# agakshat/spacefortress

Hardware: NVIDIA B200
Metric: env-steps/sec with 84x84 obs (higher is better)
Workload: dtype f64

## Files before the change

### spacefortress_b200/csrc/sf_kernels.cu

```cuda
#include <cuda_runtime.h>
#include <stdio.h>
#include <stdlib.h>
#include <string.h>

#include <algorithm>
#include <mutex>
#include <string>
#include <vector>

#include "../../include/sf_b200.h"
#include "sf_geom.h"
#include "sf_render.cuh"
#include "sf_state.cuh"
#include "sf_step.cuh"
#include "sf_tables.h"

#define SF_WARPS_PER_BLOCK SF_RENDER_WARPS
#define SF_BLOCK (32 * SF_WARPS_PER_BLOCK)
#ifndef SF_BLOCKS_PER_SM
#define SF_BLOCKS_PER_SM 1
#endif

__host__ __device__ inline unsigned sf_hash3(unsigned seed, unsigned long long env, unsigned long long t) {
  unsigned long long z = (env * 0x9E3779B97F4A7C15ull) ^ (t * 0xC2B2AE3D27D4EB4Full) ^ ((unsigned long long)seed << 32 | 0x5Fu);
  z ^= z >> 30; z *= 0xBF58476D1CE4E5B9ull;
  z ^= z >> 27; z *= 0x94D049BB133111EBull;
  z ^= z >> 31;
  return (unsigned)(z >> 32);
}
__host__ __device__ inline int sf_hash_action(unsigned seed, unsigned long long env, unsigned long long t, int num_actions) {
  return (int)(((unsigned long long)sf_hash3(seed, env, t) * (unsigned)num_actions) >> 32);
}

__device__ __forceinline__ long long sf_warp_sum_ll(long long v) {
#pragma unroll
  for (int o = 16; o; o >>= 1) v += __shfl_xor_sync(0xffffffffu, v, o);
  return v;
}

__device__ __noinline__ void sf_accumulate_episode_vals(unsigned long long* epi, bool finished, int lane, int ret_i, int length, int points_bits, int raw_bits,
                                                        int max_vlner, int4 st0, int4 st1, int4 st2) {
  long long f[SF_NUM_EPISODE_STATS];
  long long ret = ret_i;
  f[0] = 1; f[1] = ret; f[2] = ret * ret; f[3] = length;
  f[4] = st0.x; f[5] = st0.y; f[6] = st0.z; f[7] = st0.w;
  f[8] = st1.x; f[9] = st1.y; f[10] = st1.z; f[11] = st1.w;
  f[12] = st2.x; f[13] = st2.y; f[14] = st2.z; f[15] = st2.w; f[16] = max_vlner;
  f[17] = (long long)__float2int_rz(__int_as_float(points_bits));
  f[18] = __double2ll_rn((double)__int_as_float(raw_bits) * 1000.0);
  f[19] = st1.y;
  f[20] = 0; f[21] = 0; f[22] = 0; f[23] = 0;
#pragma unroll
  for (int k = 0; k < 20; k++) {
    long long v = sf_warp_sum_ll(finished ? f[k] : 0);
    if (lane == 0 && v) atomicAdd(&epi[k], (unsigned long long)v);
  }
  int mv = finished ? max_vlner : 0;
  mv = sf_warp_max(mv);
  if (lane == 0 && mv) atomicMax(&epi[20], (unsigned long long)mv);
}
__device__ __forceinline__ void sf_accumulate_episode(const SfDev& D, int env, SfEnv& e, bool finished, int lane) {
  int4 st0 = make_int4(0, 0, 0, 0), st1 = st0, st2 = st0;
  if (finished) { sf_flush_stats(D, env, e); st0 = __ldcg(&D.st0[env]); st1 = __ldcg(&D.st1[env]); st2 = __ldcg(&D.st2[env]); }
  sf_accumulate_episode_vals(D.epi, finished, lane, e.q3.w, e.q3.z, e.q3.x, e.q3.y, e.st3.x, st0, st1, st2);
}
__device__ __noinline__ void sf_accumulate_episode_ref(const SfDev& D, int env, SfEnv& e, bool finished, int lane) {
  sf_accumulate_episode(D, env, e, finished, lane);
}

__device__ __forceinline__ void sf_make_env_rec(const SfEnv& e, int env, unsigned shell_vis, SfEnvRec& r) {
  r.px = e.pos.x; r.py = e.pos.y;
  r.core = (unsigned)e.q0.x; r.pmask = (unsigned)e.q0.y;
  r.points_i = __float2int_rz(__int_as_float(e.q3.x));
  r.vuln = e.q1.z;
  r.kill_bar = (e.q1.z > 10 && e.q1.y < 250) ? 1 : 0;
  r.env = env;
  r.s0 = 0; r.ebox = 0;
  if (!(r.core & SF_CORE_SHIP_ALIVE)) {
    const SfPt c = sf_xform_base(r.px, r.py);
    r.ebox = (((c.x >> 8) - 13) + 64) | ((((c.y >> 8) - 13) + 64) << 8);
  }
  r.life = (unsigned)e.st3.z + 1u;
  r.building = 0;
  r.ns = sf_count_strokes(r.core, r.pmask, shell_vis);
  r.shell_vis = (int)shell_vis;
}

struct SfSched {
  int next_group, done;
};

struct SfRollArgs {
  int T, EB, ngroups, flags;
  const int* actions;
  unsigned action_seed;
  long long t0;
  unsigned char* obs;
  int* reward;
  unsigned char* done;
  unsigned char* fortkill;
  unsigned* events;
  SfSched* sched;
  int env0, envn;
  uint4* host_obs;
  uint4* mirror;
  unsigned long long* delta_stats;
  int delta_lanes;
};

__device__ __noinline__ void sf_step_group(const SfDev& D, const SfRollArgs& A, int group, int t, SfEnvRec* recs) {
  const int lane = threadIdx.x & 31;
  const SfHot* H = &sf_block_smem().hot;
  const bool autoreset = !(A.flags & SF_FLAG_NO_AUTORESET);
  const int env = A.env0 + group * A.EB + lane;
  const bool mine = lane < A.EB && env < A.env0 + A.envn;
  SfEnv e;
  bool finished = false;
  unsigned shell_vis = 0;
#ifdef SF_BARRIER_TIMING
  unsigned stmask_ = __ballot_sync(0xffffffffu, mine);
#endif
  SF_ST_BEGIN();
  SfStepSmem& SS = sf_block_smem().step;
  const bool first_tick = t == 0, last_tick = t == A.T - 1;
  if (mine) {
    if (first_tick) sf_load_env(D, env, e);
    else {
      e.pos = SS.pos[lane]; e.vel = SS.vel[lane];
      e.q0 = SS.q0[lane]; e.q1 = SS.q1[lane]; e.q2 = SS.q2[lane]; e.q3 = SS.q3[lane]; e.st3 = SS.st3[lane];
      e.d0 = SS.d0[lane]; e.d1 = SS.d1[lane]; e.d2 = SS.d2[lane];
    }
#ifdef SF_BARRIER_TIMING
    if (e.q0.x == 0x7fffffff) e.q0.y = 0;
#endif
    SF_ST(8);
    int a = A.actions ? A.actions[(size_t)t * D.n + env]
                      : sf_hash_action(A.action_seed, (unsigned long long)(D.first_global_env + env), (unsigned long long)(A.t0 + t), D.num_actions);
    int km = (A.flags & SF_FLAG_ACTIONS_ARE_KEYMASKS) ? (a & 15) : D.keymask_of_action[min(max(a, 0), D.num_actions - 1)];
    SfStepOut o;
#ifdef SF_BARRIER_TIMING
    o.sync_mask = stmask_;
#endif
    sf_env_step(D, H, env, e, km, autoreset, (A.flags & SF_FLAG_RAW_REWARD) != 0, o);
    size_t oi = (size_t)t * D.n + env;
    if (A.reward) A.reward[oi] = o.reward;
    if (A.done) A.done[oi] = o.done;
    if (A.fortkill) A.fortkill[oi] = o.fort_kill;
    if (A.events) A.events[oi] = o.events;
    finished = o.done && autoreset;
    shell_vis = o.shell_vis;
  }
#ifdef SF_BARRIER_TIMING
  ts_ = clock64(); stmask_ = 0xffffffffu;
#endif
  if (__any_sync(0xffffffffu, finished)) {
#ifdef SF_STEP_ENV_BY_REF
    sf_accumulate_episode_ref(D, env, e, finished, lane);
#else
    sf_accumulate_episode(D, env, e, finished, lane);
#endif
    if (finished) { sf_new_game(D, H, env, e); shell_vis = 0; }
  }
  if (mine) {
    if (last_tick) sf_store_env(D, env, e);
    else {
      SS.pos[lane] = e.pos; SS.vel[lane] = e.vel;
      SS.q0[lane] = e.q0; SS.q1[lane] = e.q1; SS.q2[lane] = e.q2; SS.q3[lane] = e.q3; SS.st3[lane] = e.st3;
      if ((t & 7) == 7) sf_flush_stats(D, env, e);
      SS.d0[lane] = e.d0; SS.d1[lane] = e.d1; SS.d2[lane] = e.d2;
    }
    sf_make_env_rec(e, env, shell_vis, recs[lane]);
  } else recs[lane].env = -1;
  __syncwarp();
  SF_ST(15);
}


__device__ __noinline__ void sf_rollout_stepper(const SfDev& D, const SfRollArgs& A) {
  const int lane = threadIdx.x & 31;
  SfBlockSmem& B = sf_block_smem();
  const bool native = (A.flags & SF_FLAG_NATIVE_OBS) != 0;
  int stage = 0, group = blockIdx.x;
#pragma unroll 1
  for (int k = 1; group < A.ngroups; k ^= 1) {
    if (lane == 0) B.next_group[k] = A.sched ? (int)gridDim.x + atomicAdd(&A.sched->next_group, 1) : group + (int)gridDim.x;
    sf_stepper_ticks(D, B, lane, native, A.T, stage, [&](int t, SfTeamSmem& Tm, int h) { sf_step_group(D, A, group, t, &Tm.env[32 * h]); });
    group = B.next_group[k];
  }
  if (lane == 0 && A.sched) {
    __threadfence();
    if (atomicAdd(&A.sched->done, 1) == (int)gridDim.x - 1) { A.sched->next_group = 0; A.sched->done = 0; __threadfence(); }
  }
}
__device__ __forceinline__ void sf_rollout_drawer(const SfDev& D, const SfRollArgs& A) {
  const int lane = threadIdx.x & 31;
  SfBlockSmem& B = sf_block_smem();
  SfWarpSmem& W = sf_my_smem();
  SfFrameOut out;
  out.native = (A.flags & SF_FLAG_NATIVE_OBS) ? 1 : 0;
  out.obs_bytes = out.native ? (size_t)SF_NAT_H * SF_NAT_W : (size_t)84 * 84;
  out.obs = A.obs;
  out.tick_bytes = (size_t)D.n * out.obs_bytes;
  SfStageState st;
  st.stage = 0; st.prev_used = 0;
  int group = blockIdx.x;
#pragma unroll 1
  for (int k = 1; group < A.ngroups; k ^= 1) {
    sf_drawer_ticks(D, B, W, lane, out, A.T, st);
    group = B.next_group[k];
  }
}

__device__ __noinline__ void sf_block_host_delta(const SfDev& D, const SfRollArgs& A) {
  const unsigned lane = threadIdx.x & 31;
  const unsigned gmask = (1u << A.delta_lanes) - 1u, gsh = lane & ~(unsigned)(A.delta_lanes - 1);
  const uint4* cur = reinterpret_cast<const uint4*>(A.obs);
  const size_t per16 = (size_t)(84 * 84) / 16;
  unsigned sent = 0;
#pragma unroll 1
  for (int group = blockIdx.x; group < A.ngroups; group += gridDim.x) {
    const int env_lo = A.env0 + group * A.EB, env_hi = min(env_lo + A.EB, A.env0 + A.envn);
    const size_t c1 = (size_t)env_hi * per16;
#pragma unroll 1
    for (size_t base = (size_t)env_lo * per16; base < c1; base += 4 * SF_BLOCK) {
      uint4 a[4], b[4];
#pragma unroll
      for (int u = 0; u < 4; u++) {
        const size_t i = base + u * SF_BLOCK + threadIdx.x;
        a[u] = b[u] = make_uint4(0, 0, 0, 0);
        if (i < c1) { a[u] = __ldcg(cur + i); b[u] = __ldcg(A.mirror + i); }
      }
#pragma unroll
      for (int u = 0; u < 4; u++) {
        const size_t i = base + u * SF_BLOCK + threadIdx.x;
        const bool diff = (a[u].x != b[u].x) | (a[u].y != b[u].y) | (a[u].z != b[u].z) | (a[u].w != b[u].w);
        const unsigned m = __ballot_sync(0xffffffffu, diff);
        if (m == 0) continue;
        if (i < c1 && ((m >> gsh) & gmask)) { A.host_obs[i] = a[u]; sent++; }
        if (diff) A.mirror[i] = a[u];
      }
    }
  }
  for (int o = 16; o; o >>= 1) sent += __shfl_xor_sync(0xffffffffu, sent, o);
  if (lane == 0 && sent) atomicAdd(&A.delta_stats[0], (unsigned long long)sent * 16u);
  if (blockIdx.x == 0 && threadIdx.x == 0) atomicAdd(&A.delta_stats[1], 1ull);
}

template <bool HOST_DELTA>
__global__ void __launch_bounds__(SF_BLOCK, SF_BLOCKS_PER_SM) sf_rollout_kernel(const __grid_constant__ SfDev D, const __grid_constant__ SfRollArgs A) {
  sf_block_smem_init(D.static_image);
  sf_warp_smem_init(sf_my_smem(), threadIdx.x & 31);
  if (threadIdx.x < 32) sf_rollout_stepper(D, A); else sf_rollout_drawer(D, A);
  if (HOST_DELTA) {
    __syncthreads();
    sf_block_host_delta(D, A);
  }
}

__global__ void __launch_bounds__(128) sf_step_only_kernel(SfDev D, SfRollArgs A) {
  const int env = A.env0 + blockIdx.x * blockDim.x + threadIdx.x;
  const int lane = threadIdx.x & 31;
  const bool mine = env < A.env0 + A.envn;
  const bool autoreset = !(A.flags & SF_FLAG_NO_AUTORESET);
  SfEnv e;
  if (mine) sf_load_env(D, env, e);
  for (int t = 0; t < A.T; t++) {
    bool finished = false;
    if (mine) {
      int a = A.actions ? A.actions[(size_t)t * D.n + env]
                        : sf_hash_action(A.action_seed, (unsigned long long)(D.first_global_env + env), (unsigned long long)(A.t0 + t), D.num_actions);
      int km = (A.flags & SF_FLAG_ACTIONS_ARE_KEYMASKS) ? (a & 15) : D.keymask_of_action[min(max(a, 0), D.num_actions - 1)];
      SfStepOut o;
#ifdef SF_BARRIER_TIMING
      o.sync_mask = __activemask();
#endif
      sf_env_step(D, &D.tab->hot, env, e, km, autoreset, (A.flags & SF_FLAG_RAW_REWARD) != 0, o);
      size_t oi = (size_t)t * D.n + env;
      if (A.reward) A.reward[oi] = o.reward;
      if (A.done) A.done[oi] = o.done;
      if (A.fortkill) A.fortkill[oi] = o.fort_kill;
      if (A.events) A.events[oi] = o.events;
      finished = o.done && autoreset;
    }
    if (__any_sync(0xffffffffu, finished)) {
      sf_accumulate_episode(D, env, e, finished, lane);
      if (finished) sf_new_game(D, &D.tab->hot, env, e);
    }
    if (mine && (t & 7) == 7) sf_flush_stats(D, env, e);
  }
  if (mine) sf_store_env(D, env, e);
}

__global__ void __launch_bounds__(SF_BLOCK, SF_BLOCKS_PER_SM) sf_render_kernel(SfDev D, unsigned char* obs, int flags, const unsigned char* mask, int EB, int ngroups) {
  const int lane = threadIdx.x & 31;
  SfBlockSmem& B = sf_block_smem();
  SfWarpSmem& W = sf_my_smem();
  sf_block_smem_init(D.static_image);
  sf_warp_smem_init(W, lane);
  const bool native = (flags & SF_FLAG_NATIVE_OBS) != 0;
  if (threadIdx.x < 32) {
    int stage = 0;
#pragma unroll 1
    for (int group = blockIdx.x; group < ngroups; group += gridDim.x)
      sf_stepper_ticks(D, B, lane, native, 1, stage, [&](int, SfTeamSmem& Tm, int) {
        const int env = group * EB + lane;
        const bool mine = lane < EB && env < D.n && (!mask || mask[env]);
        if (mine) {
          SfEnv e;
          sf_load_env(D, env, e);
          sf_make_env_rec(e, env, sf_visible_shells(D, env, (unsigned)e.q0.y), Tm.env[lane]);
        } else Tm.env[lane].env = -1;
        __syncwarp();
      });
  } else {
    SfFrameOut out;
    out.native = native ? 1 : 0;
    out.obs_bytes = out.native ? (size_t)SF_NAT_H * SF_NAT_W : (size_t)84 * 84;
    out.obs = obs;
    out.tick_bytes = 0;
    SfStageState st;
    st.stage = 0; st.prev_used = 0;
#pragma unroll 1
    for (int group = blockIdx.x; group < ngroups; group += gridDim.x) sf_drawer_ticks(D, B, W, lane, out, 1, st);
  }
}

__global__ void __launch_bounds__(SF_BLOCK) sf_pack_static_kernel(SfDev D, unsigned char* image) {
  sf_block_smem_fill(D.tab);
  __syncthreads();
  const int4* src = reinterpret_cast<const int4*>(&sf_block_smem());
  for (int k = threadIdx.x; k < (int)(SF_STATIC_BYTES / 16); k += blockDim.x) reinterpret_cast<int4*>(image)[k] = src[k];
}

__global__ void sf_seed_kernel(SfDev D, const unsigned* seeds) {
  const int env = blockIdx.x * blockDim.x + threadIdx.x;
  if (env >= D.n) return;
  SfEnv e;
  sf_load_env(D, env, e);
  sf_srand(D, env, e, seeds ? seeds[env] : 1u);
  D.expstamp[env] = 0;
  D.expo_meta[env] = make_uint2(0u, 0u);
  sf_store_env(D, env, e);
}

__global__ void sf_set_ticks_kernel(SfDev D, const int* ticks) {
  const int env = blockIdx.x * blockDim.x + threadIdx.x;
  if (env >= D.n) return;
  int4 q = D.q3[env];
  q.z = max(ticks[env], 0);
  D.q3[env] = q;
}

__global__ void sf_reset_kernel(SfDev D, const unsigned char* mask, int clear_prev_vlner) {
  const int env = blockIdx.x * blockDim.x + threadIdx.x;
  if (env >= D.n) return;
  if (mask && !mask[env]) return;
  SfEnv e;
  sf_load_env(D, env, e);
  if (clear_prev_vlner) e.q1.w = 0;
  sf_new_game(D, &D.tab->hot, env, e);
  sf_store_env(D, env, e);
}


struct SfExtra { double vdir, aim, ndist; };
__device__ inline SfExtra sf_compute_extra(const SfEnv& e) {
  SfExtra x;
  x.vdir = 0.0; x.aim = 0.0; x.ndist = 0.0;
  if (e.q3.z == 0) return x;
  const double ang = (double)((unsigned)e.q0.x & SF_CORE_ANGLE_MASK);
  if (SF_DSQRT(SF_DADD(SF_DMUL(e.vel.x, e.vel.x), SF_DMUL(e.vel.y, e.vel.y))) != 0.0) {
    const double o = atan2(-SF_DSUB(SF_FORT_Y, e.pos.y), SF_DSUB(SF_FORT_X, e.pos.x));
    const double v = atan2(e.vel.y, e.vel.x);
    double d = SF_DSUB(v, o);
    if (d > SF_PI) d = SF_DSUB(d, SF_PI * 2);
    if (d < -SF_PI) d = SF_DADD(d, SF_PI * 2);
    x.vdir = sf_rad2deg(d);
  }
  double o = atan2(SF_DSUB(e.pos.y, SF_FORT_Y), SF_DSUB(e.pos.x, SF_FORT_X));
  o = SF_DADD(SF_DSUB(sf_rad2deg(o), ang), 180.0);
  if (o < -180.0) o = SF_DADD(o, 360.0);
  x.aim = o;
  const double dx = SF_DSUB(e.pos.x, SF_FORT_X), dy0 = SF_DSUB(e.pos.y, e.pos.y);
  const double fdist = SF_DSQRT(SF_DADD(SF_DMUL(dx, dx), SF_DMUL(dy0, dy0)));
  x.ndist = SF_DADD(-1.0, SF_DDIV(SF_DSUB(fdist, 40.0), SF_DDIV(SF_DSUB(200.0, 40.0), 2.0)));
  return x;
}
__device__ __forceinline__ double sf_clip1(double v) { return v < -1.0 ? -1.0 : (v > 1.0 ? 1.0 : v); }
__device__ __forceinline__ double sf_pymod360(double v) {
  double m = fmod(v, 360.0);
  if (m != 0.0) { if (m < 0.0) m = SF_DADD(m, 360.0); } else m = 0.0;
  return m;
}

template <class OutT>
__global__ void sf_features_kernel(SfDev D, int kind, OutT* out) {
  const int env = blockIdx.x * blockDim.x + threadIdx.x;
  if (env >= D.n) return;
  SfEnv e;
  sf_load_env(D, env, e);
  const SfExtra x = sf_compute_extra(e);
  const unsigned core = (unsigned)e.q0.x;
  const double alive = (core & SF_CORE_SHIP_ALIVE) ? 1.0 : 0.0, falive = (core & SF_CORE_FORT_ALIVE) ? 1.0 : 0.0;
  const int vuln = e.q1.z;
  const double kill_window = (vuln > 10 && e.q1.y < 250) ? 1.0 : 0.0;
  const int nm = __popc((unsigned)e.q0.y & SF_PMASK_MISSILES), ns = __popc(((unsigned)e.q0.y >> SF_PMASK_SHELL_SHIFT) & 0xFu);
  const double fang = 10.0 * (double)((core >> SF_CORE_FANG_SHIFT) & 63u), sang = (double)(core & SF_CORE_ANGLE_MASK);
  const int nt = D.autoturn ? 2 : 4;
  double f[19];
  int nf;
  if (kind == SF_OBS_MONITORS) {
    nf = 10;
    f[0] = nm > 0 ? 0.5 : -0.5; f[1] = falive != 0.0 ? 0.5 : -0.5; f[2] = vuln > 10 ? 0.5 : -0.5; f[3] = kill_window != 0.0 ? 0.5 : -0.5;
    f[4] = x.aim < 3 ? 0.5 : -0.5; f[5] = x.aim > 3 ? 0.5 : -0.5;
    f[6] = x.ndist > .75 ? 0.5 : -0.5; f[7] = x.ndist > .25 ? 0.5 : -0.5; f[8] = x.ndist < -.25 ? 0.5 : -0.5; f[9] = x.ndist < -.75 ? 0.5 : -0.5;
  } else if (kind == SF_OBS_NORMALIZED_FEATURES) {
    nf = 15 + nt;
    f[0] = alive; f[1] = SF_DDIV(e.pos.x, 90.0); f[2] = SF_DDIV(e.pos.y, 92.0); f[3] = SF_DDIV(e.vel.x, 10.0); f[4] = SF_DDIV(e.vel.y, 10.0);
    f[5] = SF_DDIV(sang, 360.0); f[6] = SF_DDIV(x.aim, 180.0); f[7] = SF_DDIV(sf_pymod360(x.vdir), 360.0); f[8] = x.ndist;
    f[9] = falive; f[10] = SF_DDIV(fang, 360.0); f[11] = SF_DDIV((double)max(vuln, 10), 10.0); f[12] = kill_window;
    f[13] = SF_DDIV((double)nm, 20.0); f[14] = SF_DDIV((double)ns, 20.0);
    const double max_ticks = 5294.0;
    f[15] = SF_DDIV((double)e.q2.x, max_ticks); f[16] = SF_DDIV((double)e.q2.y, max_ticks);
    f[17] = SF_DDIV((double)e.q2.z, max_ticks); f[18] = SF_DDIV((double)e.q2.w, max_ticks);
    for (int k = 0; k < 19; k++) f[k] = sf_clip1(f[k]);
  } else {
    nf = 15 + nt;
    f[0] = alive; f[1] = e.pos.x; f[2] = e.pos.y; f[3] = e.vel.x; f[4] = e.vel.y; f[5] = sang; f[6] = x.aim; f[7] = x.vdir; f[8] = x.ndist;
    f[9] = falive; f[10] = fang; f[11] = (double)vuln; f[12] = kill_window; f[13] = (double)nm; f[14] = (double)ns;
    f[15] = (double)e.q2.x; f[16] = (double)e.q2.y; f[17] = (double)e.q2.z; f[18] = (double)e.q2.w;
  }
  OutT* o = out + (size_t)env * nf;
  for (int k = 0; k < nf; k++) o[k] = (OutT)f[k];
}

__global__ void sf_get_state_kernel(SfDev D, int first, int count, sf_state_record* out) {
  const int k = blockIdx.x * blockDim.x + threadIdx.x;
  if (k >= count) return;
  const int i = first + k;
  const SfTables* T = D.tab;
  SfEnv e;
  sf_load_env(D, i, e);
  sf_state_record r;
  memset(&r, 0, sizeof(r));
  unsigned core = (unsigned)e.q0.x;
  r.ship_x = e.pos.x; r.ship_y = e.pos.y; r.ship_vx = e.vel.x; r.ship_vy = e.vel.y;
  r.ship_angle = (double)(core & SF_CORE_ANGLE_MASK);
  r.fortress_angle = 10.0 * ((core >> SF_CORE_FANG_SHIFT) & 63u);
  r.fortress_last_angle = 10.0 * ((core >> SF_CORE_FLAST_SHIFT) & 63u);
  r.missile_mask = (unsigned)e.q0.y & SF_PMASK_MISSILES;
  r.shell_mask = ((unsigned)e.q0.y >> SF_PMASK_SHELL_SHIFT) & 0xFu;
  for (int s = 0; s < SF_MAX_MISSILES; s++) if ((r.missile_mask >> s) & 1) {
    double2 p = D.mpos[(size_t)s * D.n_pad + i];
    int a = D.mang[(size_t)s * D.n_pad + i];
    r.missile_x[s] = p.x; r.missile_y[s] = p.y; r.missile_angle[s] = a;
    r.missile_vx[s] = SF_DMUL(20.0, T->cos_deg[a]); r.missile_vy[s] = SF_DMUL(20.0, T->sin_deg[a]);
  }
  for (int s = 0; s < SF_DEV_SHELLS; s++) if ((r.shell_mask >> s) & 1) {
    double2 p = D.spos[(size_t)s * D.n_pad + i], v = D.svel[(size_t)s * D.n_pad + i];
    r.shell_x[s] = p.x; r.shell_y[s] = p.y; r.shell_vx[s] = v.x; r.shell_vy[s] = v.y;
    r.shell_angle[s] = D.sang[(size_t)s * D.n_pad + i];
  }
  r.points = __int_as_float(e.q3.x); r.raw_points = __int_as_float(e.q3.y);
  r.ship_alive = (core & SF_CORE_SHIP_ALIVE) != 0; r.fortress_alive = (core & SF_CORE_FORT_ALIVE) != 0;
  r.ship_death_timer = e.q0.z;
  r.fire_timer = e.q2.x; r.thrust_timer = e.q2.y; r.left_timer = e.q2.z; r.right_timer = e.q2.w;
  r.thrust_flag = (core & SF_CORE_THRUST) != 0; r.fire_flag = (core & SF_CORE_FIRE) != 0;
  r.left_flag = (core & SF_CORE_LEFT) != 0; r.right_flag = (core & SF_CORE_RIGHT) != 0;
  r.turn_flag = (r.left_flag && !r.right_flag) ? 1 : (!r.left_flag && r.right_flag) ? 2 : 0;
  r.fortress_timer = e.q0.w; r.fortress_death_timer = e.q1.x; r.fortress_vuln_timer = e.q1.y;
  r.vulnerability = e.q1.z; r.tick = e.q3.z; r.time = e.q3.z * SF_TICK_MS;
  const int4 st0 = D.st0[i], st1 = D.st1[i], st2 = D.st2[i];
  r.stats[0] = st0.x; r.stats[1] = st0.y; r.stats[2] = st0.z; r.stats[3] = st0.w;
  r.stats[4] = st1.x; r.stats[5] = st1.y; r.stats[6] = st1.z; r.stats[7] = st1.w;
  r.stats[8] = st2.x; r.stats[9] = st2.y; r.stats[10] = st2.z; r.stats[11] = st2.w;
  r.stats[12] = e.st3.x;
  r.prev_vlner = e.q1.w;
  r.rng_seed = (unsigned)e.st3.w; r.rng_count = (unsigned)e.st3.z;
  r.ep_return = e.q3.w;
  out[k] = r;
}

__global__ void sf_set_state_kernel(SfDev D, int first, int count, const sf_state_record* in) {
  const int k = blockIdx.x * blockDim.x + threadIdx.x;
  if (k >= count) return;
  const int i = first + k;
  const sf_state_record& r = in[k];
  SfEnv e;
  sf_load_env(D, i, e);
  if ((unsigned)e.st3.w != r.rng_seed || (unsigned)e.st3.z > r.rng_count) sf_srand(D, i, e, r.rng_seed);
  while ((unsigned)e.st3.z < r.rng_count) (void)sf_rand(D, i, e);
  unsigned core = ((unsigned)(int)r.ship_angle & SF_CORE_ANGLE_MASK) | (((unsigned)(int)(r.fortress_angle / 10.0) & 63u) << SF_CORE_FANG_SHIFT) |
                  (((unsigned)(int)(r.fortress_last_angle / 10.0) & 63u) << SF_CORE_FLAST_SHIFT);
  if (r.ship_alive) core |= SF_CORE_SHIP_ALIVE;
  if (r.fortress_alive) core |= SF_CORE_FORT_ALIVE;
  if (r.fire_flag) core |= SF_CORE_FIRE;
  if (r.thrust_flag) core |= SF_CORE_THRUST;
  if (r.left_flag) core |= SF_CORE_LEFT;
  if (r.right_flag) core |= SF_CORE_RIGHT;
  e.pos = make_double2(r.ship_x, r.ship_y); e.vel = make_double2(r.ship_vx, r.ship_vy);
  e.q0 = make_int4((int)core, (int)((r.missile_mask & SF_PMASK_MISSILES) | ((r.shell_mask & 0xFu) << SF_PMASK_SHELL_SHIFT)), r.ship_death_timer, r.fortress_timer);
  e.q1 = make_int4(r.fortress_death_timer, r.fortress_vuln_timer, r.vulnerability, r.prev_vlner);
  e.q2 = make_int4(r.fire_timer, r.thrust_timer, r.left_timer, r.right_timer);
  e.q3 = make_int4(__float_as_int(r.points), __float_as_int(r.raw_points), r.tick, r.ep_return);
  D.st0[i] = make_int4(r.stats[0], r.stats[1], r.stats[2], r.stats[3]);
  D.st1[i] = make_int4(r.stats[4], r.stats[5], r.stats[6], r.stats[7]);
  D.st2[i] = make_int4(r.stats[8], r.stats[9], r.stats[10], r.stats[11]);
  e.st3.x = r.stats[12];
  for (int s = 0; s < SF_MAX_MISSILES; s++) if ((r.missile_mask >> s) & 1) {
    D.mpos[(size_t)s * D.n_pad + i] = make_double2(r.missile_x[s], r.missile_y[s]);
    D.mang[(size_t)s * D.n_pad + i] = (short)(int)r.missile_angle[s];
  }
  for (int s = 0; s < SF_DEV_SHELLS; s++) if ((r.shell_mask >> s) & 1) {
    D.spos[(size_t)s * D.n_pad + i] = make_double2(r.shell_x[s], r.shell_y[s]);
    D.svel[(size_t)s * D.n_pad + i] = make_double2(r.shell_vx[s], r.shell_vy[s]);
    D.sang[(size_t)s * D.n_pad + i] = r.shell_angle[s];
  }
  D.expstamp[i] = 0;
  D.expo_meta[i] = make_uint2(0u, 0u);
  sf_store_env(D, i, e);
}

#define SF_BLOB_CHUNKS (SF_ENV_BLOB_BYTES / 16)
#define SF_BLOB_PITCH (SF_BLOB_CHUNKS + 1)
#define SF_BLOB_BLOCKS_PER_SM 8
enum { SF_BO_POS = 16, SF_BO_VEL = 32, SF_BO_Q = 48, SF_BO_ST = 112, SF_BO_MPOS = 176, SF_BO_SPOS = 496, SF_BO_SVEL = 560,
       SF_BO_SANG = 624, SF_BO_MANG = 656, SF_BO_RNG = 696, SF_BO_END = 820 };
static_assert(SF_BO_MANG + 2 * SF_MAX_MISSILES == SF_BO_RNG && SF_BO_RNG + 4 * SF_RNG_WORDS == SF_BO_END, "blob layout");
static_assert(SF_BO_END <= SF_ENV_BLOB_BYTES && SF_ENV_BLOB_BYTES % 16 == 0, "blob size");

__device__ __forceinline__ void sf_cp_async(void* smem, const void* gmem, int bytes) {
  const unsigned s = (unsigned)__cvta_generic_to_shared(smem);
  if (bytes == 16) asm volatile("cp.async.cg.shared.global [%0], [%1], 16;\n" ::"r"(s), "l"(gmem) : "memory");
  else if (bytes == 8) asm volatile("cp.async.ca.shared.global [%0], [%1], 8;\n" ::"r"(s), "l"(gmem) : "memory");
  else asm volatile("cp.async.ca.shared.global [%0], [%1], 4;\n" ::"r"(s), "l"(gmem) : "memory");
}
__device__ __forceinline__ void sf_cp_async_wait() { asm volatile("cp.async.wait_all;\n" ::: "memory"); }

__global__ void __launch_bounds__(32) sf_save_envs_kernel(SfDev D, int gametype, const int* __restrict__ idx, int count, int4* __restrict__ blob) {
  __shared__ int4 tile[32 * SF_BLOB_PITCH];
  const int lane = threadIdx.x;
  const size_t np = (size_t)D.n_pad;
  int4* row = tile + lane * SF_BLOB_PITCH;
  char* rb = reinterpret_cast<char*>(row);
  const int4 z = make_int4(0, 0, 0, 0);
  for (int base = blockIdx.x * 32; base < count; base += gridDim.x * 32) {
    const int k = base + lane;
    const int i = k < count ? (idx ? idx[k] : k) : -1;
    if (i >= 0 && i < D.n) {
      const int4 q0 = D.q0[i];
      const unsigned pm = (unsigned)q0.y;
      row[0] = make_int4((int)SF_ENV_BLOB_MAGIC, SF_ENV_BLOB_VERSION, gametype, 0);
      sf_cp_async(rb + SF_BO_POS, &D.pos[i], 16);
      sf_cp_async(rb + SF_BO_VEL, &D.vel[i], 16);
      row[SF_BO_Q / 16] = q0;
      sf_cp_async(rb + SF_BO_Q + 16, &D.q1[i], 16);
      sf_cp_async(rb + SF_BO_Q + 32, &D.q2[i], 16);
      sf_cp_async(rb + SF_BO_Q + 48, &D.q3[i], 16);
      sf_cp_async(rb + SF_BO_ST, &D.st0[i], 16);
      sf_cp_async(rb + SF_BO_ST + 16, &D.st1[i], 16);
      sf_cp_async(rb + SF_BO_ST + 32, &D.st2[i], 16);
      sf_cp_async(rb + SF_BO_ST + 48, &D.st3[i], 16);
      short* mang = reinterpret_cast<short*>(rb + SF_BO_MANG);
#pragma unroll
      for (int s = 0; s < SF_MAX_MISSILES; s++) {
        const bool live = (pm >> s) & 1u;
        if (live) sf_cp_async(rb + SF_BO_MPOS + 16 * s, &D.mpos[s * np + i], 16);
        else row[SF_BO_MPOS / 16 + s] = z;
        mang[s] = live ? D.mang[s * np + i] : (short)0;
      }
#pragma unroll
      for (int s = 0; s < SF_DEV_SHELLS; s++) {
        if ((pm >> (SF_PMASK_SHELL_SHIFT + s)) & 1u) {
          sf_cp_async(rb + SF_BO_SPOS + 16 * s, &D.spos[s * np + i], 16);
          sf_cp_async(rb + SF_BO_SVEL + 16 * s, &D.svel[s * np + i], 16);
          sf_cp_async(rb + SF_BO_SANG + 8 * s, &D.sang[s * np + i], 8);
        } else {
          row[SF_BO_SPOS / 16 + s] = z;
          row[SF_BO_SVEL / 16 + s] = z;
          reinterpret_cast<double*>(rb + SF_BO_SANG)[s] = 0.0;
        }
      }
#pragma unroll
      for (int w = 0; w < SF_RNG_WORDS; w++) sf_cp_async(rb + SF_BO_RNG + 4 * w, &D.rng[w * np + i], 4);
      for (int b = SF_BO_END; b < SF_ENV_BLOB_BYTES; b += 4) *reinterpret_cast<int*>(rb + b) = 0;
    } else if (k < count) {
      for (int c = 0; c < SF_BLOB_CHUNKS; c++) row[c] = z;
    }
    sf_cp_async_wait();
    __syncwarp();
    const int rows = min(32, count - base);
    int4* out = blob + (size_t)base * SF_BLOB_CHUNKS;
#pragma unroll 4
    for (int c = lane; c < rows * SF_BLOB_CHUNKS; c += 32) {
      const int r = c / SF_BLOB_CHUNKS;
      out[c] = tile[r * SF_BLOB_PITCH + (c - r * SF_BLOB_CHUNKS)];
    }
    __syncwarp();
  }
}

__global__ void __launch_bounds__(32) sf_load_envs_kernel(SfDev D, int gametype, const int4* __restrict__ blob, const int* __restrict__ idx, int count,
                                                          int* rejected) {
  __shared__ int4 tile[32 * SF_BLOB_PITCH];
  const int lane = threadIdx.x;
  const size_t np = (size_t)D.n_pad;
  const int4* row = tile + lane * SF_BLOB_PITCH;
  const char* rb = reinterpret_cast<const char*>(row);
  for (int base = blockIdx.x * 32; base < count; base += gridDim.x * 32) {
    const int rows = min(32, count - base);
    const int4* in = blob + (size_t)base * SF_BLOB_CHUNKS;
#pragma unroll 4
    for (int c = lane; c < rows * SF_BLOB_CHUNKS; c += 32) {
      const int r = c / SF_BLOB_CHUNKS;
      sf_cp_async(&tile[r * SF_BLOB_PITCH + (c - r * SF_BLOB_CHUNKS)], &in[c], 16);
    }
    sf_cp_async_wait();
    __syncwarp();
    const int k = base + lane;
    const int i = k < count ? (idx ? idx[k] : k) : -1;
    bool ok = false;
    if (k < count) {
      const int4 hd = row[0];
      ok = (unsigned)hd.x == SF_ENV_BLOB_MAGIC && hd.y == SF_ENV_BLOB_VERSION && hd.z == gametype && i >= 0 && i < D.n;
    }
    const unsigned bad = __ballot_sync(0xFFFFFFFFu, k < count && !ok);
    if (lane == 0 && bad && rejected) atomicAdd(rejected, __popc(bad));
    if (ok) {
      const int4 q0 = row[SF_BO_Q / 16];
      const unsigned pm = (unsigned)q0.y;
      D.pos[i] = *reinterpret_cast<const double2*>(rb + SF_BO_POS);
      D.vel[i] = *reinterpret_cast<const double2*>(rb + SF_BO_VEL);
      D.q0[i] = q0;
      D.q1[i] = row[SF_BO_Q / 16 + 1];
      D.q2[i] = row[SF_BO_Q / 16 + 2];
      D.q3[i] = row[SF_BO_Q / 16 + 3];
      D.st0[i] = row[SF_BO_ST / 16];
      D.st1[i] = row[SF_BO_ST / 16 + 1];
      D.st2[i] = row[SF_BO_ST / 16 + 2];
      D.st3[i] = row[SF_BO_ST / 16 + 3];
      const short* mang = reinterpret_cast<const short*>(rb + SF_BO_MANG);
#pragma unroll
      for (int s = 0; s < SF_MAX_MISSILES; s++) if ((pm >> s) & 1u) {
        D.mpos[s * np + i] = *reinterpret_cast<const double2*>(rb + SF_BO_MPOS + 16 * s);
        D.mang[s * np + i] = mang[s];
      }
#pragma unroll
      for (int s = 0; s < SF_DEV_SHELLS; s++) if ((pm >> (SF_PMASK_SHELL_SHIFT + s)) & 1u) {
        D.spos[s * np + i] = *reinterpret_cast<const double2*>(rb + SF_BO_SPOS + 16 * s);
        D.svel[s * np + i] = *reinterpret_cast<const double2*>(rb + SF_BO_SVEL + 16 * s);
        D.sang[s * np + i] = reinterpret_cast<const double*>(rb + SF_BO_SANG)[s];
      }
      const unsigned* rng = reinterpret_cast<const unsigned*>(rb + SF_BO_RNG);
#pragma unroll
      for (int w = 0; w < SF_RNG_WORDS; w++) D.rng[w * np + i] = rng[w];
      D.expstamp[i] = 0;
      D.expo_meta[i] = make_uint2(0u, 0u);
    }
    __syncwarp();
  }
}

static thread_local std::string g_err;
static int fail(int code, const std::string& msg) { g_err = msg; return code; }
#define CUDA_TRY(x) do { cudaError_t e_ = (x); if (e_ != cudaSuccess) return fail(SF_ERR_CUDA, std::string(#x) + ": " + cudaGetErrorString(e_)); } while (0)

#define SF_MAX_MIRRORS 4
#define SF_HOST_MAX_SLICES 8
struct sf_handle {
  SfDev dev;
  int device;
  int action_set;
  int gametype;
  int num_sms;
  void* slab;
  size_t slab_bytes;
  SfTables* h_tab;
  int* d_actions; unsigned char* d_obs; int* d_reward; unsigned char* d_done; unsigned char* d_kill; unsigned* d_events;
  size_t staging_obs_bytes;
  SfSched* d_sched;
  cudaStream_t host_compute, host_copy;
  cudaEvent_t host_ev[SF_HOST_MAX_SLICES];
  int host_slices;
  struct Mirror { const void* host; unsigned char* d; size_t cap, bytes; unsigned long long used; };
  Mirror mirrors[SF_MAX_MIRRORS];
  unsigned long long mirror_clock;
  unsigned long long* d_delta_stats;
  unsigned long long full_calls;
  int delta_lanes;
};

extern "C" const char* sf_last_error(void) { return g_err.c_str(); }
extern "C" int sf_version(void) { return 100; }

static int gametype_of(const char* s) {
  if (!s) return -1;
  if (!strcmp(s, "youturn")) return 0;
  if (!strcmp(s, "autoturn")) return 1;
  if (!strcmp(s, "test-youturn")) return 2;
  if (!strcmp(s, "test-autoturn")) return 3;
  return -1;
}

static int build_actions(int gametype, int action_set, int* km) {
  bool youturn = gametype == 0 || gametype == 2;
  if (action_set == 1) {
    const int tab[5] = {0, SF_KEY_FIRE, SF_KEY_THRUST, SF_KEY_LEFT, SF_KEY_RIGHT};
    int n = youturn ? 5 : 3;
    for (int i = 0; i < n; i++) km[i] = tab[i];
    return n;
  }
  if (action_set == 0 && !youturn) {
    for (int a = 0; a < 4; a++) km[a] = ((a >> 1) & 1 ? SF_KEY_FIRE : 0) | ((a & 1) ? SF_KEY_THRUST : 0);
    return 4;
  }
  if (action_set == 0 || action_set == -1) {
    for (int a = 0; a < 16; a++) {
      int m = ((a >> 1) & 1 ? SF_KEY_FIRE : 0) | ((a & 1) ? SF_KEY_THRUST : 0) | ((a >> 2) & 1 ? SF_KEY_LEFT : 0) | ((a >> 3) & 1 ? SF_KEY_RIGHT : 0);
      km[a] = youturn ? m : (m & (SF_KEY_FIRE | SF_KEY_THRUST));
    }
    return 16;
  }
  return -1;
}

template <class T>
static T* carve(char*& p, size_t count) {
  T* r = reinterpret_cast<T*>(p);
  size_t bytes = (count * sizeof(T) + 255) & ~(size_t)255;
  p += bytes;
  return r;
}

static size_t layout(SfDev& d, char* base) {
  char* p = base;
  size_t np = (size_t)d.n_pad;
  d.pos = carve<double2>(p, np); d.vel = carve<double2>(p, np);
  d.q0 = carve<int4>(p, np); d.q1 = carve<int4>(p, np); d.q2 = carve<int4>(p, np); d.q3 = carve<int4>(p, np);
  d.st0 = carve<int4>(p, np); d.st1 = carve<int4>(p, np); d.st2 = carve<int4>(p, np); d.st3 = carve<int4>(p, np);
  d.mpos = carve<double2>(p, np * SF_MAX_MISSILES); d.mang = carve<short>(p, np * SF_MAX_MISSILES);
  d.spos = carve<double2>(p, np * SF_DEV_SHELLS); d.svel = carve<double2>(p, np * SF_DEV_SHELLS); d.sang = carve<double>(p, np * SF_DEV_SHELLS);
  d.rng = carve<unsigned>(p, np * SF_RNG_WORDS);
  d.expc = carve<unsigned char>(p, np * SF_EXP_W * SF_EXP_W);
  d.expstamp = carve<unsigned>(p, np);
  d.expo = carve<unsigned char>(p, np * SF_EXPO_BYTES);
  d.expo_meta = carve<uint2>(p, np);
  d.epi = carve<unsigned long long>(p, SF_NUM_EPISODE_STATS);
  d.tab = carve<SfTables>(p, 1);
  d.static_image = carve<unsigned char>(p, SF_STATIC_BYTES);
  return (size_t)(p - base);
}

extern "C" int sf_destroy(sf_handle* h);

extern "C" int sf_create(const char* gametype, int action_set, int n_envs, int device, sf_handle** out) {
  if (!out) return fail(SF_ERR_INVALID, "out is NULL");
  *out = nullptr;
  int gt = gametype_of(gametype);
  if (gt < 0) return fail(SF_ERR_INVALID, std::string("cannot initialize Game. Unknown config value: `") + (gametype ? gametype : "(null)") + "'");
  if (n_envs <= 0) return fail(SF_ERR_INVALID, "n_envs must be positive");
  int km[16];
  int na = build_actions(gt, action_set, km);
  if (na < 0) return fail(SF_ERR_INVALID, "action_set must be 1, 0 or -1");
  int ndev = 0;
  CUDA_TRY(cudaGetDeviceCount(&ndev));
  if (device < 0 || device >= ndev) return fail(SF_ERR_CUDA, "no such CUDA device (this library has no CPU fallback)");
  CUDA_TRY(cudaSetDevice(device));
  int num_sms = 0;
  CUDA_TRY(cudaDeviceGetAttribute(&num_sms, cudaDevAttrMultiProcessorCount, device));

  sf_handle* h = new sf_handle();
  memset(h, 0, sizeof(*h));
  h->device = device; h->num_sms = num_sms > 0 ? num_sms : 148; h->action_set = action_set; h->gametype = gt;
  SfDev& d = h->dev;
  d.n = n_envs; d.n_pad = (n_envs + 31) & ~31;
  d.autoturn = (gt == 1 || gt == 3);
  bool test = gt >= 2;
  d.shaped = !test;
  d.destroy_fortress = test ? 100 : 1;
  d.death_penalty = test ? 100 : 1;
  d.missile_penalty = test ? 2.0f : (float)0.05;
  d.num_actions = na;
  for (int i = 0; i < 16; i++) d.keymask_of_action[i] = i < na ? km[i] : 0;
  d.first_global_env = 0;

  h->h_tab = new SfTables();
  char err[256] = {0};
  if (sf_build_tables(h->h_tab, err, sizeof(err))) { std::string m = err; delete h->h_tab; delete h; return fail(SF_ERR_INVALID, "table build failed: " + m); }

  auto bail = [&](const char* what, cudaError_t ce) { std::string m = std::string(what) + ": " + cudaGetErrorString(ce); sf_destroy(h); return fail(SF_ERR_CUDA, m); };
  cudaError_t ce;
  h->slab_bytes = layout(d, nullptr);
  if ((ce = cudaMalloc(&h->slab, h->slab_bytes)) != cudaSuccess) return bail("cudaMalloc state slab", ce);
  layout(d, (char*)h->slab);
  if ((ce = cudaMalloc(&h->d_sched, sizeof(SfSched))) != cudaSuccess) return bail("cudaMalloc scheduler state", ce);
  if ((ce = cudaMemset(h->d_sched, 0, sizeof(SfSched))) != cudaSuccess) return bail("cudaMemset scheduler state", ce);
  if ((ce = cudaMemset(h->slab, 0, h->slab_bytes)) != cudaSuccess) return bail("cudaMemset state slab", ce);
  if ((ce = cudaMemcpy((void*)d.tab, h->h_tab, sizeof(SfTables), cudaMemcpyHostToDevice)) != cudaSuccess) return bail("upload tables", ce);
  if ((ce = cudaFuncSetAttribute(sf_rollout_kernel<false>, cudaFuncAttributeMaxDynamicSharedMemorySize, (int)SF_RENDER_SMEM_BYTES(SF_WARPS_PER_BLOCK))) != cudaSuccess) return bail("shared memory opt-in (rollout)", ce);
  if ((ce = cudaFuncSetAttribute(sf_rollout_kernel<true>, cudaFuncAttributeMaxDynamicSharedMemorySize, (int)SF_RENDER_SMEM_BYTES(SF_WARPS_PER_BLOCK))) != cudaSuccess) return bail("shared memory opt-in (rollout, host delta)", ce);
  if ((ce = cudaFuncSetAttribute(sf_render_kernel, cudaFuncAttributeMaxDynamicSharedMemorySize, (int)SF_RENDER_SMEM_BYTES(SF_WARPS_PER_BLOCK))) != cudaSuccess) return bail("shared memory opt-in (render)", ce);
  if ((ce = cudaFuncSetAttribute(sf_pack_static_kernel, cudaFuncAttributeMaxDynamicSharedMemorySize, (int)SF_RENDER_SMEM_BYTES(SF_WARPS_PER_BLOCK))) != cudaSuccess) return bail("shared memory opt-in (pack)", ce);
  if ((ce = cudaFuncSetAttribute(sf_save_envs_kernel, cudaFuncAttributePreferredSharedMemoryCarveout, (int)cudaSharedmemCarveoutMaxShared)) != cudaSuccess) return bail("shared memory carveout (save envs)", ce);
  if ((ce = cudaFuncSetAttribute(sf_load_envs_kernel, cudaFuncAttributePreferredSharedMemoryCarveout, (int)cudaSharedmemCarveoutMaxShared)) != cudaSuccess) return bail("shared memory carveout (load envs)", ce);
  sf_pack_static_kernel<<<1, SF_BLOCK, SF_RENDER_SMEM_BYTES(SF_WARPS_PER_BLOCK)>>>(d, const_cast<unsigned char*>(d.static_image));
  if ((ce = cudaGetLastError()) != cudaSuccess) return bail("static image kernel launch", ce);
  sf_seed_kernel<<<(d.n + 127) / 128, 128>>>(d, nullptr);
  if ((ce = cudaGetLastError()) != cudaSuccess) return bail("seed kernel launch", ce);
  if ((ce = cudaDeviceSynchronize()) != cudaSuccess) return bail("seed kernel", ce);
  *out = h;
  return SF_OK;
}

extern "C" int sf_destroy(sf_handle* h) {
  if (!h) return SF_OK;
  cudaSetDevice(h->device);
  if (h->slab) cudaFree(h->slab);
  if (h->d_actions) cudaFree(h->d_actions);
  if (h->d_obs) cudaFree(h->d_obs);
  if (h->d_reward) cudaFree(h->d_reward);
  if (h->d_done) cudaFree(h->d_done);
  if (h->d_kill) cudaFree(h->d_kill);
  if (h->d_events) cudaFree(h->d_events);
  if (h->d_sched) cudaFree(h->d_sched);
  for (auto& m : h->mirrors) if (m.d) cudaFree(m.d);
  if (h->d_delta_stats) cudaFree(h->d_delta_stats);
  if (h->host_compute) cudaStreamDestroy(h->host_compute);
  if (h->host_copy) cudaStreamDestroy(h->host_copy);
  for (int k = 0; k < SF_HOST_MAX_SLICES; k++) if (h->host_ev[k]) cudaEventDestroy(h->host_ev[k]);
  delete h->h_tab;
  delete h;
  return SF_OK;
}

extern "C" int sf_num_envs(const sf_handle* h) { return h ? h->dev.n : -1; }
extern "C" int sf_num_actions(const sf_handle* h) { return h ? h->dev.num_actions : -1; }
extern "C" int sf_action_keymask(const sf_handle* h, int action) {
  if (!h || action < 0 || action >= h->dev.num_actions) return -1;
  return h->dev.keymask_of_action[action];
}
extern "C" long long sf_state_bytes(const sf_handle* h) { return h ? (long long)h->slab_bytes : -1; }

extern "C" int sf_seed(sf_handle* h, const uint32_t* h_seeds, long long first_global_env, void* stream) {
  if (!h) return fail(SF_ERR_INVALID, "handle is NULL");
  CUDA_TRY(cudaSetDevice(h->device));
  cudaStream_t st = (cudaStream_t)stream;
  h->dev.first_global_env = first_global_env;
  unsigned* d_seeds = nullptr;
  cudaError_t ce = cudaSuccess;
  if (h_seeds) {
    CUDA_TRY(cudaMalloc(&d_seeds, sizeof(unsigned) * h->dev.n));
    ce = cudaMemcpyAsync(d_seeds, h_seeds, sizeof(unsigned) * h->dev.n, cudaMemcpyHostToDevice, st);
  }
  if (ce == cudaSuccess) {
    sf_seed_kernel<<<(h->dev.n + 127) / 128, 128, 0, st>>>(h->dev, d_seeds);
    ce = cudaGetLastError();
  }
  if (d_seeds) {
    cudaError_t cs = cudaStreamSynchronize(st);
    if (ce == cudaSuccess) ce = cs;
    cudaFree(d_seeds);
  }
  if (ce != cudaSuccess) return fail(SF_ERR_CUDA, std::string("sf_seed: ") + cudaGetErrorString(ce));
  return SF_OK;
}

static void group_shape(const sf_handle* h, int n, int* EB, int* ngroups, int* blocks) {
  const int sms = h->num_sms * SF_BLOCKS_PER_SM, teams = sms;
  int eb = n <= teams * SF_GROUP_ENVS ? (n + teams - 1) / teams : SF_GROUP_ENVS;
  if (const char* ov = getenv("SF_ENVS_PER_BLOCK")) { int e = atoi(ov); if (e >= 1 && e <= SF_GROUP_ENVS) eb = e; }
  *EB = eb;
  *ngroups = (n + eb - 1) / eb;
  *blocks = std::min(*ngroups, sms);
}

static int launch_render(sf_handle* h, unsigned char* d_obs, int flags, const unsigned char* d_mask, cudaStream_t st) {
  int EB, ngroups, blocks;
  group_shape(h, h->dev.n, &EB, &ngroups, &blocks);
  sf_render_kernel<<<blocks, SF_BLOCK, SF_RENDER_SMEM_BYTES(SF_WARPS_PER_BLOCK), st>>>(h->dev, d_obs, flags, d_mask, EB, ngroups);
  CUDA_TRY(cudaGetLastError());
  return SF_OK;
}

#include <cuda_bf16.h>
#define SF_PI_THREADS 192
template <bool F32>
__global__ void __launch_bounds__(SF_PI_THREADS) sf_policy_input_kernel(const unsigned char* __restrict__ frames, long long fstride, int n, const int* __restrict__ valid,
                                                                       uint4* __restrict__ out) {
  __shared__ unsigned tile[2][4 * 4 * 21];
  __shared__ unsigned lut[256];
  const int env = blockIdx.x, tid = threadIdx.x;
  for (int v = tid; v < 256; v += SF_PI_THREADS) {
    if (F32) lut[v] = __float_as_uint(__fmul_rn((float)v, __fdiv_rn(1.0f, 255.0f)));
    else { const __nv_bfloat16 h = __float2bfloat16_rn(__fdiv_rn((float)v, 255.0f)); lut[v] = *reinterpret_cast<const unsigned short*>(&h); }
  }
  const int nvalid = min(max(valid[env], 0), 4);
  const unsigned char* base = frames + (long long)env * (84 * 84);
  const int k1 = tid + SF_PI_THREADS;
  const int f0 = tid / 84, r0 = tid - f0 * 84, f1 = k1 / 84, r1 = k1 - f1 * 84;
  const bool on0 = f0 >= 4 - nvalid, on1 = k1 < 336 && f1 >= 4 - nvalid;
  const unsigned char* p0 = base + (long long)f0 * fstride + (r0 / 21) * 84 + (r0 % 21) * 4;
  const unsigned char* p1 = base + (long long)(k1 < 336 ? f1 : 0) * fstride + (r1 / 21) * 84 + (r1 % 21) * 4;
  const int X = tid >> 3, c8 = tid & 7, f = c8 >> 1, dy0 = (c8 & 1) * 2;
  const int ta = (f * 4 + dy0) * 21 + X, tb = ta + 21;
  uint4* orow = out + (long long)env * (21 * 21 * 8) * (F32 ? 2 : 1);
  auto cvt2 = [&](unsigned lo, unsigned hi) { return lut[lo] | (lut[hi] << 16); };
#pragma unroll 1
  for (int Y = 0; Y < 21; Y++) {
    unsigned* T = tile[Y & 1];
    T[tid] = on0 ? *reinterpret_cast<const unsigned*>(p0 + Y * (4 * 84)) : 0u;
    if (k1 < 336) T[k1] = on1 ? *reinterpret_cast<const unsigned*>(p1 + Y * (4 * 84)) : 0u;
    __syncthreads();
    if (tid < 21 * 8) {
      const unsigned a = T[ta], b = T[tb];
      if (F32) {
        uint4 o0, o1;
        o0.x = lut[a & 255u]; o0.y = lut[(a >> 8) & 255u]; o0.z = lut[(a >> 16) & 255u]; o0.w = lut[a >> 24];
        o1.x = lut[b & 255u]; o1.y = lut[(b >> 8) & 255u]; o1.z = lut[(b >> 16) & 255u]; o1.w = lut[b >> 24];
        orow[(Y * (21 * 8) + tid) * 2] = o0; orow[(Y * (21 * 8) + tid) * 2 + 1] = o1;
      } else {
        uint4 o;
        o.x = cvt2(a & 255u, (a >> 8) & 255u); o.y = cvt2((a >> 16) & 255u, a >> 24);
        o.z = cvt2(b & 255u, (b >> 8) & 255u); o.w = cvt2((b >> 16) & 255u, b >> 24);
        orow[Y * (21 * 8) + tid] = o;
      }
    }
  }
}

static int policy_input_common(const uint8_t* d_frames, long long frame_stride_bytes, int n, const int32_t* d_valid, void* d_out, bool f32, void* stream) {
  if (!d_frames || !d_valid || !d_out || n <= 0 || (frame_stride_bytes & 3)) return fail(SF_ERR_INVALID, "sf_policy_input: bad arguments");
  cudaPointerAttributes pa;
  CUDA_TRY(cudaPointerGetAttributes(&pa, d_frames));
  if (pa.type != cudaMemoryTypeDevice && pa.type != cudaMemoryTypeManaged) return fail(SF_ERR_INVALID, "sf_policy_input: d_frames is not device memory");
  CUDA_TRY(cudaSetDevice(pa.device));
  if (f32) sf_policy_input_kernel<true><<<(unsigned)n, SF_PI_THREADS, 0, (cudaStream_t)stream>>>(d_frames, frame_stride_bytes, n, d_valid, reinterpret_cast<uint4*>(d_out));
  else sf_policy_input_kernel<false><<<(unsigned)n, SF_PI_THREADS, 0, (cudaStream_t)stream>>>(d_frames, frame_stride_bytes, n, d_valid, reinterpret_cast<uint4*>(d_out));
  CUDA_TRY(cudaGetLastError());
  return SF_OK;
}
extern "C" int sf_policy_input(const uint8_t* d_frames, long long frame_stride_bytes, int n, const int32_t* d_valid, void* d_out_bf16, void* stream) {
  return policy_input_common(d_frames, frame_stride_bytes, n, d_valid, d_out_bf16, false, stream);
}
extern "C" int sf_policy_input_f32(const uint8_t* d_frames, long long frame_stride_bytes, int n, const int32_t* d_valid, float* d_out_f32, void* stream) {
  return policy_input_common(d_frames, frame_stride_bytes, n, d_valid, d_out_f32, true, stream);
}

extern "C" int sf_num_features(const sf_handle* h, int obs_type) {
  if (!h) return -1;
  if (obs_type == SF_OBS_MONITORS) return 10;
  if (obs_type == SF_OBS_FEATURES || obs_type == SF_OBS_NORMALIZED_FEATURES) return 15 + (h->dev.autoturn ? 2 : 4);
  return -1;
}
static int features_common(sf_handle* h, int obs_type, void* d_out, bool f64, void* stream) {
  if (!h || !d_out) return fail(SF_ERR_INVALID, "handle or out is NULL");
  if (sf_num_features(h, obs_type) < 0) return fail(SF_ERR_INVALID, "obs_type must be SF_OBS_FEATURES, SF_OBS_NORMALIZED_FEATURES or SF_OBS_MONITORS");
  CUDA_TRY(cudaSetDevice(h->device));
  if (f64) sf_features_kernel<double><<<(h->dev.n + 127) / 128, 128, 0, (cudaStream_t)stream>>>(h->dev, obs_type, (double*)d_out);
  else sf_features_kernel<float><<<(h->dev.n + 127) / 128, 128, 0, (cudaStream_t)stream>>>(h->dev, obs_type, (float*)d_out);
  CUDA_TRY(cudaGetLastError());
  return SF_OK;
}
extern "C" int sf_features(sf_handle* h, int obs_type, float* d_out, void* stream) { return features_common(h, obs_type, d_out, false, stream); }
extern "C" int sf_features_f64(sf_handle* h, int obs_type, double* d_out, void* stream) { return features_common(h, obs_type, d_out, true, stream); }

extern "C" int sf_set_ticks(sf_handle* h, const int32_t* h_ticks) {
  if (!h || !h_ticks) return fail(SF_ERR_INVALID, "handle or ticks is NULL");
  CUDA_TRY(cudaSetDevice(h->device));
  int* d = nullptr;
  CUDA_TRY(cudaMalloc(&d, sizeof(int) * (size_t)h->dev.n));
  cudaError_t ce = cudaDeviceSynchronize();
  if (ce == cudaSuccess) ce = cudaMemcpy(d, h_ticks, sizeof(int) * (size_t)h->dev.n, cudaMemcpyHostToDevice);
  if (ce == cudaSuccess) {
    sf_set_ticks_kernel<<<(h->dev.n + 127) / 128, 128>>>(h->dev, d);
    ce = cudaDeviceSynchronize();
  }
  cudaFree(d);
  if (ce != cudaSuccess) return fail(SF_ERR_CUDA, std::string("sf_set_ticks: ") + cudaGetErrorString(ce));
  return SF_OK;
}

extern "C" int sf_reset(sf_handle* h, const uint8_t* d_mask, int clear_prev_vlner, uint8_t* d_obs, int flags, void* stream) {
  if (!h) return fail(SF_ERR_INVALID, "handle is NULL");
  CUDA_TRY(cudaSetDevice(h->device));
  cudaStream_t st = (cudaStream_t)stream;
  sf_reset_kernel<<<(h->dev.n + 127) / 128, 128, 0, st>>>(h->dev, d_mask, clear_prev_vlner);
  CUDA_TRY(cudaGetLastError());
  if (d_obs) return launch_render(h, d_obs, flags, d_mask, st);
  return SF_OK;
}

extern "C" int sf_render(sf_handle* h, uint8_t* d_obs, int flags, void* stream) {
  if (!h || !d_obs) return fail(SF_ERR_INVALID, "handle or obs is NULL");
  CUDA_TRY(cudaSetDevice(h->device));
  return launch_render(h, d_obs, flags, nullptr, (cudaStream_t)stream);
}

static int launch_rollout(sf_handle* h, const SfRollArgs& a, cudaStream_t st) {
  const SfDev& d = h->dev;
  bool render = (a.flags & SF_FLAG_RENDER) && a.obs;
  if (render) {
    SfRollArgs b = a;
    int blocks;
    group_shape(h, b.envn, &b.EB, &b.ngroups, &blocks);
    b.sched = (a.env0 == 0 && a.envn == d.n && !a.host_obs) ? h->d_sched : nullptr;
    if (b.host_obs) sf_rollout_kernel<true><<<blocks, SF_BLOCK, SF_RENDER_SMEM_BYTES(SF_WARPS_PER_BLOCK), st>>>(d, b);
    else sf_rollout_kernel<false><<<blocks, SF_BLOCK, SF_RENDER_SMEM_BYTES(SF_WARPS_PER_BLOCK), st>>>(d, b);
  } else {
    sf_step_only_kernel<<<(a.envn + 127) / 128, 128, 0, st>>>(d, a);
  }
  CUDA_TRY(cudaGetLastError());
  return SF_OK;
}

extern "C" int sf_step(sf_handle* h, const int32_t* d_actions, uint8_t* d_obs, int32_t* d_reward, uint8_t* d_done,
                       uint8_t* d_fortkill, uint32_t* d_events, int flags, void* stream) {
  if (!h || !d_actions) return fail(SF_ERR_INVALID, "handle or actions is NULL");
  CUDA_TRY(cudaSetDevice(h->device));
  SfRollArgs a = {};
  a.T = 1; a.EB = 1; a.ngroups = 0; a.flags = flags; a.actions = d_actions; a.action_seed = 0; a.t0 = 0;
  a.obs = d_obs; a.reward = d_reward; a.done = d_done; a.fortkill = d_fortkill; a.events = d_events; a.sched = nullptr; a.env0 = 0; a.envn = h->dev.n;
  return launch_rollout(h, a, (cudaStream_t)stream);
}

extern "C" int sf_rollout(sf_handle* h, int T, const int32_t* d_actions, uint32_t action_seed, long long t0, uint8_t* d_obs,
                          int32_t* d_reward, uint8_t* d_done, uint8_t* d_fortkill, int flags, void* stream) {
  if (!h || T <= 0) return fail(SF_ERR_INVALID, "handle is NULL or T <= 0");
  CUDA_TRY(cudaSetDevice(h->device));
  SfRollArgs a = {};
  a.T = T; a.EB = 1; a.ngroups = 0; a.flags = flags; a.actions = d_actions; a.action_seed = action_seed; a.t0 = t0;
  a.obs = d_obs; a.reward = d_reward; a.done = d_done; a.fortkill = d_fortkill; a.events = nullptr; a.sched = nullptr; a.env0 = 0; a.envn = h->dev.n;
  return launch_rollout(h, a, (cudaStream_t)stream);
}

extern "C" int sf_synthetic_action(uint32_t action_seed, long long global_env, long long t, int num_actions) {
  return sf_hash_action(action_seed, (unsigned long long)global_env, (unsigned long long)t, num_actions);
}

template <int LANES>
__global__ void __launch_bounds__(256) sf_host_delta_kernel(const uint4* __restrict__ cur, uint4* __restrict__ mirror, uint4* __restrict__ host,
                                                             size_t n16, int tail, unsigned long long* stats) {
  __shared__ unsigned block_sent;
  if (threadIdx.x == 0) block_sent = 0;
  __syncthreads();
  const unsigned lane = threadIdx.x & 31;
  const size_t stride = (size_t)gridDim.x * blockDim.x;
  const size_t n16_warp = (n16 + 31) & ~(size_t)31;
  unsigned sent = 0;
  for (size_t i = (size_t)blockIdx.x * blockDim.x + threadIdx.x; i < n16_warp; i += stride) {
    const bool in = i < n16;
    uint4 a = make_uint4(0, 0, 0, 0), b = a;
    if (in) { a = __ldcg(cur + i); b = __ldcg(mirror + i); }
    const bool diff = (a.x != b.x) | (a.y != b.y) | (a.z != b.z) | (a.w != b.w);
    const unsigned m = __ballot_sync(0xffffffffu, diff);
    if (m == 0) continue;
    if (in && ((m >> (lane & ~(unsigned)(LANES - 1))) & ((1u << LANES) - 1u))) { host[i] = a; sent++; }
    if (diff) mirror[i] = a;
  }
  if (tail && blockIdx.x == 0 && threadIdx.x < (unsigned)tail) {
    const size_t o = n16 * 16 + threadIdx.x;
    const unsigned char v = reinterpret_cast<const unsigned char*>(cur)[o];
    reinterpret_cast<unsigned char*>(host)[o] = v; reinterpret_cast<unsigned char*>(mirror)[o] = v;
  }
  for (int o = 16; o; o >>= 1) sent += __shfl_xor_sync(0xffffffffu, sent, o);
  if (lane == 0 && sent) atomicAdd(&block_sent, sent);
  __syncthreads();
  if (threadIdx.x == 0) {
    if (block_sent) atomicAdd(&stats[0], (unsigned long long)block_sent * 16u);
    if (blockIdx.x == 0) atomicAdd(&stats[1], 1ull);
  }
}

static int ensure_staging(sf_handle* h, size_t obs_bytes) {
  size_t n = (size_t)h->dev.n;
  if (!h->host_compute) {
    CUDA_TRY(cudaStreamCreateWithFlags(&h->host_compute, cudaStreamNonBlocking));
    CUDA_TRY(cudaStreamCreateWithFlags(&h->host_copy, cudaStreamNonBlocking));
    for (int k = 0; k < SF_HOST_MAX_SLICES; k++) CUDA_TRY(cudaEventCreateWithFlags(&h->host_ev[k], cudaEventDisableTiming));
    h->host_slices = 4;
    if (const char* ov = getenv("SF_HOST_SLICES")) { int v = atoi(ov); if (v >= 1 && v <= SF_HOST_MAX_SLICES) h->host_slices = v; }
    h->delta_lanes = 4;
    if (const char* ov = getenv("SF_DELTA_GRANULE")) { int v = atoi(ov); if (v == 16 || v == 32 || v == 64 || v == 128 || v == 256) h->delta_lanes = v / 16; }
  }
  if (!h->d_actions) {
    CUDA_TRY(cudaMalloc(&h->d_actions, n * 4)); CUDA_TRY(cudaMalloc(&h->d_reward, n * 4));
    CUDA_TRY(cudaMalloc(&h->d_done, n)); CUDA_TRY(cudaMalloc(&h->d_kill, n)); CUDA_TRY(cudaMalloc(&h->d_events, n * 4));
  }
  if (obs_bytes > h->staging_obs_bytes) {
    if (h->d_obs) { cudaFree(h->d_obs); h->d_obs = nullptr; }
    CUDA_TRY(cudaMalloc(&h->d_obs, obs_bytes));
    h->staging_obs_bytes = obs_bytes;
  }
  return SF_OK;
}

extern "C" int sf_host_alloc(void** out, long long bytes) {
  if (!out || bytes <= 0) return fail(SF_ERR_INVALID, "sf_host_alloc: bad arguments");
  CUDA_TRY(cudaHostAlloc(out, (size_t)bytes, cudaHostAllocPortable | cudaHostAllocMapped));
  return SF_OK;
}
extern "C" int sf_host_free(void* p) {
  if (p) CUDA_TRY(cudaFreeHost(p));
  return SF_OK;
}

static void* device_alias(const void* host) {
  cudaPointerAttributes at;
  if (!host || cudaPointerGetAttributes(&at, host) != cudaSuccess) { cudaGetLastError(); return nullptr; }
  return at.type == cudaMemoryTypeHost ? at.devicePointer : nullptr;
}

#ifdef SF_HOST_PROFILE
#include <time.h>
static double g_hp[8]; static long g_hp_calls; static double g_hp_last;
static double hp_now() { timespec ts; clock_gettime(CLOCK_MONOTONIC, &ts); return ts.tv_sec * 1e9 + ts.tv_nsec; }
#define SF_HP(k) do { double t_ = hp_now(); if (k == 0) { g_hp_calls++; } else g_hp[k] += t_ - g_hp_last; g_hp_last = t_; \
  if (k == 5 && g_hp_calls % 512 == 0) { fprintf(stderr, "sf_step_host phases (us): entry %.1f legacy-sync %.1f aliases %.1f launches %.1f wait %.1f\n", \
    g_hp[1] / 512e3, g_hp[2] / 512e3, g_hp[3] / 512e3, g_hp[4] / 512e3, g_hp[5] / 512e3); for (double& v : g_hp) v = 0; } } while (0)
#else
#define SF_HP(k) do {} while (0)
#endif

extern "C" int sf_step_host(sf_handle* h, const int32_t* h_actions, uint8_t* h_obs, int32_t* h_reward, uint8_t* h_done,
                            uint8_t* h_fortkill, uint32_t* h_events, int flags) {
  SF_HP(0);
  if (!h || !h_actions) return fail(SF_ERR_INVALID, "handle or actions is NULL");
  CUDA_TRY(cudaSetDevice(h->device));
  size_t n = (size_t)h->dev.n;
  size_t per = (flags & SF_FLAG_NATIVE_OBS) ? (size_t)SF_NAT_H * SF_NAT_W : (size_t)84 * 84;
  bool render = (flags & SF_FLAG_RENDER) && h_obs;
  int rc = ensure_staging(h, render ? n * per : 0);
  if (rc) return rc;
  cudaStream_t sc = h->host_compute, sx = h->host_copy;
  uint4* host_alias = nullptr;
  sf_handle::Mirror* mir = nullptr;
  const size_t obs_bytes = n * per;
  const bool want_delta = render && (flags & SF_FLAG_HOST_DELTA);
  if (want_delta) {
    host_alias = reinterpret_cast<uint4*>(device_alias(h_obs));
    if (!host_alias) return fail(SF_ERR_INVALID, "SF_FLAG_HOST_DELTA needs a page-locked h_obs (sf_host_alloc, cudaHostAlloc, cudaHostRegister)");
    if (((uintptr_t)h_obs | (uintptr_t)host_alias) & 15) return fail(SF_ERR_INVALID, "SF_FLAG_HOST_DELTA needs a 16-byte aligned h_obs");
    for (auto& m : h->mirrors) if (m.host == h_obs) mir = &m;
    if (!mir) {
      for (auto& m : h->mirrors) if (!mir || (mir->host && (!m.host || m.used < mir->used))) mir = &m;
      mir->host = nullptr;
    }
    if (obs_bytes > mir->cap) {
      if (mir->d) { cudaFree(mir->d); mir->d = nullptr; mir->cap = 0; }
      mir->host = nullptr;
      CUDA_TRY(cudaMalloc(&mir->d, obs_bytes));
      mir->cap = obs_bytes;
    }
    mir->used = ++h->mirror_clock;
    if (!h->d_delta_stats) {
      CUDA_TRY(cudaMalloc(&h->d_delta_stats, 16));
      CUDA_TRY(cudaMemset(h->d_delta_stats, 0, 16));
    }
  }
  const bool delta = want_delta && mir->host == h_obs && mir->bytes == obs_bytes;
  flags &= ~SF_FLAG_HOST_DELTA;
  SF_HP(1);
  CUDA_TRY(cudaStreamSynchronize(cudaStreamLegacy));
  SF_HP(2);
  const int* k_actions = (const int*)device_alias(h_actions);
  int* k_reward = (int*)device_alias(h_reward);
  unsigned char* k_done = (unsigned char*)device_alias(h_done);
  unsigned char* k_kill = (unsigned char*)device_alias(h_fortkill);
  unsigned* k_events = (unsigned*)device_alias(h_events);
  SF_HP(3);
  if (!k_actions) CUDA_TRY(cudaMemcpyAsync(h->d_actions, h_actions, n * 4, cudaMemcpyHostToDevice, sc));
  const int slices = (render && !delta && n >= 2048) ? h->host_slices : 1;
  const bool fused_delta = delta && per % 16 == 0;
  for (int k = 0; k < slices; k++) {
    const size_t e0 = n * k / slices, e1 = n * (k + 1) / slices;
    SfRollArgs a = {};
    a.T = 1; a.EB = 1; a.ngroups = 0; a.flags = render ? flags : (flags & ~SF_FLAG_RENDER); a.action_seed = 0; a.t0 = 0;
    a.actions = k_actions ? k_actions : h->d_actions;
    a.obs = render ? h->d_obs : nullptr; a.reward = k_reward ? k_reward : h->d_reward; a.done = k_done ? k_done : h->d_done;
    a.fortkill = k_kill ? k_kill : h->d_kill; a.events = k_events ? k_events : h->d_events; a.sched = nullptr;
    a.env0 = (int)e0; a.envn = (int)(e1 - e0);
    if (fused_delta) { a.host_obs = host_alias; a.mirror = reinterpret_cast<uint4*>(mir->d); a.delta_stats = h->d_delta_stats; a.delta_lanes = h->delta_lanes; }
    rc = launch_rollout(h, a, sc);
    if (rc) { cudaStreamSynchronize(sc); cudaStreamSynchronize(sx); return rc; }
    if (render && !delta) {
      CUDA_TRY(cudaEventRecord(h->host_ev[k], sc));
      CUDA_TRY(cudaStreamWaitEvent(sx, h->host_ev[k], 0));
      CUDA_TRY(cudaMemcpyAsync(h_obs + e0 * per, h->d_obs + e0 * per, (e1 - e0) * per, cudaMemcpyDeviceToHost, sx));
    }
  }
  if (delta && !fused_delta) {
    const size_t n16 = obs_bytes / 16;
    const int blocks = (int)std::min<size_t>((n16 + 255) / 256, (size_t)h->num_sms * 8);
    auto kern = h->delta_lanes == 1 ? sf_host_delta_kernel<1> : (h->delta_lanes >= 4 ? sf_host_delta_kernel<4> : sf_host_delta_kernel<2>);
    kern<<<std::max(blocks, 1), 256, 0, sc>>>(reinterpret_cast<const uint4*>(h->d_obs), reinterpret_cast<uint4*>(mir->d), host_alias,
                                              n16, (int)(obs_bytes & 15), h->d_delta_stats);
    CUDA_TRY(cudaGetLastError());
  } else if (want_delta) {
    CUDA_TRY(cudaMemcpyAsync(mir->d, h->d_obs, obs_bytes, cudaMemcpyDeviceToDevice, sc));
    mir->host = h_obs; mir->bytes = obs_bytes;
  }
  if (render && !delta) h->full_calls++;
  if (h_reward && !k_reward) CUDA_TRY(cudaMemcpyAsync(h_reward, h->d_reward, n * 4, cudaMemcpyDeviceToHost, sc));
  if (h_done && !k_done) CUDA_TRY(cudaMemcpyAsync(h_done, h->d_done, n, cudaMemcpyDeviceToHost, sc));
  if (h_fortkill && !k_kill) CUDA_TRY(cudaMemcpyAsync(h_fortkill, h->d_kill, n, cudaMemcpyDeviceToHost, sc));
  if (h_events && !k_events) CUDA_TRY(cudaMemcpyAsync(h_events, h->d_events, n * 4, cudaMemcpyDeviceToHost, sc));
  SF_HP(4);
  cudaError_t e1 = cudaStreamSynchronize(sc), e2 = (render && !delta) ? cudaStreamSynchronize(sx) : cudaSuccess;
  SF_HP(5);
  if (e1 != cudaSuccess || e2 != cudaSuccess) {
    for (auto& m : h->mirrors) m.host = nullptr;
    return fail(SF_ERR_CUDA, std::string("sf_step_host: ") + cudaGetErrorString(e1 != cudaSuccess ? e1 : e2));
  }
  return SF_OK;
}

extern "C" int sf_host_forget(sf_handle* h, const void* h_obs) {
  if (!h) return fail(SF_ERR_INVALID, "handle is NULL");
  for (auto& m : h->mirrors) if (m.host == h_obs || !h_obs) m.host = nullptr;
  return SF_OK;
}

extern "C" int sf_host_delta_stats(sf_handle* h, unsigned long long* out3) {
  if (!h || !out3) return fail(SF_ERR_INVALID, "handle or out is NULL");
  CUDA_TRY(cudaSetDevice(h->device));
  out3[0] = out3[1] = 0; out3[2] = h->full_calls;
  if (h->d_delta_stats) {
    CUDA_TRY(cudaStreamSynchronize(h->host_compute));
    CUDA_TRY(cudaMemcpy(out3, h->d_delta_stats, 16, cudaMemcpyDeviceToHost));
  }
  return SF_OK;
}

extern "C" int sf_get_state(sf_handle* h, int first, int count, sf_state_record* h_out) {
  if (!h || !h_out || first < 0 || count < 0 || first + count > h->dev.n) return fail(SF_ERR_INVALID, "bad range");
  if (count == 0) return SF_OK;
  CUDA_TRY(cudaSetDevice(h->device));
  sf_state_record* d = nullptr;
  CUDA_TRY(cudaMalloc(&d, sizeof(sf_state_record) * (size_t)count));
  cudaError_t ce = cudaDeviceSynchronize();
  if (ce == cudaSuccess) {
    sf_get_state_kernel<<<(count + 63) / 64, 64>>>(h->dev, first, count, d);
    ce = cudaMemcpy(h_out, d, sizeof(sf_state_record) * (size_t)count, cudaMemcpyDeviceToHost);
  }
  cudaFree(d);
  if (ce != cudaSuccess) return fail(SF_ERR_CUDA, std::string("get_state: ") + cudaGetErrorString(ce));
  return SF_OK;
}

extern "C" int sf_set_state(sf_handle* h, int first, int count, const sf_state_record* h_in) {
  if (!h || !h_in || first < 0 || count < 0 || first + count > h->dev.n) return fail(SF_ERR_INVALID, "bad range");
  for (int k = 0; k < count; k++) {
    const sf_state_record& r = h_in[k];
    if (r.ship_angle != (double)(int)r.ship_angle || r.ship_angle < 0 || r.ship_angle >= 360)
      return fail(SF_ERR_UNSUPPORTED, "ship_angle must be an integer degree in [0,360) (it always is in the reference: game.cpp:148,317-324)");
    double fa = r.fortress_angle / 10.0, fl = r.fortress_last_angle / 10.0;
    if (fa != (double)(int)fa || fa < 0 || fa >= 36 || fl != (double)(int)fl || fl < 0 || fl >= 36)
      return fail(SF_ERR_UNSUPPORTED, "fortress angles must be multiples of 10 in [0,360) (game.cpp:40-41,206)");
    if (r.shell_mask >> SF_DEV_SHELLS) return fail(SF_ERR_UNSUPPORTED, "shell slots >= 4 can never be alive (at most 3 shells are in flight)");
    if (r.missile_mask >> SF_MAX_MISSILES) return fail(SF_ERR_INVALID, "missile_mask has more than 20 bits");
    for (int s = 0; s < SF_MAX_MISSILES; s++) if ((r.missile_mask >> s) & 1) {
      double a = r.missile_angle[s];
      if (a != (double)(int)a || a < 0 || a >= 360) return fail(SF_ERR_UNSUPPORTED, "missile angles must be integer degrees in [0,360)");
    }
  }
  if (count == 0) return SF_OK;
  CUDA_TRY(cudaSetDevice(h->device));
  sf_state_record* d = nullptr;
  CUDA_TRY(cudaMalloc(&d, sizeof(sf_state_record) * (size_t)count));
  cudaError_t ce = cudaMemcpy(d, h_in, sizeof(sf_state_record) * (size_t)count, cudaMemcpyHostToDevice);
  if (ce == cudaSuccess) ce = cudaDeviceSynchronize();
  if (ce == cudaSuccess) {
    sf_set_state_kernel<<<(count + 63) / 64, 64>>>(h->dev, first, count, d);
    ce = cudaDeviceSynchronize();
  }
  cudaFree(d);
  if (ce != cudaSuccess) return fail(SF_ERR_CUDA, std::string("set_state: ") + cudaGetErrorString(ce));
  return SF_OK;
}

static int blob_args(const sf_handle* h, const int32_t* d_env_idx, int count, const void* d_blob) {
  if (!h || !d_blob) return fail(SF_ERR_INVALID, "handle or blob is NULL");
  if (count < 0 || (!d_env_idx && count > h->dev.n)) return fail(SF_ERR_INVALID, "count out of range");
  if ((uintptr_t)d_blob & 15) return fail(SF_ERR_INVALID, "the blob must be 16-byte aligned");
  return SF_OK;
}
static int blob_blocks(const sf_handle* h, int count) { return std::min((count + 31) / 32, h->num_sms * SF_BLOB_BLOCKS_PER_SM); }

extern "C" int sf_save_envs(sf_handle* h, const int32_t* d_env_idx, int count, uint8_t* d_blob, void* stream) {
  if (int rc = blob_args(h, d_env_idx, count, d_blob)) return rc;
  if (count == 0) return SF_OK;
  CUDA_TRY(cudaSetDevice(h->device));
  sf_save_envs_kernel<<<blob_blocks(h, count), 32, 0, (cudaStream_t)stream>>>(h->dev, h->gametype, d_env_idx, count, reinterpret_cast<int4*>(d_blob));
  CUDA_TRY(cudaGetLastError());
  return SF_OK;
}

extern "C" int sf_load_envs(sf_handle* h, const uint8_t* d_blob, const int32_t* d_env_idx, int count, int32_t* d_rejected, void* stream) {
  if (int rc = blob_args(h, d_env_idx, count, d_blob)) return rc;
  if (count == 0) return SF_OK;
  CUDA_TRY(cudaSetDevice(h->device));
  sf_load_envs_kernel<<<blob_blocks(h, count), 32, 0, (cudaStream_t)stream>>>(h->dev, h->gametype, reinterpret_cast<const int4*>(d_blob), d_env_idx, count, d_rejected);
  CUDA_TRY(cudaGetLastError());
  return SF_OK;
}

__global__ void sf_epi_copy_kernel(unsigned long long* epi, long long* out, int reset) {
  int k = threadIdx.x;
  if (k < SF_NUM_EPISODE_STATS) {
    out[k] = (long long)epi[k];
    if (reset) epi[k] = 0;
  }
}

extern "C" int sf_episode_stats(sf_handle* h, long long* d_out, int reset, void* stream) {
  if (!h || !d_out) return fail(SF_ERR_INVALID, "handle or out is NULL");
  CUDA_TRY(cudaSetDevice(h->device));
  sf_epi_copy_kernel<<<1, 32, 0, (cudaStream_t)stream>>>(h->dev.epi, d_out, reset);
  CUDA_TRY(cudaGetLastError());
  return SF_OK;
}

#ifdef SF_BARRIER_TIMING
extern "C" int sf_barrier_cycles(unsigned long long* h_out, int reset) {
  cudaDeviceSynchronize();
  cudaMemcpyFromSymbol(h_out, sf_bar_cycles, sizeof(unsigned long long) * 16);
  if (reset) { unsigned long long z[16] = {0}; cudaMemcpyToSymbol(sf_bar_cycles, z, sizeof(z)); }
  return SF_OK;
}
#endif
#ifdef SF_TIMELINE
extern "C" int sf_timeline(unsigned long long* h_out) {
  cudaDeviceSynchronize();
  cudaMemcpyFromSymbol(h_out, sf_tl, sizeof(unsigned long long) * 160 * 2 * SF_TL_MAX);
  static unsigned long long z[160 * 2 * SF_TL_MAX];
  cudaMemcpyToSymbol(sf_tl, z, sizeof(z));
  return SF_TL_MAX;
}
#endif
#ifdef SF_PHASE_TIMING
extern "C" int sf_debug_cycles(unsigned long long* h_out, int reset) {
  cudaDeviceSynchronize();
  cudaMemcpyFromSymbol(h_out, sf_dbg_cycles, sizeof(unsigned long long) * 96);
  if (reset) { unsigned long long z[96] = {0}; cudaMemcpyToSymbol(sf_dbg_cycles, z, sizeof(z)); }
  return SF_OK;
}
#endif

extern "C" int sf_set_glyph_masks(sf_handle* h, const uint8_t* h_alpha, const uint8_t* h_slot) {
  if (!h || (!h_alpha) != (!h_slot)) return fail(SF_ERR_INVALID, "handle is NULL, or only one of alpha / slot given");
  SfTables* nt = new SfTables();
  char err[256] = {0};
  if (sf_build_tables_glyphs(nt, err, sizeof(err), h_alpha, h_slot)) { std::string m = err; delete nt; return fail(SF_ERR_INVALID, "table build failed: " + m); }
  cudaError_t ce = cudaSetDevice(h->device);
  if (ce == cudaSuccess) ce = cudaDeviceSynchronize();
  if (ce == cudaSuccess) ce = cudaMemcpy((void*)h->dev.tab, nt, sizeof(SfTables), cudaMemcpyHostToDevice);
  if (ce == cudaSuccess) ce = cudaMemset(h->dev.expo_meta, 0, sizeof(uint2) * (size_t)h->dev.n_pad);
  if (ce == cudaSuccess) {
    sf_pack_static_kernel<<<1, SF_BLOCK, SF_RENDER_SMEM_BYTES(SF_WARPS_PER_BLOCK)>>>(h->dev, const_cast<unsigned char*>(h->dev.static_image));
    ce = cudaGetLastError();
    if (ce == cudaSuccess) ce = cudaDeviceSynchronize();
  }
  if (ce != cudaSuccess) { delete nt; return fail(SF_ERR_CUDA, std::string("sf_set_glyph_masks: ") + cudaGetErrorString(ce)); }
  delete h->h_tab;
  h->h_tab = nt;
  return SF_OK;
}

extern "C" int sf_background(const sf_handle* h, uint8_t* h_native, uint8_t* h_obs) {
  if (!h) return fail(SF_ERR_INVALID, "handle is NULL");
  if (h_native)
    for (int r = 0; r < SF_NAT_H; r++) memcpy(h_native + r * SF_NAT_W, h->h_tab->bg_nat + r * SF_NAT_STRIDE, SF_NAT_W);
  if (h_obs) memcpy(h_obs, h->h_tab->bg_obs, 84 * 84);
  return SF_OK;
}
```

### spacefortress_b200/csrc/sf_render.cuh

```cuda
#pragma once
#include "sf_geom.h"
#include "sf_state.cuh"
#include "sf_tables.h"

#define SF_GROUP_ENVS_ 32
#define SF_BATCH_QUADS 32
#define SF_MAX_GROUPS 256
#define SF_PATCH_STRIDE 32
#define SF_PATCH_BYTES (36 * 32)
#define SF_WIN_MAX_W 31
#define SF_WIN_MAX_H 34
#define SF_YBIAS 4096
#define SF_TAG_SHIP 0
#define SF_TAG_PROJECTILE 1
#define SF_SPAN_NONE 0xFFFFFFFFu
#define SF_QF_IRREGULAR 2

#ifndef SF_RENDER_WARPS
#define SF_RENDER_WARPS 24
#endif
#define SF_FORT_LIST_SMEM 48
#define SF_GROUP_ENVS 32
#ifndef SF_STAGE_TICKS
#define SF_STAGE_TICKS 2
#endif
#define SF_STAGE_SLOTS (SF_GROUP_ENVS * SF_STAGE_TICKS)
#define SF_ROUND_STROKES (8 * (SF_RENDER_WARPS - 1))
#define SF_CELLS_SHIP 144
#define SF_CELLS_MISSILE 49
#define SF_CELLS_SHELL 49
#ifndef SF_POOL_CELLS
#define SF_POOL_CELLS 12288
#endif
#define SF_POOL_REGIONS SF_ROUND_STROKES


struct __align__(16) SfWarpSmem {
  union {
    int4 edge[SF_BATCH_QUADS * 4];
    unsigned char patch[SF_PATCH_BYTES];
  };
  int4 qinfo[SF_BATCH_QUADS];
  int4 srec[SF_BATCH_QUADS];
  unsigned short glist[SF_MAX_GROUPS];
  int ngroups, pad0, pad1, pad2;
#ifdef SF_PHASE_TIMING
  long long prof_last, prof_pad;
#endif
};

struct __align__(16) SfEnvRec {
  double px, py;
  unsigned core, pmask;
  int points_i, vuln, kill_bar;
  int env;
  int s0, ns;
  int ebox;
  int shell_vis;
  int building;
  unsigned life;
};
__device__ __forceinline__ unsigned sf_expo_key(const SfEnvRec& r) {
  const int fst = (r.core & (1u << 22)) ? (int)((r.core >> 9) & 63u) : 36;
  const int bst = r.kill_bar ? 11 : min(r.vuln, 10);
  return (unsigned)fst | ((unsigned)bst << 6) | (((unsigned)r.points_i & 0x3FFFFu) << 10);
}
struct __align__(8) SfStrokeRec { double x, y; int desc, region; };

struct __align__(16) SfTeamSmem {
  SfEnvRec env[SF_STAGE_SLOTS];
  SfStrokeRec stroke[SF_ROUND_STROKES];
  int4 region[SF_POOL_REGIONS];
  int r0, r1, nstrokes, build_env;
  int next_task, netask, next_patch, chunk;
  int more, nticks, build_env2, base_ready;
  int nregions, cells_used, dbg_max_b, dbg_max_c;
  unsigned short etask[SF_STAGE_SLOTS * 5];
  unsigned short exp_item0[SF_EXP_QUADS];
  short exp_qxmin[SF_EXP_QUADS];
  signed char exp_row0[SF_EXP_QUADS];
  unsigned short exp_len[SF_EXPT_ITEMS][SF_EXPT_NC];
  alignas(16) unsigned arc_mask[SF_EXP_W * SF_EXP_W][4];
  alignas(16) unsigned short cells[SF_POOL_CELLS];
};

struct __align__(16) SfStepSmem {
  double2 pos[SF_GROUP_ENVS_], vel[SF_GROUP_ENVS_];
  int4 q0[SF_GROUP_ENVS_], q1[SF_GROUP_ENVS_], q2[SF_GROUP_ENVS_], q3[SF_GROUP_ENVS_], st3[SF_GROUP_ENVS_];
  unsigned d0[SF_GROUP_ENVS_], d1[SF_GROUP_ENVS_], d2[SF_GROUP_ENVS_];
};

struct __align__(16) SfBlockSmem {
  int4 xtap[84];
  int4 ytap[84];
  alignas(16) unsigned char bg_obs[84 * 84];
  alignas(16) unsigned char bg_nat[SF_NAT_H * SF_NAT_STRIDE];
  unsigned char col_out0[SF_NAT_W + 2], col_out1[SF_NAT_W + 2], row_out0[SF_NAT_H], row_out1[SF_NAT_H];
  unsigned char fort_rect[SF_FORT_STATES][4];
  unsigned short fort_list_xy[36][SF_FORT_LIST_SMEM];
  unsigned char fort_list_a[36][SF_FORT_LIST_SMEM];
  unsigned char fort_list_n[36];
  unsigned char fort_sparse[SF_FORT_STATES][16];
  alignas(16) unsigned magic[SF_MAGIC_N];
  alignas(16) SfHot hot;
  double wf_line[3][4][4];
  int wf_nlines[4];
  unsigned colour_white, padc[3];
  unsigned char exp_colour[SF_EXP_STROKES + 3];
  alignas(16) unsigned long long init_mbar, pad_mbar;
#ifdef SF_TIMELINE
  int tl_n[4];
#endif
  int next_group[2], padg[2];
  SfStepSmem step;
  SfTeamSmem team[2];
};

#define SF_STATIC_BYTES ((offsetof(SfBlockSmem, init_mbar) + 15) & ~(size_t)15)

extern __shared__ __align__(16) unsigned char sf_smem_raw[];
__device__ __forceinline__ SfBlockSmem& sf_block_smem() { return *reinterpret_cast<SfBlockSmem*>(sf_smem_raw); }
__device__ __forceinline__ SfTeamSmem& sf_team(int sg) { return sf_block_smem().team[sg]; }
#ifdef SF_BARRIER_TIMING
__device__ unsigned long long sf_bar_cycles[16];
__device__ __forceinline__ void sf_bar_add(int k, long long t0) { if ((threadIdx.x & 31) == 0) atomicAdd(&sf_bar_cycles[k], (unsigned long long)(clock64() - t0)); }
#endif
__device__ __forceinline__ void sf_team_sync() {
#ifdef SF_BARRIER_TIMING
  const long long t0 = clock64();
#endif
  asm volatile("bar.sync 1, %0;" :: "r"(32 * SF_RENDER_WARPS) : "memory");
#ifdef SF_BARRIER_TIMING
  sf_bar_add(threadIdx.x < 32 ? 2 : 0, t0);
#endif
}
__device__ __forceinline__ void sf_render_sync() {
#ifdef SF_BARRIER_TIMING
  const long long t0 = clock64();
#endif
  asm volatile("bar.sync 2, %0;" :: "r"(32 * (SF_RENDER_WARPS - 1)) : "memory");
#ifdef SF_BARRIER_TIMING
  sf_bar_add(1, t0);
#endif
}
#ifdef SF_TIMELINE
#define SF_TL_MAX 96
__device__ unsigned long long sf_tl[160 * 2 * SF_TL_MAX];
__device__ __forceinline__ void sf_tl_mark(int tag) {
  const int warp = threadIdx.x >> 5;
  if ((threadIdx.x & 31) == 0 && warp < 2 && blockIdx.x < 160) {
    SfBlockSmem& B = sf_block_smem();
    const int k = B.tl_n[warp]++;
    if (k < SF_TL_MAX) {
      unsigned long long g;
      asm volatile("mov.u64 %0, %%globaltimer;" : "=l"(g));
      sf_tl[(blockIdx.x * 2 + warp) * SF_TL_MAX + k] = (g << 8) | (unsigned long long)tag;
    }
  }
}
#define SF_TL(tag) sf_tl_mark(tag)
#else
#define SF_TL(tag) ((void)0)
#endif
__device__ __forceinline__ SfWarpSmem& sf_warp_smem(int warp) { return reinterpret_cast<SfWarpSmem*>(sf_smem_raw + sizeof(SfBlockSmem))[warp]; }
__device__ __forceinline__ SfWarpSmem& sf_my_smem() { return sf_warp_smem(threadIdx.x >> 5); }
#define SF_RENDER_SMEM_BYTES(warps) (sizeof(SfBlockSmem) + sizeof(SfWarpSmem) * (warps))

#ifdef SF_PHASE_TIMING
__device__ unsigned long long sf_dbg_cycles[96];
__device__ __forceinline__ void sf_prof(int k) {
  if ((threadIdx.x & 31) == 0 && blockIdx.x == 0) {
    SfWarpSmem& W = sf_my_smem();
    const long long now = clock64();
    atomicAdd(&sf_dbg_cycles[k], (unsigned long long)(now - W.prof_last));
    W.prof_last = now;
  }
}
__device__ __forceinline__ void sf_prof_reset() { if ((threadIdx.x & 31) == 0 && blockIdx.x == 0) sf_my_smem().prof_last = clock64(); }
__device__ __forceinline__ void sf_prof_count(int k, int v) { if ((threadIdx.x & 31) == 0 && blockIdx.x == 0) atomicAdd(&sf_dbg_cycles[k], (unsigned long long)v); }
#define SF_PROF(k) sf_prof(k)
#define SF_PROF_RESET() sf_prof_reset()
#define SF_PROF_COUNT(k, v) sf_prof_count(k, v)
#else
#define SF_PROF(k) ((void)0)
#define SF_PROF_RESET() ((void)0)
#define SF_PROF_COUNT(k, v) ((void)0)
#endif

__device__ __forceinline__ int sf_warp_min(int v) {
#pragma unroll
  for (int o = 16; o; o >>= 1) v = min(v, __shfl_xor_sync(0xffffffffu, v, o));
  return v;
}
__device__ __forceinline__ int sf_warp_max(int v) {
#pragma unroll
  for (int o = 16; o; o >>= 1) v = max(v, __shfl_xor_sync(0xffffffffu, v, o));
  return v;
}
__device__ __forceinline__ int sf_div_small(int a, int b, float inv_b) {
  return __float2int_rz(((float)a + 0.5f) * inv_b);
}
__device__ __forceinline__ int sf_div15(int d) { return (d * 2185) >> 15; }

__device__ __forceinline__ void sf_block_smem_fill(const SfTables* T) {
  SfBlockSmem& B = sf_block_smem();
  for (int k = threadIdx.x; k < 168; k += blockDim.x) {
    const SfTap t = k < 84 ? T->xtap[k] : T->ytap[k - 84];
    int4 v = make_int4(t.si | (t.cnt << 8), __float_as_int(t.a[0]), __float_as_int(t.a[1]), __float_as_int(t.a[2]));
    if (k < 84) B.xtap[k] = v; else B.ytap[k - 84] = v;
  }
  for (int k = threadIdx.x; k < 84 * 84 / 16; k += blockDim.x) reinterpret_cast<int4*>(B.bg_obs)[k] = __ldg(reinterpret_cast<const int4*>(T->bg_obs) + k);
  for (int k = threadIdx.x; k < SF_NAT_H * SF_NAT_STRIDE / 16; k += blockDim.x) reinterpret_cast<int4*>(B.bg_nat)[k] = __ldg(reinterpret_cast<const int4*>(T->bg_nat) + k);
  for (int k = threadIdx.x; k < SF_NAT_W + 2; k += blockDim.x) { B.col_out0[k] = k < SF_NAT_W ? (unsigned char)T->col_out0[k] : 0; B.col_out1[k] = k < SF_NAT_W ? (unsigned char)T->col_out1[k] : 0; }
  for (int k = threadIdx.x; k < SF_NAT_H; k += blockDim.x) { B.row_out0[k] = (unsigned char)T->row_out0[k]; B.row_out1[k] = (unsigned char)T->row_out1[k]; }
  for (int k = threadIdx.x; k < SF_FORT_STATES * 4; k += blockDim.x) B.fort_rect[k >> 2][k & 3] = T->fort_rect[k >> 2][k & 3];
  for (int k = threadIdx.x; k < 36 * SF_FORT_LIST_SMEM; k += blockDim.x) {
    const int st = k / SF_FORT_LIST_SMEM, i = k - st * SF_FORT_LIST_SMEM;
    B.fort_list_xy[st][i] = T->fort_list_xy[st][i]; B.fort_list_a[st][i] = i < T->fort_list_n[st] ? T->fort_list_a[st][i] : 0;
  }
  if (threadIdx.x < 36) B.fort_list_n[threadIdx.x] = (unsigned char)min(T->fort_list_n[threadIdx.x], 255);
  for (int k = threadIdx.x; k < SF_FORT_STATES * 16; k += blockDim.x) B.fort_sparse[k >> 4][k & 15] = T->fort_sparse[k >> 4][k & 15];
  for (int k = threadIdx.x; k < SF_MAGIC_N; k += blockDim.x) B.magic[k] = T->magic[k];
  for (int k = threadIdx.x; k < (int)(sizeof(SfHot) / 16); k += blockDim.x) reinterpret_cast<int4*>(&B.hot)[k] = __ldg(reinterpret_cast<const int4*>(&T->hot) + k);
  for (int k = threadIdx.x; k < 48; k += blockDim.x) (&B.wf_line[0][0][0])[k] = (&T->wf_line[0][0][0])[k];
  if (threadIdx.x < 4) B.wf_nlines[threadIdx.x] = threadIdx.x < 3 ? T->wf_nlines[threadIdx.x] : 0;
  if (threadIdx.x < 4) (&B.colour_white)[threadIdx.x] = threadIdx.x == 0 ? T->colour_white : 0u;
  for (int k = threadIdx.x; k < SF_EXP_STROKES + 3; k += blockDim.x) B.exp_colour[k] = k < SF_EXP_STROKES ? T->exp_colour[k] : 0;
}

__device__ __forceinline__ void sf_block_smem_init(const unsigned char* image) {
  SfBlockSmem& B = sf_block_smem();
#ifdef SF_TIMELINE
  if ((threadIdx.x & 31) == 0 && (threadIdx.x >> 5) < 2) B.tl_n[threadIdx.x >> 5] = 0;
  SF_TL(1);
#endif
  const unsigned bar = (unsigned)__cvta_generic_to_shared(&B.init_mbar);
  if (threadIdx.x == 0) {
    asm volatile("mbarrier.init.shared::cta.b64 [%0], 1;" :: "r"(bar) : "memory");
    asm volatile("fence.mbarrier_init.release.cluster;" ::: "memory");
    asm volatile("mbarrier.arrive.expect_tx.shared::cta.b64 _, [%0], %1;" :: "r"(bar), "r"((unsigned)SF_STATIC_BYTES) : "memory");
    asm volatile("cp.async.bulk.shared::cluster.global.mbarrier::complete_tx::bytes [%0], [%1], %2, [%3];"
                 :: "r"((unsigned)__cvta_generic_to_shared(&B)), "l"(image), "r"((unsigned)SF_STATIC_BYTES), "r"(bar) : "memory");
  }
  for (int c = 0; c < 2; c++) {
    for (int k = threadIdx.x; k < SF_POOL_CELLS / 2; k += blockDim.x) reinterpret_cast<unsigned*>(B.team[c].cells)[k] = 0u;
    for (int k = threadIdx.x; k < SF_EXP_W * SF_EXP_W * 4; k += blockDim.x) (&B.team[c].arc_mask[0][0])[k] = 0u;
    if (threadIdx.x == 32) {
      SfTeamSmem& Tm = B.team[c];
      Tm.next_task = 0; Tm.next_patch = 0; Tm.netask = 0; Tm.chunk = 8; Tm.nregions = 0; Tm.cells_used = 0;
    }
  }
  asm volatile("fence.proxy.async.shared::cta;" ::: "memory");
  __syncthreads();
  unsigned ok;
  do {
    asm volatile("{ .reg .pred p; mbarrier.try_wait.parity.shared::cta.b64 p, [%1], 0; selp.u32 %0, 1, 0, p; }" : "=r"(ok) : "r"(bar) : "memory");
  } while (!ok);
  SF_TL(2);
}
__device__ __forceinline__ void sf_warp_smem_init(SfWarpSmem& W, int lane) {
  if (lane == 0) W.ngroups = 0;
  __syncwarp();
}

template <class F>
__device__ __forceinline__ void sf_for_rect(int lane, int w, int h, F body) {
  const int s = w <= 8 ? 3 : (w <= 16 ? 4 : 5);
  const int c = lane & ((1 << s) - 1), rstep = 32 >> s;
  if (c < w)
    for (int r = lane >> s; r < h; r += rstep) body(c, r);
}

template <class L, class S>
__device__ __forceinline__ void sf_for_rect4(int lane, int w, int h, L load, S store) {
  const int s = w <= 8 ? 3 : (w <= 16 ? 4 : 5);
  const int c = lane & ((1 << s) - 1), rstep = 32 >> s;
  if (c < w)
    for (int r = lane >> s; r < h; r += 4 * rstep) {
      const int r1 = r + rstep, r2 = r + 2 * rstep, r3 = r + 3 * rstep;
      auto v0 = load(c, r);
      auto v1 = load(c, r1 < h ? r1 : r), v2 = load(c, r2 < h ? r2 : r), v3 = load(c, r3 < h ? r3 : r);
      store(c, r, v0);
      if (r1 < h) store(c, r1, v1);
      if (r2 < h) store(c, r2, v2);
      if (r3 < h) store(c, r3, v3);
    }
}

__device__ __forceinline__ int4 sf_make_edge(const SfTables* T, int xa, int ga, int xb, int gb) {
  const int dy = gb - ga, dx = xb - xa;
  const unsigned M = sf_block_smem().magic[min(dy, SF_MAGIC_N - 1)];
  const int a = ga + SF_YBIAS, b = gb + SF_YBIAS;
  if (dy == 1) return make_int4(xa, a | (b << 16), 0, 0);
  return dx >= 0 ? make_int4(xa, a | (b << 16), dx, (int)M) : make_int4(xb, b | (a << 16), dx, (int)M);
}
__device__ __forceinline__ int sf_edge_x(int4 E, int sb) {
  return E.x + (int)__umulhi((unsigned)((sb - (E.y & 0xFFFF)) * E.z), (unsigned)E.w);
}

struct SfQuadGeom {
  int ymin_g, ymax_g, xmin, xmax;
  int split;
  int flags;
};

__device__ __noinline__ void sf_store_quad_edges(const SfTables* T, int qi, int x0, int y0, int x1, int y1, int x2, int y2, int x3, int y3,
                                                  SfQuadGeom& G) {
  SfWarpSmem& W = sf_my_smem();
  const int g0 = sf_grid_y(y0), g1 = sf_grid_y(y1), g2 = sf_grid_y(y2), g3 = sf_grid_y(y3);
  const int4 none = make_int4(0, 0, 0, 0);
  int4 E0 = none, E1 = none, E2 = none, E3 = none;
  int d0 = 0, d1 = 0, d2 = 0, d3 = 0;
  if (g0 < g1) { E0 = sf_make_edge(T, x0, g0, x1, g1); d0 = 1; } else if (g0 > g1) { E0 = sf_make_edge(T, x1, g1, x0, g0); d0 = -1; }
  if (g1 < g2) { E1 = sf_make_edge(T, x1, g1, x2, g2); d1 = 1; } else if (g1 > g2) { E1 = sf_make_edge(T, x2, g2, x1, g1); d1 = -1; }
  if (g2 < g3) { E2 = sf_make_edge(T, x2, g2, x3, g3); d2 = 1; } else if (g2 > g3) { E2 = sf_make_edge(T, x3, g3, x2, g2); d2 = -1; }
  if (g3 < g0) { E3 = sf_make_edge(T, x3, g3, x0, g0); d3 = 1; } else if (g3 > g0) { E3 = sf_make_edge(T, x0, g0, x3, g3); d3 = -1; }
  const int nd = (d0 > 0) + (d1 > 0) + (d2 > 0) + (d3 > 0), nu = (d0 < 0) + (d1 < 0) + (d2 < 0) + (d3 < 0);
  const int gmin = min(min(g0, g1), min(g2, g3)), gmax = max(max(g0, g1), max(g2, g3));
  G.flags = 0; G.split = 0;
  if (nd == 0 || nu == 0) { G.ymin_g = 1 << 30; G.ymax_g = -(1 << 30); G.xmin = 1 << 30; G.xmax = -(1 << 30); return; }
  if (nd > 2 || nu > 2) {
    W.edge[qi * 4 + 0] = E0; W.edge[qi * 4 + 1] = E1; W.edge[qi * 4 + 2] = E2; W.edge[qi * 4 + 3] = E3;
    G.flags = SF_QF_IRREGULAR;
  } else {
    auto top = [](int4 E) { return min(E.y & 0xFFFF, (int)((unsigned)E.y >> 16)); };
    int4 dnA = d0 > 0 ? E0 : d1 > 0 ? E1 : d2 > 0 ? E2 : E3;
    int4 dnB = d3 > 0 ? E3 : d2 > 0 ? E2 : d1 > 0 ? E1 : E0;
    int4 upA = d0 < 0 ? E0 : d1 < 0 ? E1 : d2 < 0 ? E2 : E3;
    int4 upB = d3 < 0 ? E3 : d2 < 0 ? E2 : d1 < 0 ? E1 : E0;
    if (top(dnB) < top(dnA)) { int4 t = dnA; dnA = dnB; dnB = t; }
    if (top(upB) < top(upA)) { int4 t = upA; upA = upB; upB = t; }
    W.edge[qi * 4 + 0] = dnA; W.edge[qi * 4 + 1] = dnB; W.edge[qi * 4 + 2] = upA; W.edge[qi * 4 + 3] = upB;
    G.split = top(dnB) | (top(upB) << 16);
  }
  G.ymin_g = gmin; G.ymax_g = gmax;
  G.xmin = min(min(x0, x1), min(x2, x3)); G.xmax = max(max(x0, x1), max(x2, x3));
}


__device__ __forceinline__ int sf_row_of(int g) { return (g >= 0) ? g / SF_GRID_Y : -((-g + SF_GRID_Y - 1) / SF_GRID_Y); }

__device__ __forceinline__ int sf_open_regions(int lane, bool want, int ymin_g, int ymax_g, int xmin, int xmax, unsigned colour, int tag, int sg) {
  SfTeamSmem& Tm = sf_team(sg);
  int cx0 = 0, py0 = 0, w = 0, h = 0;
  bool ok = want && ymin_g < ymax_g;
  if (ok) {
    py0 = max(sf_row_of(ymin_g), 0); int py1 = min(sf_row_of(ymax_g - 1), SF_NAT_H - 1);
    cx0 = max(xmin >> 8, 0); int cx1 = min((xmax - 1) >> 8, SF_NAT_W - 1);
    ok = py0 <= py1 && cx0 <= cx1;
    w = cx1 - cx0 + 1; h = py1 - py0 + 1;
    if (w > 255 || h > 255) ok = false;
  }
  const int cells = ok ? w * h : 0;
  int incl = cells;
#pragma unroll
  for (int o = 1; o < 32; o <<= 1) { int t = __shfl_up_sync(0xffffffffu, incl, o); if (lane >= o) incl += t; }
  const unsigned okmask = __ballot_sync(0xffffffffu, ok);
  int base_c = 0, base_r = 0;
  if (lane == 31) { base_c = atomicAdd(&Tm.cells_used, incl); base_r = atomicAdd(&Tm.nregions, __popc(okmask)); }
  base_c = __shfl_sync(0xffffffffu, base_c, 31); base_r = __shfl_sync(0xffffffffu, base_r, 31);
  const int rid = base_r + __popc(okmask & ((1u << lane) - 1u));
  if (ok && (base_c + incl > SF_POOL_CELLS || rid >= SF_POOL_REGIONS)) ok = false;
  if (!ok) return -1;
  Tm.region[rid] = make_int4(cx0, py0, w | (h << 16), (base_c + incl - cells) | (tag << 15) | ((int)colour << 16));
  return rid;
}

__device__ __forceinline__ void sf_publish_quads(SfWarpSmem& W, int lane, const SfQuadGeom& G, bool has, int rid, bool head, int slot, int nq, int ymin_g, int ymax_g, int sg) {
  const SfTeamSmem& Tm = sf_team(sg);
  int len = 0;
  int4 R = make_int4(0, 0, 0, 0);
  if (rid >= 0) R = Tm.region[rid];
  const int w = R.z & 0xFFFF, h = (R.z >> 16) & 0xFFFF;
  const int top = R.y * SF_GRID_Y + SF_YBIAS;
  if (has && rid >= 0) {
    const int g0 = max(G.ymin_g + SF_YBIAS, top), g1 = min(G.ymax_g + SF_YBIAS, top + h * SF_GRID_Y);
    W.qinfo[lane] = make_int4(g0 | (max(g1, g0) << 16), G.split, G.flags, 0);
  } else W.qinfo[lane] = make_int4(0, 0, 0, 0);
  if (head && rid >= 0) {
    const int s0 = max(ymin_g + SF_YBIAS, top), s1 = min(ymax_g + SF_YBIAS, top + h * SF_GRID_Y);
    len = max(s1 - s0, 0);
    W.srec[slot] = make_int4(R.x | (w << 8) | (nq << 16) | (lane << 24), top, R.w & 0x7FFF, s0 | (max(s1, s0) << 16));
  }
  const int n8 = (len + 7) >> 3;
  int gs = n8;
#pragma unroll
  for (int o = 1; o < 32; o <<= 1) { int t = __shfl_up_sync(0xffffffffu, gs, o); if (lane >= o) gs += t; }
  const int total = __shfl_sync(0xffffffffu, gs, 31);
  gs -= n8;
  for (int k = 0; k < n8; k++)
    if (gs + k < SF_MAX_GROUPS) W.glist[gs + k] = (unsigned short)(slot | (k << 5));
  if (lane == 0) W.ngroups = min(total, SF_MAX_GROUPS);
  __syncwarp();
}

__device__ __forceinline__ unsigned sf_quad_span_regular(const SfWarpSmem& W, int q, int sb, int xlo, int xhi) {
  const int4 Q = W.qinfo[q];
  const int4 Ed = W.edge[q * 4 + (sb >= (Q.y & 0xFFFF) ? 1 : 0)];
  const int4 Eu = W.edge[q * 4 + 2 + (sb >= (int)((unsigned)Q.y >> 16) ? 1 : 0)];
  const int xd = sf_edge_x(Ed, sb), xu = sf_edge_x(Eu, sb);
  const int lo = max(min(xd, xu), xlo) - xlo, hi = min(max(xd, xu), xhi) - xlo;
  const bool live = sb >= (Q.x & 0xFFFF) && sb < (int)((unsigned)Q.x >> 16) && lo < hi;
  return live ? (((unsigned)lo << 16) | (unsigned)hi) : SF_SPAN_NONE;
}

__device__ __forceinline__ void sf_emit_span_pred(unsigned* acc32, int cell0, int a, int b) {
  const bool any = a < b;
  const int c1 = a >> 8, c2 = (b - 1) >> 8;
  const int ci = cell0 + c1, cj = cell0 + c2;
  const unsigned len1 = (unsigned)(min(b, (c1 + 1) << 8) - a), len2 = (unsigned)(b - (c2 << 8));
  if (any) atomicAdd(&acc32[ci >> 1], len1 << ((ci & 1) << 4));
  if (any && c2 > c1) atomicAdd(&acc32[cj >> 1], len2 << ((cj & 1) << 4));
  if (any && c2 > c1 + 1)
    for (int c = c1 + 1; c < c2; c++) { const int cm = cell0 + c; atomicAdd(&acc32[cm >> 1], 256u << ((cm & 1) << 4)); }
}

__device__ __noinline__ void sf_accumulate_pass(int owner, int g0, int sg) {
  const SfWarpSmem& W = sf_warp_smem(owner);
  const int lane = threadIdx.x & 31;
  const int ngroups = W.ngroups;
  unsigned* acc32 = reinterpret_cast<unsigned*>(sf_team(sg).cells);
  const int gi = min(g0 + (lane >> 3), ngroups - 1);
  const int ent = W.glist[gi];
  const int4 S = W.srec[ent & 31];
  const int sb = (S.w & 0xFFFF) + ((ent >> 5) << 3) + (lane & 7);
  const bool valid = g0 + (lane >> 3) < ngroups && sb < (int)((unsigned)S.w >> 16);
  const int q0 = (int)((unsigned)S.x >> 24);
  const int w = (S.x >> 8) & 255;
  const int xlo = (S.x & 255) << 8, xhi = xlo + (w << 8);
  const int cell0 = S.z + sf_div15(max(sb - S.y, 0)) * w;
  unsigned k0 = sf_quad_span_regular(W, q0, sb, xlo, xhi);
  unsigned k1 = sf_quad_span_regular(W, q0 + 1, sb, xlo, xhi);
  unsigned k2 = sf_quad_span_regular(W, q0 + 2, sb, xlo, xhi);
  unsigned k3 = SF_SPAN_NONE;
  if (__any_sync(0xffffffffu, ((S.x >> 16) & 255) > 3)) k3 = sf_quad_span_regular(W, q0 + 3, sb, xlo, xhi);
  if (!valid) { k0 = SF_SPAN_NONE; k1 = SF_SPAN_NONE; k2 = SF_SPAN_NONE; k3 = SF_SPAN_NONE; }
  unsigned t0 = min(k0, k1), t1 = max(k0, k1), t2 = min(k2, k3), t3 = max(k2, k3);
  k0 = min(t0, t2); k2 = max(t0, t2);
  k1 = min(t1, t3); k3 = max(t1, t3);
  t0 = min(k1, k2); k2 = max(k1, k2); k1 = t0;
  int reach = 0;
  { const int a = (int)(k0 >> 16), b = k0 == SF_SPAN_NONE ? 0 : (int)(k0 & 0xFFFFu); sf_emit_span_pred(acc32, cell0, a, b); reach = b; }
  { const int a = max((int)(k1 >> 16), reach), b = k1 == SF_SPAN_NONE ? 0 : (int)(k1 & 0xFFFFu); sf_emit_span_pred(acc32, cell0, a, b); reach = max(reach, b); }
  { const int a = max((int)(k2 >> 16), reach), b = k2 == SF_SPAN_NONE ? 0 : (int)(k2 & 0xFFFFu); sf_emit_span_pred(acc32, cell0, a, b); reach = max(reach, b); }
  { const int a = max((int)(k3 >> 16), reach), b = k3 == SF_SPAN_NONE ? 0 : (int)(k3 & 0xFFFFu); sf_emit_span_pred(acc32, cell0, a, b); }
}

#define SF_WIN_X0(win) ((win) & 255)
#define SF_WIN_Y0(win) (((win) >> 8) & 255)
#define SF_WIN_W(win) (((win) >> 16) & 255)
#define SF_WIN_H(win) (((unsigned)(win)) >> 24)

__device__ __forceinline__ void sf_patch_init(SfWarpSmem& W, const SfTables* T, int lane, int win) {
  const int nx0 = SF_WIN_X0(win), ny0 = SF_WIN_Y0(win);
  const unsigned char* bg = sf_block_smem().bg_nat + ny0 * SF_NAT_STRIDE + nx0;
  sf_for_rect(lane, SF_WIN_W(win), SF_WIN_H(win), [&](int c, int r) { W.patch[r * SF_PATCH_STRIDE + c] = bg[r * SF_NAT_STRIDE + c]; });
  __syncwarp();
}

__device__ __noinline__ void sf_blend_region(int rid, int win, int sg) {
  SfWarpSmem& W = sf_my_smem();
  const SfTeamSmem& O = sf_team(sg);
  const int lane = threadIdx.x & 31;
  const int4 R = O.region[rid];
  const int w = R.z & 0xFFFF, h = (R.z >> 16) & 0xFFFF;
  const int nx0 = SF_WIN_X0(win), ny0 = SF_WIN_Y0(win);
  const int ix0 = max(R.x, nx0), ix1 = min(R.x + w, nx0 + SF_WIN_W(win));
  const int iy0 = max(R.y, ny0), iy1 = min(R.y + h, ny0 + (int)SF_WIN_H(win));
  if (ix0 >= ix1 || iy0 >= iy1) return;
  const unsigned colour = ((unsigned)R.w >> 16) & 255u;
  const unsigned short* cells = O.cells + (R.w & 0x7FFF) + (iy0 - R.y) * w + (ix0 - R.x);
  unsigned char* p0 = W.patch + (iy0 - ny0) * SF_PATCH_STRIDE + (ix0 - nx0);
  sf_for_rect(lane, ix1 - ix0, iy1 - iy0, [&](int c, int r) {
    unsigned L = cells[r * w + c];
    if (L) {
      unsigned char* px = p0 + r * SF_PATCH_STRIDE + c;
      *px = (unsigned char)sf_blend(*px, colour, sf_len_to_alpha(L));
    }
  });
  __syncwarp();
}

__device__ __noinline__ bool sf_composite(const SfTables* T, unsigned char* expcache, int e, int win, int sg) {
  SfWarpSmem& W = sf_my_smem();
  const SfBlockSmem& B = sf_block_smem();
  const SfEnvRec& rec = sf_team(sg).env[e];
  const int lane = threadIdx.x & 31;
  const unsigned core = rec.core;
  const int nx0 = SF_WIN_X0(win), ny0 = SF_WIN_Y0(win);
  const int nx1 = nx0 + SF_WIN_W(win), ny1 = ny0 + (int)SF_WIN_H(win);
  SF_PROF(31);
  sf_patch_init(W, T, lane, win);
  SF_PROF(22);
  int sr = -1, tag = SF_TAG_PROJECTILE;
  bool hit = false;
  if (lane < rec.ns) {
    sr = sf_team(sg).stroke[rec.s0 + lane].region;
    if (sr >= 0) {
      const int4 R = sf_team(sg).region[sr];
      hit = R.x < nx1 && R.x + (R.z & 0xFFFF) > nx0 && R.y < ny1 && R.y + ((R.z >> 16) & 0xFFFF) > ny0;
      tag = (R.w >> 15) & 1;
    }
  }
  unsigned rmask = __ballot_sync(0xffffffffu, hit);
  const bool no_wireframe = rmask == 0u;
  const bool first_is_ship = __shfl_sync(0xffffffffu, tag, 0) == SF_TAG_SHIP;
  SF_PROF(23);
  if (core & SF_CORE_SHIP_ALIVE) {
    if ((rmask & 1u) && first_is_ship) { const int s0r = __shfl_sync(0xffffffffu, sr, 0); sf_blend_region(s0r, win, sg); rmask &= ~1u; }
  } else {
    const int ebox = rec.ebox;
    const int bx0 = (ebox & 255) - 64, by0 = ((ebox >> 8) & 255) - 64;
    const int ix0 = max(max(bx0, 0), nx0), ix1 = min(min(bx0 + SF_EXP_W, SF_NAT_W), nx1);
    const int iy0 = max(max(by0, 0), ny0), iy1 = min(min(by0 + SF_EXP_W, SF_NAT_H), ny1);
    if (ix0 < ix1 && iy0 < iy1) {
      {
        const unsigned* src32 = reinterpret_cast<const unsigned*>(expcache + (iy0 - by0) * SF_EXP_W);
        const int nw = (SF_EXP_W / 4) * (iy1 - iy0);
        unsigned v[7];
#pragma unroll
        for (int u = 0; u < 7; u++) v[u] = lane + 32 * u < nw ? __ldcg(&src32[lane + 32 * u]) : 0u;
#pragma unroll
        for (int u = 0; u < 7; u++) {
          const int k = lane + 32 * u;
          if (k < nw) {
            const int row = (k * 9363) >> 16, x4 = bx0 + (k - row * (SF_EXP_W / 4)) * 4;
            unsigned char* dst = W.patch + (iy0 + row - ny0) * SF_PATCH_STRIDE - nx0;
#pragma unroll
            for (int b = 0; b < 4; b++)
              if (x4 + b >= ix0 && x4 + b < ix1) dst[x4 + b] = (unsigned char)(v[u] >> (8 * b));
          }
        }
      }
      __syncwarp();
    }
  }
  SF_PROF(24);
  {
    const int fst = (core & SF_CORE_FORT_ALIVE) ? (int)((core >> SF_CORE_FANG_SHIFT) & 63u) : 36;
    const unsigned char* fr = B.fort_rect[fst];
    if ((int)fr[0] < nx1 && (int)fr[2] >= nx0 && (int)fr[1] < ny1 && (int)fr[3] >= ny0) {
      if (fst < 36) {
        const int n = B.fort_list_n[fst];
        const bool in_smem = n <= SF_FORT_LIST_SMEM;
#pragma unroll 1
        for (int k = lane; k < n; k += 32) {
          const int xy = in_smem ? B.fort_list_xy[fst][k] : T->fort_list_xy[fst][k];
          const unsigned a = in_smem ? B.fort_list_a[fst][k] : T->fort_list_a[fst][k];
          const int x = xy & 255, y = xy >> 8;
          if (x >= nx0 && x < nx1 && y >= ny0 && y < ny1) {
            unsigned char* px = &W.patch[(y - ny0) * SF_PATCH_STRIDE + (x - nx0)];
            *px = (unsigned char)sf_blend(*px, B.colour_white, a);
          }
        }
      } else {
        const int ix0 = max(SF_FEXP_X0, nx0), ix1 = min(SF_FEXP_X0 + SF_EXP_W, nx1);
        const int iy0 = max(SF_FEXP_Y0, ny0), iy1 = min(SF_FEXP_Y0 + SF_EXP_W, ny1);
        if (ix0 < ix1 && iy0 < iy1) {
          sf_for_rect(lane, ix1 - ix0, iy1 - iy0, [&](int c, int r) {
            const int idx = (iy0 + r - SF_FEXP_Y0) * SF_EXP_W + (ix0 + c - SF_FEXP_X0);
            unsigned a0 = T->fexp_alpha[0][idx];
            if (a0) {
              unsigned char* px = &W.patch[(iy0 + r - ny0) * SF_PATCH_STRIDE + (ix0 + c - nx0)];
              unsigned v = sf_blend(*px, T->fexp_colour[0][idx], a0);
              for (int l = 1; l < T->fexp_layers; l++) {
                unsigned a = T->fexp_alpha[l][idx];
                if (!a) break;
                v = sf_blend(v, T->fexp_colour[l][idx], a);
              }
              *px = (unsigned char)v;
            }
          });
        }
      }
      __syncwarp();
    }
  }
  SF_PROF(25);
#pragma unroll 1
  while (rmask) {
    const int q = __ffs(rmask) - 1;
    rmask &= rmask - 1;
    const int sq = __shfl_sync(0xffffffffu, sr, q);
    sf_blend_region(sq, win, sg);
  }
  SF_PROF(26);
  {
    const int ix0 = max(SF_TEXT_X0, nx0), ix1 = min(SF_TEXT_X0 + SF_TEXT_W, nx1);
    const int iy0 = max(SF_TEXT_Y0, ny0), iy1 = min(SF_TEXT_Y0 + SF_TEXT_H, ny1);
    if (ix0 < ix1 && iy0 < iy1) {
      const int pts = min(max(rec.points_i, 0), 9999999);
      sf_for_rect(lane, ix1 - ix0, iy1 - iy0, [&](int c, int r) {
        const int tc = ix0 + c - SF_TEXT_X0, tr = iy0 + r - SF_TEXT_Y0;
        const int slot = T->text_slot[tc];
        if (slot < 7) {
          int div = 1;
          for (int k = slot; k < 6; k++) div *= 10;
          unsigned a = T->text_alpha[(pts / div) % 10][tr * SF_TEXT_W + tc];
          if (a) {
            unsigned char* px = &W.patch[(iy0 + r - ny0) * SF_PATCH_STRIDE + (ix0 + c - nx0)];
            *px = (unsigned char)sf_blend(*px, T->colour_text, a);
          }
        }
      });
      __syncwarp();
    }
  }
  {
    const int ix0 = max(SF_BAR_X0, nx0), ix1 = min(SF_BAR_X0 + SF_BAR_W, nx1);
    const int iy0 = max(SF_BAR_Y0, ny0), iy1 = min(SF_BAR_Y0 + SF_BAR_H, ny1);
    if (ix0 < ix1 && iy0 < iy1) {
      const int filled = 4 * min(rec.vuln, 10);
      const unsigned fg = rec.kill_bar ? T->colour_bar_kill : T->colour_bar_fg;
      sf_for_rect(lane, ix1 - ix0, iy1 - iy0, [&](int c, int r) {
        const unsigned a = T->bar_alpha[iy0 + r - SF_BAR_Y0];
        unsigned char* px = &W.patch[(iy0 + r - ny0) * SF_PATCH_STRIDE + (ix0 + c - nx0)];
        unsigned v = sf_blend(*px, T->colour_bar_bg, a);
        if (ix0 + c - SF_BAR_X0 < filled) v = sf_blend(v, fg, a);
        *px = (unsigned char)v;
      });
      __syncwarp();
    }
  }
  return no_wireframe;
}

__device__ __noinline__ void sf_window_out(int win, int orect, unsigned char* __restrict__ obs84, unsigned char* __restrict__ cache, int corigin) {
  const SfWarpSmem& W = sf_my_smem();
  const SfBlockSmem& B = sf_block_smem();
  const int lane = threadIdx.x & 31;
  const int nx0 = SF_WIN_X0(win), ny0 = SF_WIN_Y0(win);
  const int j0 = orect & 255, i0 = (orect >> 8) & 255;
  sf_for_rect(lane, (orect >> 16) & 255, (int)((unsigned)orect >> 24), [&](int c, int r) {
    const int i = i0 + r, j = j0 + c;
    const int4 tx = B.xtap[j], ty = B.ytap[i];
    const unsigned char* S = &W.patch[((ty.x & 255) - ny0) * SF_PATCH_STRIDE + ((tx.x & 255) - nx0)];
    const float ax0 = __int_as_float(tx.y), ax1 = __int_as_float(tx.z);
    const float b0 = __fadd_rn(__fmul_rn((float)S[0], ax0), __fmul_rn((float)S[1], ax1));
    const float b1 = __fadd_rn(__fmul_rn((float)S[SF_PATCH_STRIDE], ax0), __fmul_rn((float)S[SF_PATCH_STRIDE + 1], ax1));
    const float b2 = __fadd_rn(__fmul_rn((float)S[2 * SF_PATCH_STRIDE], ax0), __fmul_rn((float)S[2 * SF_PATCH_STRIDE + 1], ax1));
    float sum = __fmul_rn(__int_as_float(ty.y), b0);
    sum = __fadd_rn(sum, __fmul_rn(__int_as_float(ty.z), b1));
    sum = __fadd_rn(sum, __fmul_rn(__int_as_float(ty.w), b2));
    const unsigned char v = (unsigned char)__float2int_rn(sum);
    obs84[i * 84 + j] = v;
    if (cache) cache[(i - (corigin >> 8)) * SF_EXPO_STRIDE + (j - (corigin & 255))] = v;
  });
}

__device__ __forceinline__ bool sf_window_orect(const SfTables* T, unsigned char* expcache, int e, int j0, int i0, int j1, int i1, unsigned char* obs84,
                                                unsigned char* cache, int corigin, int sg) {
  const SfBlockSmem& B = sf_block_smem();
  const int tx0 = B.xtap[j0].x, tx1 = B.xtap[j1].x, ty0 = B.ytap[i0].x, ty1 = B.ytap[i1].x;
  const int nx0 = tx0 & 255, nx1 = (tx1 & 255) + (tx1 >> 8) - 1, ny0 = ty0 & 255, ny1 = (ty1 & 255) + (ty1 >> 8) - 1;
  if (nx1 - nx0 + 1 > SF_WIN_MAX_W || ny1 - ny0 + 1 > SF_WIN_MAX_H) __trap();
  const int win = nx0 | (ny0 << 8) | ((nx1 - nx0 + 1) << 16) | ((ny1 - ny0 + 1) << 24);
  const int orect = j0 | (i0 << 8) | ((j1 - j0 + 1) << 16) | ((i1 - i0 + 1) << 24);
  const bool pure = sf_composite(T, expcache, e, win, sg);
  SF_PROF(27);
  sf_window_out(win, orect, obs84, pure ? cache : nullptr, corigin);
  __syncwarp();
  SF_PROF(28);
  return pure && cache;
}

__device__ __forceinline__ int sf_wire_geometry(SfWarpSmem& W, int lane, const SfTables* T, int kind, double px, double py, int angle, int sg) {
  SF_PROF(31);
  const int slot = lane >> 2, line = lane & 3;
  SfQuadGeom G;
  G.ymin_g = 1 << 30; G.ymax_g = -(1 << 30); G.xmin = 1 << 30; G.xmax = -(1 << 30); G.split = 0; G.flags = 0;
  bool has = false;
  if (kind >= 0) {
    double dxv = SF_DADD(SF_DMUL(px, SF_CTM_SCALE), SF_CTM_X0), dyv = SF_DADD(SF_DMUL(py, SF_CTM_SCALE), SF_CTM_Y0);
    bool visible = !(dxv < -9.0 || dxv > SF_NAT_W + 9.0 || dyv < -9.0 || dyv > SF_NAT_H + 9.0);
    const SfBlockSmem& B = sf_block_smem();
    if (visible && line < B.wf_nlines[kind]) {
      const double2 cs = make_double2(B.hot.cs[angle][0], B.hot.cs[angle][1]);
      SfWireXf m = sf_wire_xf(px, py, cs.x, cs.y);
      const double* L = B.wf_line[kind][line];
      SfPt a = sf_xform_wire(m, L[0], L[1]), b = sf_xform_wire(m, L[2], L[3]);
      SfQuad q;
      if (sf_stroke_quad(a, b, q)) {
        sf_store_quad_edges(T, lane, q.p[0].x, q.p[0].y, q.p[1].x, q.p[1].y, q.p[2].x, q.p[2].y, q.p[3].x, q.p[3].y, G);
        has = G.ymin_g < G.ymax_g;
      }
    }
  }
  int ymin_g = G.ymin_g, ymax_g = G.ymax_g, xmin = G.xmin, xmax = G.xmax;
#pragma unroll
  for (int o = 1; o <= 2; o <<= 1) {
    ymin_g = min(ymin_g, __shfl_xor_sync(0xffffffffu, ymin_g, o)); ymax_g = max(ymax_g, __shfl_xor_sync(0xffffffffu, ymax_g, o));
    xmin = min(xmin, __shfl_xor_sync(0xffffffffu, xmin, o)); xmax = max(xmax, __shfl_xor_sync(0xffffffffu, xmax, o));
  }
  SF_PROF(16);
  int rid = sf_open_regions(lane, line == 0 && kind >= 0, ymin_g, ymax_g, xmin, xmax, sf_block_smem().colour_white, kind == 0 ? SF_TAG_SHIP : SF_TAG_PROJECTILE, sg);
  SF_PROF(17);
  rid = __shfl_sync(0xffffffffu, rid, lane & ~3);
  sf_publish_quads(W, lane, G, has, rid, line == 0 && kind >= 0, slot, kind >= 0 ? sf_block_smem().wf_nlines[kind] : 0, ymin_g, ymax_g, sg);
  SF_PROF(18);
  return rid;
}

__device__ __forceinline__ void sf_phase_exp_items(const SfDev& D, int be, int lane, int wi, int nw, int sg) {
  SfTeamSmem& Tm = sf_team(sg);
  const SfEnvRec& rec = Tm.env[be];
  const SfPt c = sf_xform_base(rec.px, rec.py);
  const SfExpPhase& P = D.tab->exp_phase[c.y & 255];
  const int Y = c.y >> 8, bx0 = (c.x >> 8) - 13, by0 = Y - 13;
  const int n = __ldg(&P.n_items);
  for (int q = wi * 32 + lane; q < SF_EXP_QUADS; q += nw * 32) { Tm.exp_item0[q] = __ldg(&P.item0[q]); Tm.exp_row0[q] = __ldg(&P.row0[q]); Tm.exp_qxmin[q] = __ldg(&P.qxmin[q]); }
#pragma unroll 1
  for (int it = wi * 32 + lane; it < n; it += nw * 32) {
    const uint2 Iw = __ldg(reinterpret_cast<const uint2*>(&P.item[it]));
    const int quad = Iw.x & 255, row = Y + (int)(signed char)((Iw.x >> 8) & 255), ns = (Iw.x >> 16) & 255, span0 = Iw.y & 0xFFFF;
    const int colmin = (c.x + __ldg(&P.qxmin[quad])) >> 8;
    const int shift = c.x - (colmin << 8);
    int acc[SF_EXPT_NC];
#pragma unroll
    for (int cc = 0; cc < SF_EXPT_NC; cc++) acc[cc] = 0;
    if (row >= 0 && row < SF_NAT_H) {
      unsigned sp[SF_GRID_Y];
#pragma unroll
      for (int k = 0; k < SF_GRID_Y; k++) sp[k] = k < ns ? __ldg(reinterpret_cast<const unsigned*>(&P.span[span0 + k][0])) : 0u;
#pragma unroll
      for (int k = 0; k < SF_GRID_Y; k++) {
        const int a = (int)(short)(sp[k] & 0xFFFFu) + shift, b = (int)(short)(sp[k] >> 16) + shift;
#pragma unroll
        for (int cc = 0; cc < SF_EXPT_NC; cc++) acc[cc] += max(min(b, (cc + 1) << 8) - max(a, cc << 8), 0);
      }
    }
#pragma unroll
    for (int cc = 0; cc < SF_EXPT_NC; cc++) {
      Tm.exp_len[it][cc] = (unsigned short)acc[cc];
      const int col = colmin + cc;
      if (acc[cc] && (unsigned)col < (unsigned)SF_NAT_W && (unsigned)(row - by0) < (unsigned)SF_EXP_W && (unsigned)(col - bx0) < (unsigned)SF_EXP_W) atomicOr(&Tm.arc_mask[(row - by0) * SF_EXP_W + (col - bx0)][quad >> 5], 1u << (quad & 31));
    }
  }
}

__device__ __forceinline__ void sf_phase_sprite(const SfDev& D, SfBlockSmem& B, int be, int lane, int wi, int nw, int sg) {
  SfTeamSmem& Tm = sf_team(sg);
  const SfTables* T = D.tab;
  SfEnvRec& rec = Tm.env[be];
  const SfPt c = sf_xform_base(rec.px, rec.py);
  const SfExpPhase& P = T->exp_phase[c.y & 255];
  const int Y = c.y >> 8, bx0 = (c.x >> 8) - 13, by0 = Y - 13;
  unsigned char* sprite = D.expc + (size_t)rec.env * (SF_EXP_W * SF_EXP_W);
#pragma unroll 1
  for (int p = wi * 32 + lane; p < SF_EXP_W * SF_EXP_W; p += nw * 32) {
    const int y = p / SF_EXP_W, x = p - y * SF_EXP_W;
    const int nx = bx0 + x, ny = by0 + y;
    unsigned v = 0;
    if ((unsigned)nx < (unsigned)SF_NAT_W && (unsigned)ny < (unsigned)SF_NAT_H) {
      v = B.bg_nat[ny * SF_NAT_STRIDE + nx];
      const uint4 M = *reinterpret_cast<const uint4*>(Tm.arc_mask[p]);
      unsigned circle = 0;
#pragma unroll 1
      for (int wd = 0; wd < 4; wd++) {
        unsigned m = wd == 0 ? M.x : wd == 1 ? M.y : wd == 2 ? M.z : M.w;
        while (m) {
          const int q = wd * 32 + __ffs(m) - 1;
          m &= m - 1;
          const int it = Tm.exp_item0[q] + (ny - Y - (int)Tm.exp_row0[q]);
          const int colmin = (c.x + Tm.exp_qxmin[q]) >> 8;
          const unsigned L = Tm.exp_len[it][nx - colmin];
          if (q < SF_EXP_STROKES - 1) v = sf_blend(v, B.exp_colour[q], sf_len_to_alpha(L));
          else circle += L;
        }
      }
      if (circle) v = sf_blend(v, B.exp_colour[SF_EXP_STROKES - 1], sf_len_to_alpha(circle));
      *reinterpret_cast<uint4*>(Tm.arc_mask[p]) = make_uint4(0u, 0u, 0u, 0u);
    }
    sprite[p] = (unsigned char)v;
  }
  if (wi == 0 && lane == 0) D.expstamp[rec.env] = rec.life;
}

struct SfFrameOut {
  unsigned char* obs;
  size_t obs_bytes;
  size_t tick_bytes;
  int native;
};
__device__ __forceinline__ unsigned char* sf_frame_ptr(const SfFrameOut& out, int e, int env) {
  return out.obs + (size_t)(e >> 5) * out.tick_bytes + (size_t)env * out.obs_bytes;
}

__device__ __forceinline__ unsigned sf_visible_shells(const SfDev& D, int env, unsigned pmask) {
  unsigned vis = 0;
  const double thr = D.tab->hot.touch2[2];
  for (unsigned m = (pmask >> SF_PMASK_SHELL_SHIFT) & 0xFu; m; m &= m - 1) {
    const int s = __ffs(m) - 1;
    const double2 p = D.spos[(size_t)s * D.n_pad + env];
    const double dx = SF_DSUB(p.x, SF_FORT_X), dy = SF_DSUB(p.y, SF_FORT_Y);
    if (SF_DADD(SF_DMUL(dx, dx), SF_DMUL(dy, dy)) > thr) vis |= 1u << s;
  }
  return vis;
}
__device__ __forceinline__ int sf_count_strokes(unsigned core, unsigned pmask, unsigned vis) {
  return ((core & SF_CORE_SHIP_ALIVE) ? 1 : 0) + __popc(pmask & SF_PMASK_MISSILES) + __popc(vis);
}

struct SfScanState {
  int carry_cnt, carry_need, carry_task;
  int r1, nst, build_env, build_env2, nbuilders;
  bool closed;
  unsigned later_any;
};
__device__ __forceinline__ void sf_scan_begin(SfScanState& S) {
  S.carry_cnt = 0; S.carry_need = 0; S.carry_task = 0;
  S.r1 = 0; S.nst = 0; S.build_env = -1; S.build_env2 = -1; S.nbuilders = 0;
  S.closed = false; S.later_any = 0u;
}
__device__ __forceinline__ void sf_scan_half(SfTeamSmem& Tm, int lane, int h, int r_begin, SfScanState& S) {
  if (!S.closed) S.r1 = 32 * (h + 1);
  const int slot = 32 * h + lane;
  SfEnvRec& rec = Tm.env[slot];
  const bool cand = slot >= r_begin && rec.env >= 0;
  const int cnt = cand ? rec.ns : 0;
  int need = 0;
  if (cand) need = ((rec.core & SF_CORE_SHIP_ALIVE) ? SF_CELLS_SHIP : 0) + __popc(rec.pmask & SF_PMASK_MISSILES) * SF_CELLS_MISSILE + __popc(rec.shell_vis) * SF_CELLS_SHELL;
  const bool deadc = cand && !(rec.core & SF_CORE_SHIP_ALIVE), scorec = cand && rec.points_i > 0;
  const int qvalidc = deadc ? (rec.building >> 4) & 15 : 0;
  const int cnttc = (deadc ? 4 - __popc(qvalidc) : 0) + (scorec ? 1 : 0);
  unsigned long long packed = (unsigned long long)cnt | ((unsigned long long)need << 12) | ((unsigned long long)cnttc << 32);
#pragma unroll
  for (int o = 1; o < 32; o <<= 1) { const unsigned long long t = __shfl_up_sync(0xffffffffu, packed, o); if (lane >= o) packed += t; }
  const int incl = (int)(packed & 0xFFFu) + S.carry_cnt, incl_need = (int)((packed >> 12) & 0xFFFFFu) + S.carry_need;
  const int inclt_all = (int)(packed >> 32);
  const unsigned builders = __ballot_sync(0xffffffffu, cand && (rec.building & 1));
  unsigned third = builders;
  for (int k = S.nbuilders; k < 2 && third; k++) third &= third - 1;
  const unsigned over = __ballot_sync(0xffffffffu, incl > SF_ROUND_STROKES || incl_need > SF_POOL_CELLS) | (third ? ~((third & (0u - third)) - 1u) : 0u);
  if (!S.closed && over) { S.r1 = 32 * h + __ffs(over) - 1; S.closed = true; }
  for (unsigned bm = builders; bm && S.build_env2 < 0; bm &= bm - 1) {
    const int sl = 32 * h + __ffs(bm) - 1;
    if (S.build_env < 0) S.build_env = sl; else S.build_env2 = sl;
  }
  S.nbuilders += __popc(builders);
  const bool in_round = cand && slot < S.r1;
  if (in_round) rec.s0 = incl - cnt;
  const unsigned inr = __ballot_sync(0xffffffffu, in_round);
  if (inr) S.nst = __shfl_sync(0xffffffffu, incl, 31 - __clz((int)inr));
  S.later_any |= __ballot_sync(0xffffffffu, cand && slot >= S.r1);
  if (in_round) {
    int k = inclt_all - cnttc + S.carry_task;
    if (deadc) for (int q = 0; q < 4; q++) if (!((qvalidc >> q) & 1)) Tm.etask[k++] = (unsigned short)(slot | (q << 6));
    if (scorec) Tm.etask[k] = (unsigned short)(slot | (4 << 6));
  }
  if (inr) S.carry_task += __shfl_sync(0xffffffffu, inclt_all, 31 - __clz((int)inr));
  S.carry_cnt = __shfl_sync(0xffffffffu, incl, 31); S.carry_need = __shfl_sync(0xffffffffu, incl_need, 31);
}
__device__ __forceinline__ void sf_scan_finish(SfTeamSmem& Tm, int lane, int r_begin, const SfScanState& S) {
  if (lane == 0) {
    Tm.more = S.later_any != 0u;
    Tm.r0 = r_begin; Tm.r1 = S.r1; Tm.nstrokes = S.nst;
    Tm.build_env = (S.build_env >= 0 && S.build_env < S.r1) ? S.build_env : -1;
    Tm.build_env2 = (Tm.build_env >= 0 && S.build_env2 >= 0 && S.build_env2 < S.r1) ? S.build_env2 : -1;
    Tm.base_ready = 0;
#ifndef SF_CHUNK_WARPS
#define SF_CHUNK_WARPS 12
#endif
    Tm.chunk = min(max((S.nst + SF_CHUNK_WARPS - 1) / SF_CHUNK_WARPS, 1), 8);
    Tm.netask = S.carry_task;
  }
  __syncwarp();
}
__device__ __forceinline__ void sf_round_scan(SfTeamSmem& Tm, int lane, int r_begin, int nslots) {
  SfScanState S;
  sf_scan_begin(S);
#pragma unroll
  for (int h = 0; h < SF_STAGE_TICKS; h++)
    if (32 * h < nslots && 32 * (h + 1) > r_begin) sf_scan_half(Tm, lane, h, r_begin, S);
  sf_scan_finish(Tm, lane, r_begin, S);
}

__device__ __forceinline__ void sf_env_base_issue(const SfBlockSmem& B, int e, const SfFrameOut& out, int sg) {
  const int env = sf_team(sg).env[e].env;
  if (env < 0) return;
  const unsigned src = (unsigned)__cvta_generic_to_shared(B.bg_obs);
  unsigned char* gb = sf_frame_ptr(out, e, env);
  asm volatile("cp.async.bulk.global.shared::cta.bulk_group [%0], [%1], %2;" :: "l"(gb), "r"(src), "r"(84 * 84) : "memory");
  asm volatile("cp.async.bulk.commit_group;" ::: "memory");
}
__device__ __forceinline__ void sf_env_base_patch(const SfDev& D, const SfBlockSmem& B, int lane, int e, const SfFrameOut& out, int sg) {
  const SfTables* T = D.tab;
  const SfEnvRec& rec = sf_team(sg).env[e];
  const int env = rec.env;
  if (env < 0) return;
  const unsigned core = rec.core;
  const int fst = (core & SF_CORE_FORT_ALIVE) ? (int)((core >> SF_CORE_FANG_SHIFT) & 63u) : 36;
  const int bst = rec.kill_bar ? 11 : min(rec.vuln, 10);
  int4* g = reinterpret_cast<int4*>(sf_frame_ptr(out, e, env));
  const int4* ft = reinterpret_cast<const int4*>(T->obs_fort[fst]);
  const int fc0 = T->fort_chunk0;
  const int c0 = lane < 16 ? B.fort_sparse[fst][lane] : 255;
  const bool bar = bst != 0 && lane < SF_OBS_CHUNKS - SF_BAR_CHUNK0;
  int4 v0, vb;
  if (c0 != 255) v0 = __ldg(&ft[c0]);
  if (bar) vb = __ldg(reinterpret_cast<const int4*>(T->obs_bar[bst]) + lane);
  if (c0 != 255) g[fc0 + c0] = v0;
  if (bar) g[SF_BAR_CHUNK0 + lane] = vb;
  if (fst == 36) {
    const int nsp = T->fort_sparse_n[fst];
#pragma unroll 1
    for (int k = 16 + lane; k < nsp; k += 32) { const int c = T->fort_sparse[fst][k]; g[fc0 + c] = __ldg(&ft[c]); }
  }
  const int qvalid = !(core & SF_CORE_SHIP_ALIVE) ? (rec.building >> 4) & 15 : 0;
  if (qvalid) {
    __syncwarp();
    const int bx0 = (rec.ebox & 255) - 64, by0 = ((rec.ebox >> 8) & 255) - 64;
    const int x0 = max(bx0, 0), y0 = max(by0, 0), x1 = min(bx0 + SF_EXP_W, SF_NAT_W) - 1, y1 = min(by0 + SF_EXP_W, SF_NAT_H) - 1;
    if (x0 <= x1 && y0 <= y1) {
      const int j0 = B.col_out0[x0], j1 = B.col_out1[x1], i0 = B.row_out0[y0], i1 = B.row_out1[y1];
      const int hb = (i1 - i0 + 4) >> 2, oh = i1 - i0 + 1;
      const int ja = j0 & ~3;
      const unsigned* src = reinterpret_cast<const unsigned*>(D.expo + (size_t)env * SF_EXPO_BYTES);
      unsigned char* dst = sf_frame_ptr(out, e, env) + i0 * 84 + ja;
      unsigned rows = 0u;
#pragma unroll
      for (int q = 0; q < 4; q++)
        if ((qvalid >> q) & 1) { const int ra = q * hb, rb = min(ra + hb, oh); if (ra < rb) rows |= ((rb - ra >= 32 ? 0u : (1u << (rb - ra))) - 1u) << ra; }
      const int wfull0 = (j0 - ja + 3) >> 2, wfull1 = (j1 + 1 - ja) >> 2;
      unsigned v[8];
#pragma unroll
      for (int u = 0; u < 8; u++) {
        const int k = lane + 32 * u, w = k & 7;
        const bool on = ((rows >> (k >> 3)) & 1u) && w >= wfull0 && w < wfull1;
        v[u] = on ? __ldcg(&src[k]) : 0u;
      }
#pragma unroll
      for (int u = 0; u < 8; u++) {
        const int k = lane + 32 * u, w = k & 7;
        if (((rows >> (k >> 3)) & 1u) && w >= wfull0 && w < wfull1) *reinterpret_cast<unsigned*>(dst + (k >> 3) * 84 + 4 * w) = v[u];
      }
      if ((rows >> lane) & 1u) {
        const int wl = wfull0 - 1, wr = wfull1;
        if (wl >= 0) {
          const unsigned x = __ldcg(&src[lane * 8 + wl]);
          unsigned char* p = dst + lane * 84 + 4 * wl;
#pragma unroll
          for (int b = 0; b < 4; b++) { const int c = ja + 4 * wl + b; if (c >= j0 && c <= j1) p[b] = (unsigned char)(x >> (8 * b)); }
        }
        if (wr != wl && ja + 4 * wr <= j1) {
          const unsigned x = __ldcg(&src[lane * 8 + wr]);
          unsigned char* p = dst + lane * 84 + 4 * wr;
#pragma unroll
          for (int b = 0; b < 4; b++) { const int c = ja + 4 * wr + b; if (c >= j0 && c <= j1) p[b] = (unsigned char)(x >> (8 * b)); }
        }
      }
    }
  }
}

__device__ __forceinline__ void sf_gather_strokes(const SfDev& D, SfTeamSmem& Tm, int lane, int h) {
  const int slot = 32 * h + lane;
  const SfEnvRec& rec = Tm.env[slot];
  if (slot >= Tm.r0 && slot < Tm.r1 && rec.env >= 0) {
    const int env = rec.env, np = D.n_pad;
    const unsigned core = rec.core;
    SfStrokeRec* S = &Tm.stroke[rec.s0];
    if (core & SF_CORE_SHIP_ALIVE) { S->x = rec.px; S->y = rec.py; S->desc = 0 | ((int)(core & SF_CORE_ANGLE_MASK) << 2) | (slot << 12); S->region = -1; S++; }
    for (unsigned m = rec.pmask & SF_PMASK_MISSILES; m;) {
      const int k0 = __ffs(m) - 1; m &= m - 1;
      const int k1 = m ? __ffs(m) - 1 : k0; m &= m - 1;
      const int k2 = m ? __ffs(m) - 1 : k0; m &= m - 1;
      const double2 p0 = D.mpos[(size_t)k0 * np + env], p1 = D.mpos[(size_t)k1 * np + env], p2 = D.mpos[(size_t)k2 * np + env];
      const int a0 = D.mang[(size_t)k0 * np + env], a1 = D.mang[(size_t)k1 * np + env], a2 = D.mang[(size_t)k2 * np + env];
      S->x = p0.x; S->y = p0.y; S->desc = 1 | (a0 << 2) | (slot << 12); S->region = -1; S++;
      if (k1 != k0) { S->x = p1.x; S->y = p1.y; S->desc = 1 | (a1 << 2) | (slot << 12); S->region = -1; S++; }
      if (k2 != k0) { S->x = p2.x; S->y = p2.y; S->desc = 1 | (a2 << 2) | (slot << 12); S->region = -1; S++; }
    }
    for (unsigned m = (unsigned)rec.shell_vis; m; m &= m - 1) {
      const int k = __ffs(m) - 1;
      const double2 p = D.spos[(size_t)k * np + env];
      int angle = __double2int_rz(D.sang[(size_t)k * np + env]);
      if (angle >= 360) angle -= 360;
      S->x = p.x; S->y = p.y; S->desc = 2 | (angle << 2) | (slot << 12); S->region = -1; S++;
    }
  }
  __syncwarp();
}

__device__ __forceinline__ void sf_phase_strokes(const SfDev& D, SfBlockSmem& B, SfWarpSmem& W, int lane, int wi, int nw, int nst, int sg) {
  const SfTables* T = D.tab;
  SfTeamSmem& Tm = sf_team(sg);
  const int chunk = Tm.chunk;
  const int be = Tm.build_env;
  if (be >= 0) sf_phase_exp_items(D, be, lane, nw - 1 - wi, nw, sg);
  SF_PROF(21);
  const int s = wi * chunk;
  if (s < nst) {
    SF_PROF_COUNT(67, 1);
    const int slot = lane >> 2;
    const bool valid = slot < chunk && s + slot < nst;
    const int idx = s + slot;
    int kind = -1, angle = 0;
    double x = 0, y = 0;
    if (valid) {
      const SfStrokeRec& S = Tm.stroke[idx];
      x = S.x; y = S.y; kind = S.desc & 3; angle = (S.desc >> 2) & 1023;
    }
    const int rid = sf_wire_geometry(W, lane, T, kind, x, y, angle, sg);
    if (valid && (lane & 3) == 0) Tm.stroke[idx].region = rid;
  } else {
    if (lane == 0) W.ngroups = 0;
  }
  sf_render_sync();
  SF_PROF(64);
  if (be >= 0) {
    sf_phase_sprite(D, B, be, lane, wi, nw, sg);
    if (Tm.build_env2 >= 0) {
      sf_render_sync();
      sf_phase_exp_items(D, Tm.build_env2, lane, wi, nw, sg);
      sf_render_sync();
      sf_phase_sprite(D, B, Tm.build_env2, lane, wi, nw, sg);
    }
  }
  const int mine = lane < nw ? (sf_warp_smem(lane + 1).ngroups + 3) >> 2 : 0;
  int incl = mine;
#pragma unroll
  for (int o = 1; o < 32; o <<= 1) { int t = __shfl_up_sync(0xffffffffu, incl, o); if (lane >= o) incl += t; }
  const int total = __shfl_sync(0xffffffffu, incl, 31);
  SF_PROF_COUNT(68, total);
#pragma unroll 1
  for (int g = wi; g < total; g += nw) {
    const int owner = __popc(__ballot_sync(0xffffffffu, incl <= g));
    const int first = __shfl_sync(0xffffffffu, incl - mine, owner);
    sf_accumulate_pass(owner + 1, (g - first) << 2, sg);
  }
  SF_PROF(20);
}

__device__ __forceinline__ void sf_phase_window(const SfDev& D, SfBlockSmem& B, SfWarpSmem& W, int lane, int t, int netask, const SfFrameOut& out, int sg) {
  const SfTables* T = D.tab;
  int e, j0, i0, j1, i1;
  int quarter = -1, corigin = 0;
  if (t < netask) {
    const int et = sf_team(sg).etask[t], kind = et >> 6;
    e = et & 63;
    const SfEnvRec& rec = sf_team(sg).env[e];
    int x0, y0, x1, y1;
    if (kind < 4) {
      const int bx0 = (rec.ebox & 255) - 64, by0 = ((rec.ebox >> 8) & 255) - 64;
      x0 = max(bx0, 0); y0 = max(by0, 0); x1 = min(bx0 + SF_EXP_W, SF_NAT_W) - 1; y1 = min(by0 + SF_EXP_W, SF_NAT_H) - 1;
      if (x0 > x1 || y0 > y1) return;
    } else {
      x0 = SF_TEXT_X0; y0 = SF_TEXT_Y0; x1 = SF_TEXT_X0 + SF_TEXT_W - 1; y1 = SF_TEXT_Y0 + SF_TEXT_H - 1;
    }
    j0 = B.col_out0[x0]; j1 = B.col_out1[x1]; i0 = B.row_out0[y0]; i1 = B.row_out1[y1];
    if (kind < 4) {
      const int hb = (i1 - i0 + 4) >> 2;
      corigin = (j0 & ~3) | (i0 << 8);
      i0 += kind * hb; i1 = min(i1, i0 + hb - 1);
      if (i0 > i1) return;
      quarter = kind;
    }
  } else {
    const SfStrokeRec& S = sf_team(sg).stroke[t - netask];
    const int sr = S.region;
    if (sr < 0) return;
    e = S.desc >> 12;
    const int4 R = sf_team(sg).region[sr];
    j0 = B.col_out0[R.x]; j1 = B.col_out1[R.x + (R.z & 0xFFFF) - 1]; i0 = B.row_out0[R.y]; i1 = B.row_out1[R.y + ((R.z >> 16) & 0xFFFF) - 1];
  }
  const int env = sf_team(sg).env[e].env;
  const bool cached = sf_window_orect(T, D.expc + (size_t)env * (SF_EXP_W * SF_EXP_W), e, j0, i0, j1, i1, sf_frame_ptr(out, e, env),
                                      quarter >= 0 ? D.expo + (size_t)env * SF_EXPO_BYTES : nullptr, corigin, sg);
  if (cached && lane == 0) {
    const SfEnvRec& rec = sf_team(sg).env[e];
    const unsigned long long want = (unsigned long long)rec.life | ((unsigned long long)sf_expo_key(rec) << 32);
    unsigned long long* m = reinterpret_cast<unsigned long long*>(&D.expo_meta[env]);
    unsigned long long old = *reinterpret_cast<volatile unsigned long long*>(m);
    while ((old & 0x0FFFFFFFFFFFFFFFull) == want) {
      const unsigned long long prev = atomicCAS(m, old, old | (1ull << (60 + quarter)));
      if (prev == old) break;
      old = prev;
    }
  }
  (void)W;
}

__device__ __forceinline__ void sf_phase_native_tile(const SfDev& D, SfBlockSmem& B, SfWarpSmem& W, int lane, int e, int tile, const SfFrameOut& out, int sg) {
  const int env = sf_team(sg).env[e].env;
  if (env < 0) return;
  const int tx = (tile % 3) * 30, ty = (tile / 3) * 30;
  const int pw = min(30, SF_NAT_W - tx), ph = min(30, SF_NAT_H - ty);
  const int win = tx | (ty << 8) | (pw << 16) | (ph << 24);
  (void)sf_composite(D.tab, D.expc + (size_t)env * (SF_EXP_W * SF_EXP_W), e, win, sg);
  unsigned char* dst = sf_frame_ptr(out, e, env) + ty * SF_NAT_W + tx;
  sf_for_rect(lane, pw, ph, [&](int c, int r) { dst[r * SF_NAT_W + c] = W.patch[r * SF_PATCH_STRIDE + c]; });
  __syncwarp();
}

#ifdef SF_PHASE_TIMING
#define SF_TICK(k) do { if (threadIdx.x == 32 && blockIdx.x == 0) { long long now_ = clock64(); atomicAdd(&sf_dbg_cycles[k], (unsigned long long)(now_ - t_last_)); t_last_ = now_; } } while (0)
#define SF_WTICK(k) do { if (lane == 0 && blockIdx.x == 0) { long long now_ = clock64(); atomicAdd(&sf_dbg_cycles[k], (unsigned long long)(now_ - w_last_)); w_last_ = now_; } } while (0)
#else
#define SF_TICK(k) ((void)0)
#define SF_WTICK(k) ((void)0)
#endif

__device__ __forceinline__ void sf_publish_recs(const SfDev& D, SfTeamSmem& Tm, int lane, int h, bool native) {
  SfEnvRec& r = Tm.env[32 * h + lane];
  if (r.env >= 0 && !(r.core & SF_CORE_SHIP_ALIVE)) {
    const unsigned stamp = __ldcg(&D.expstamp[r.env]);
    const unsigned long long mw = __ldcg(reinterpret_cast<const unsigned long long*>(&D.expo_meta[r.env]));
    const unsigned mx = (unsigned)mw, my = (unsigned)(mw >> 32);
    int building = stamp != r.life ? 1 : 0;
    if (h > 0 && building && !(Tm.env[lane].core & SF_CORE_SHIP_ALIVE) && Tm.env[lane].env == r.env && Tm.env[lane].life == r.life) building = 0;
    if (!native) {
      const unsigned key = sf_expo_key(r);
      const bool same = mx == r.life && (my & 0x0FFFFFFFu) == key;
      if (same) { if (!building) building |= (int)(my >> 28) << 4; }
      else atomicExch(reinterpret_cast<unsigned long long*>(&D.expo_meta[r.env]), (unsigned long long)r.life | ((unsigned long long)key << 32));
    }
    r.building = building;
  }
  __syncwarp();
}

struct SfStageState {
  int stage;
  int prev_used;
};

__device__ __forceinline__ void sf_restart_pools(SfTeamSmem& Tm, int lane) {
  if (lane == 0) { Tm.next_task = 0; Tm.next_patch = 0; Tm.nregions = 0; Tm.cells_used = 0; }
  __syncwarp();
}

template <class Prep>
__device__ __forceinline__ void sf_prepare_first_round(const SfDev& D, const SfBlockSmem& B, SfTeamSmem& Tm, int lane, int t, int nt, SfFrameOut out, Prep prep) {
  const bool native = out.native != 0;
#ifdef SF_BARRIER_TIMING
  long long tb_ = clock64();
#define SF_BT(k) do { sf_bar_add(k, tb_); tb_ = clock64(); } while (0)
#else
#define SF_BT(k) ((void)0)
#endif
  prep(t, Tm, 0);
  SF_BT(3);
  sf_publish_recs(D, Tm, lane, 0, native);
  SF_BT(4);
  SfScanState S;
  sf_scan_begin(S);
  sf_scan_half(Tm, lane, 0, 0, S);
  sf_scan_finish(Tm, lane, 0, S);
  SF_BT(5);
  sf_gather_strokes(D, Tm, lane, 0);
  SF_BT(6);
  int nticks = 1;
#if SF_STAGE_TICKS > 1
  if (nt > 1 && !Tm.more) {
    prep(t + 1, Tm, 1);
    SF_BT(3);
    sf_publish_recs(D, Tm, lane, 1, native);
    SF_BT(4);
    sf_scan_half(Tm, lane, 1, 0, S);
    sf_scan_finish(Tm, lane, 0, S);
    SF_BT(5);
    sf_gather_strokes(D, Tm, lane, 1);
    SF_BT(6);
    nticks = 2;
  }
#endif
  if (lane == 0) Tm.nticks = nticks;
  sf_restart_pools(Tm, lane);
  SF_BT(7);
}

__device__ __forceinline__ void sf_draw_stage(const SfDev& D, SfBlockSmem& B, SfWarpSmem& W, int lane, const SfFrameOut& out, int sg) {
  const int warp = threadIdx.x >> 5;
  const int wi = warp - 1, nw = SF_RENDER_WARPS - 1;
  SfTeamSmem& Tm = sf_team(sg);
#ifdef SF_PHASE_TIMING
  long long t_last_ = clock64(), w_last_ = t_last_;
  const int gwarp = warp;
#endif
  const int r0 = Tm.r0, r1 = Tm.r1, nst = Tm.nstrokes;
  const bool base_issuer = !out.native && wi == nw - 1;
  if (base_issuer) {
#pragma unroll 1
    for (int e = r0 + lane; e < r1; e += 32) sf_env_base_issue(B, e, out, sg);
  }
  SF_PROF_RESET();
  sf_phase_strokes(D, B, W, lane, wi, nw, nst, sg);
  SF_PROF(69);
  if (!out.native) {
    if (base_issuer) {
      asm volatile("cp.async.bulk.wait_group 0;" ::: "memory");
      __syncwarp();
      if (lane == 0) { __threadfence_block(); *(volatile int*)&Tm.base_ready = 1; }
    } else {
      while (*(volatile int*)&Tm.base_ready == 0) {}
    }
    __syncwarp();
    SF_PROF(65);
#pragma unroll 1
    for (;;) {
      int e = 0;
      if (lane == 0) e = atomicAdd(&Tm.next_patch, 1);
      e = r0 + __shfl_sync(0xffffffffu, e, 0);
      if (e >= r1) break;
      sf_env_base_patch(D, B, lane, e, out, sg);
    }
    SF_PROF(66);
  }
#ifdef SF_PHASE_TIMING
  if (lane == 0 && blockIdx.x == 0) { atomicAdd(&sf_dbg_cycles[32 + (gwarp & 15)], (unsigned long long)(clock64() - w_last_)); atomicMax(&Tm.dbg_max_b, (int)(clock64() - w_last_)); }
#endif
  SF_WTICK(10);
  sf_render_sync();
  SF_TICK(2); SF_WTICK(8);
  SF_PROF_RESET();
  if (!out.native) {
    const int netask = Tm.netask;
#pragma unroll 1
    for (;;) {
      int t = 0;
      if (lane == 0) t = atomicAdd(&Tm.next_task, 1);
      t = __shfl_sync(0xffffffffu, t, 0);
      if (t >= netask + nst) break;
      SF_PROF(29);
      sf_phase_window(D, B, W, lane, t, netask, out, sg);
    }
  } else {
#pragma unroll 1
    for (int t = wi; t < (r1 - r0) * 12; t += nw) sf_phase_native_tile(D, B, W, lane, r0 + t / 12, t % 12, out, sg);
  }
#ifdef SF_PHASE_TIMING
  if (lane == 0 && blockIdx.x == 0) { atomicAdd(&sf_dbg_cycles[48 + (gwarp & 15)], (unsigned long long)(clock64() - w_last_)); atomicMax(&Tm.dbg_max_c, (int)(clock64() - w_last_)); }
  SF_WTICK(11);
  if (threadIdx.x == 32 && blockIdx.x == 0) {
    atomicAdd(&sf_dbg_cycles[71], (unsigned long long)Tm.dbg_max_b); atomicAdd(&sf_dbg_cycles[72], (unsigned long long)Tm.dbg_max_c);
    atomicAdd(&sf_dbg_cycles[73], 1ull); atomicAdd(&sf_dbg_cycles[74], (unsigned long long)(Tm.netask + nst)); atomicAdd(&sf_dbg_cycles[75], (unsigned long long)Tm.netask);
    atomicAdd(&sf_dbg_cycles[76], (unsigned long long)(Tm.build_env >= 0));
    Tm.dbg_max_b = 0; Tm.dbg_max_c = 0;
  }
#endif
}

template <class Prep>
__device__ __forceinline__ void sf_stepper_ticks(const SfDev& D, SfBlockSmem& B, int lane, bool native, int T, int& stage, Prep prep) {
  SfFrameOut out;
  out.obs = nullptr; out.obs_bytes = 0; out.tick_bytes = 0; out.native = native ? 1 : 0;
  sf_prepare_first_round(D, B, B.team[stage], lane, 0, T, out, prep);
  SF_TL(3);
  int t = 0;
#pragma unroll 1
  for (;;) {
    SF_TL(4);
    sf_team_sync();
    SF_TL(5);
    SfTeamSmem& Tm = B.team[stage];
    SfTeamSmem& Nx = B.team[stage ^ 1];
    const bool more = Tm.more != 0;
    const int nticks = Tm.nticks;
    const bool last = !more && t + nticks >= T;
    if (more) {
#pragma unroll
      for (int h = 0; h < SF_STAGE_TICKS; h++) Nx.env[32 * h + lane] = Tm.env[32 * h + lane];
      if (lane == 0) Nx.nticks = nticks;
      __syncwarp();
      sf_round_scan(Nx, lane, Tm.r1, SF_GROUP_ENVS * nticks);
      sf_gather_strokes(D, Nx, lane, nticks - 1);
      sf_restart_pools(Nx, lane);
    } else if (!last) {
      sf_prepare_first_round(D, B, Nx, lane, t + nticks, T - (t + nticks), out, prep);
    }
    stage ^= 1;
    if (!more) t += nticks;
    if (last) break;
  }
  SF_TL(7);
}

__device__ __forceinline__ void sf_drawer_ticks(const SfDev& D, SfBlockSmem& B, SfWarpSmem& W, int lane, SfFrameOut out, int T, SfStageState& st) {
  unsigned char* const obs0 = out.obs;
  int t = 0;
#pragma unroll 1
  for (;;) {
    SF_TL(4);
    sf_team_sync();
    SF_TL(5);
    SfTeamSmem& Tm = B.team[st.stage];
    SfTeamSmem& Nx = B.team[st.stage ^ 1];
    const bool more = Tm.more != 0;
    const int nticks = Tm.nticks;
    const bool last = !more && t + nticks >= T;
    {
      const int nz = (st.prev_used + 1) >> 1;
      for (int k = threadIdx.x - 32; k < nz; k += 32 * (SF_RENDER_WARPS - 1)) reinterpret_cast<unsigned*>(Nx.cells)[k] = 0u;
    }
    out.obs = obs0 + (size_t)t * out.tick_bytes;
    sf_draw_stage(D, B, W, lane, out, st.stage);
    st.prev_used = Tm.cells_used;
    st.stage ^= 1;
    if (!more) t += nticks;
    if (last) break;
  }
  SF_TL(7);
}
```

Baseline: 155.2 million.

## Replace double-buffered team smem with a multi-slot prep ring and producer/consumer barriers

```diff
diff --git a/spacefortress_b200/csrc/sf_kernels.cu b/spacefortress_b200/csrc/sf_kernels.cu
--- a/spacefortress_b200/csrc/sf_kernels.cu
+++ b/spacefortress_b200/csrc/sf_kernels.cu
@@ -182,11 +182,12 @@
   const bool native = (A.flags & SF_FLAG_NATIVE_OBS) != 0;
   int stage = 0, group = blockIdx.x;
 #pragma unroll 1
-  for (int k = 1; group < A.ngroups; k ^= 1) {
+  for (int k = 0; group < A.ngroups; k = (k + 1) % SF_NEXT_GROUPS) {
     if (lane == 0) B.next_group[k] = A.sched ? (int)gridDim.x + atomicAdd(&A.sched->next_group, 1) : group + (int)gridDim.x;
-    sf_stepper_ticks(D, B, lane, native, A.T, stage, [&](int t, SfTeamSmem& Tm, int h) { sf_step_group(D, A, group, t, &Tm.env[32 * h]); });
+    sf_stepper_ticks(D, B, lane, native, A.T, stage, [&](int t, SfStagePrep& Tm, int h) { sf_step_group(D, A, group, t, &Tm.env[32 * h]); });
     group = B.next_group[k];
   }
+  sf_stepper_drain(stage);
   if (lane == 0 && A.sched) {
     __threadfence();
     if (atomicAdd(&A.sched->done, 1) == (int)gridDim.x - 1) { A.sched->next_group = 0; A.sched->done = 0; __threadfence(); }
@@ -205,7 +206,7 @@
   st.stage = 0; st.prev_used = 0;
   int group = blockIdx.x;
 #pragma unroll 1
-  for (int k = 1; group < A.ngroups; k ^= 1) {
+  for (int k = 0; group < A.ngroups; k = (k + 1) % SF_NEXT_GROUPS) {
     sf_drawer_ticks(D, B, W, lane, out, A.T, st);
     group = B.next_group[k];
   }
@@ -302,7 +303,7 @@
     int stage = 0;
 #pragma unroll 1
     for (int group = blockIdx.x; group < ngroups; group += gridDim.x)
-      sf_stepper_ticks(D, B, lane, native, 1, stage, [&](int, SfTeamSmem& Tm, int) {
+      sf_stepper_ticks(D, B, lane, native, 1, stage, [&](int, SfStagePrep& Tm, int) {
         const int env = group * EB + lane;
         const bool mine = lane < EB && env < D.n && (!mask || mask[env]);
         if (mine) {
@@ -312,6 +313,7 @@
         } else Tm.env[lane].env = -1;
         __syncwarp();
       });
+    sf_stepper_drain(stage);
   } else {
     SfFrameOut out;
     out.native = native ? 1 : 0;
diff --git a/spacefortress_b200/csrc/sf_render.cuh b/spacefortress_b200/csrc/sf_render.cuh
--- a/spacefortress_b200/csrc/sf_render.cuh
+++ b/spacefortress_b200/csrc/sf_render.cuh
@@ -65,17 +65,27 @@
   const int bst = r.kill_bar ? 11 : min(r.vuln, 10);
   return (unsigned)fst | ((unsigned)bst << 6) | (((unsigned)r.points_i & 0x3FFFFu) << 10);
 }
-struct __align__(8) SfStrokeRec { double x, y; int desc, region; };
-
-struct __align__(16) SfTeamSmem {
+struct __align__(8) SfStrokeRec { double x, y; int desc; };
+
+#ifndef SF_PREP_SLOTS
+#define SF_PREP_SLOTS 3
+#endif
+static_assert(SF_PREP_SLOTS >= 2 && SF_PREP_SLOTS <= 6, "named barriers 3 .. 3 + 2 * SF_PREP_SLOTS - 1 must exist (16 per block)");
+#define SF_NEXT_GROUPS 8
+static_assert(SF_PREP_SLOTS + 2 <= SF_NEXT_GROUPS, "next-group ring too small for the lead of the stepping warp");
+struct __align__(16) SfStagePrep {
   SfEnvRec env[SF_STAGE_SLOTS];
   SfStrokeRec stroke[SF_ROUND_STROKES];
+  int r0, r1, nstrokes, build_env;
+  int netask, chunk, more, nticks;
+  int build_env2, padp[3];
+  unsigned short etask[SF_STAGE_SLOTS * 5];
+};
+struct __align__(16) SfStagePool {
   int4 region[SF_POOL_REGIONS];
-  int r0, r1, nstrokes, build_env;
-  int next_task, netask, next_patch, chunk;
-  int more, nticks, build_env2, base_ready;
-  int nregions, cells_used, dbg_max_b, dbg_max_c;
-  unsigned short etask[SF_STAGE_SLOTS * 5];
+  short stroke_region[SF_ROUND_STROKES];
+  int next_task, next_patch, nregions, cells_used;
+  int base_ready, dbg_max_b, dbg_max_c, padq;
   unsigned short exp_item0[SF_EXP_QUADS];
   short exp_qxmin[SF_EXP_QUADS];
   signed char exp_row0[SF_EXP_QUADS];
@@ -111,27 +121,44 @@
 #ifdef SF_TIMELINE
   int tl_n[4];
 #endif
-  int next_group[2], padg[2];
+  int next_group[SF_NEXT_GROUPS];
   SfStepSmem step;
-  SfTeamSmem team[2];
+  SfStagePrep prep[SF_PREP_SLOTS];
+  SfStagePool pool;
 };
 
 #define SF_STATIC_BYTES ((offsetof(SfBlockSmem, init_mbar) + 15) & ~(size_t)15)
 
 extern __shared__ __align__(16) unsigned char sf_smem_raw[];
 __device__ __forceinline__ SfBlockSmem& sf_block_smem() { return *reinterpret_cast<SfBlockSmem*>(sf_smem_raw); }
-__device__ __forceinline__ SfTeamSmem& sf_team(int sg) { return sf_block_smem().team[sg]; }
+__device__ __forceinline__ SfStagePrep& sf_prep(int sg) { return sf_block_smem().prep[sg]; }
+__device__ __forceinline__ SfStagePool& sf_pool() { return sf_block_smem().pool; }
 #ifdef SF_BARRIER_TIMING
 __device__ unsigned long long sf_bar_cycles[16];
 __device__ __forceinline__ void sf_bar_add(int k, long long t0) { if ((threadIdx.x & 31) == 0) atomicAdd(&sf_bar_cycles[k], (unsigned long long)(clock64() - t0)); }
 #endif
-__device__ __forceinline__ void sf_team_sync() {
+__device__ __forceinline__ void sf_stage_full_arrive(int sg) {
+  asm volatile("bar.arrive %0, %1;" :: "r"(3 + sg), "r"(32 * SF_RENDER_WARPS) : "memory");
+}
+__device__ __forceinline__ void sf_stage_full_wait(int sg) {
 #ifdef SF_BARRIER_TIMING
   const long long t0 = clock64();
 #endif
-  asm volatile("bar.sync 1, %0;" :: "r"(32 * SF_RENDER_WARPS) : "memory");
+  asm volatile("bar.sync %0, %1;" :: "r"(3 + sg), "r"(32 * SF_RENDER_WARPS) : "memory");
 #ifdef SF_BARRIER_TIMING
-  sf_bar_add(threadIdx.x < 32 ? 2 : 0, t0);
+  sf_bar_add(0, t0);
+#endif
+}
+__device__ __forceinline__ void sf_stage_empty_arrive(int sg) {
+  asm volatile("bar.arrive %0, %1;" :: "r"(3 + SF_PREP_SLOTS + sg), "r"(32 * SF_RENDER_WARPS) : "memory");
+}
+__device__ __forceinline__ void sf_stage_empty_wait(int sg) {
+#ifdef SF_BARRIER_TIMING
+  const long long t0 = clock64();
+#endif
+  asm volatile("bar.sync %0, %1;" :: "r"(3 + SF_PREP_SLOTS + sg), "r"(32 * SF_RENDER_WARPS) : "memory");
+#ifdef SF_BARRIER_TIMING
+  sf_bar_add(2, t0);
 #endif
 }
 __device__ __forceinline__ void sf_render_sync() {
@@ -242,14 +269,10 @@
     asm volatile("cp.async.bulk.shared::cluster.global.mbarrier::complete_tx::bytes [%0], [%1], %2, [%3];"
                  :: "r"((unsigned)__cvta_generic_to_shared(&B)), "l"(image), "r"((unsigned)SF_STATIC_BYTES), "r"(bar) : "memory");
   }
-  for (int c = 0; c < 2; c++) {
-    for (int k = threadIdx.x; k < SF_POOL_CELLS / 2; k += blockDim.x) reinterpret_cast<unsigned*>(B.team[c].cells)[k] = 0u;
-    for (int k = threadIdx.x; k < SF_EXP_W * SF_EXP_W * 4; k += blockDim.x) (&B.team[c].arc_mask[0][0])[k] = 0u;
-    if (threadIdx.x == 32) {
-      SfTeamSmem& Tm = B.team[c];
-      Tm.next_task = 0; Tm.next_patch = 0; Tm.netask = 0; Tm.chunk = 8; Tm.nregions = 0; Tm.cells_used = 0;
-    }
-  }
+  for (int k = threadIdx.x; k < SF_POOL_CELLS / 2; k += blockDim.x) reinterpret_cast<unsigned*>(B.pool.cells)[k] = 0u;
+  for (int k = threadIdx.x; k < SF_EXP_W * SF_EXP_W * 4; k += blockDim.x) (&B.pool.arc_mask[0][0])[k] = 0u;
+  if (threadIdx.x == 32) { B.pool.next_task = 0; B.pool.next_patch = 0; B.pool.nregions = 0; B.pool.cells_used = 0; B.pool.base_ready = 0; }
+  for (int k = threadIdx.x; k < SF_PREP_SLOTS * SF_STAGE_SLOTS; k += blockDim.x) B.prep[k / SF_STAGE_SLOTS].env[k % SF_STAGE_SLOTS].env = -1;
   asm volatile("fence.proxy.async.shared::cta;" ::: "memory");
   __syncthreads();
   unsigned ok;
@@ -340,8 +363,8 @@
 
 __device__ __forceinline__ int sf_row_of(int g) { return (g >= 0) ? g / SF_GRID_Y : -((-g + SF_GRID_Y - 1) / SF_GRID_Y); }
 
-__device__ __forceinline__ int sf_open_regions(int lane, bool want, int ymin_g, int ymax_g, int xmin, int xmax, unsigned colour, int tag, int sg) {
-  SfTeamSmem& Tm = sf_team(sg);
+__device__ __forceinline__ int sf_open_regions(int lane, bool want, int ymin_g, int ymax_g, int xmin, int xmax, unsigned colour, int tag) {
+  SfStagePool& Tm = sf_pool();
   int cx0 = 0, py0 = 0, w = 0, h = 0;
   bool ok = want && ymin_g < ymax_g;
   if (ok) {
@@ -366,8 +389,8 @@
   return rid;
 }
 
-__device__ __forceinline__ void sf_publish_quads(SfWarpSmem& W, int lane, const SfQuadGeom& G, bool has, int rid, bool head, int slot, int nq, int ymin_g, int ymax_g, int sg) {
-  const SfTeamSmem& Tm = sf_team(sg);
+__device__ __forceinline__ void sf_publish_quads(SfWarpSmem& W, int lane, const SfQuadGeom& G, bool has, int rid, bool head, int slot, int nq, int ymin_g, int ymax_g) {
+  const SfStagePool& Tm = sf_pool();
   int len = 0;
   int4 R = make_int4(0, 0, 0, 0);
   if (rid >= 0) R = Tm.region[rid];
@@ -415,11 +438,11 @@
     for (int c = c1 + 1; c < c2; c++) { const int cm = cell0 + c; atomicAdd(&acc32[cm >> 1], 256u << ((cm & 1) << 4)); }
 }
 
-__device__ __noinline__ void sf_accumulate_pass(int owner, int g0, int sg) {
+__device__ __noinline__ void sf_accumulate_pass(int owner, int g0) {
   const SfWarpSmem& W = sf_warp_smem(owner);
   const int lane = threadIdx.x & 31;
   const int ngroups = W.ngroups;
-  unsigned* acc32 = reinterpret_cast<unsigned*>(sf_team(sg).cells);
+  unsigned* acc32 = reinterpret_cast<unsigned*>(sf_pool().cells);
   const int gi = min(g0 + (lane >> 3), ngroups - 1);
   const int ent = W.glist[gi];
   const int4 S = W.srec[ent & 31];
@@ -458,9 +481,9 @@
   __syncwarp();
 }
 
-__device__ __noinline__ void sf_blend_region(int rid, int win, int sg) {
+__device__ __noinline__ void sf_blend_region(int rid, int win) {
   SfWarpSmem& W = sf_my_smem();
-  const SfTeamSmem& O = sf_team(sg);
+  const SfStagePool& O = sf_pool();
   const int lane = threadIdx.x & 31;
   const int4 R = O.region[rid];
   const int w = R.z & 0xFFFF, h = (R.z >> 16) & 0xFFFF;
@@ -484,7 +507,7 @@
 __device__ __noinline__ bool sf_composite(const SfTables* T, unsigned char* expcache, int e, int win, int sg) {
   SfWarpSmem& W = sf_my_smem();
   const SfBlockSmem& B = sf_block_smem();
-  const SfEnvRec& rec = sf_team(sg).env[e];
+  const SfEnvRec& rec = sf_prep(sg).env[e];
   const int lane = threadIdx.x & 31;
   const unsigned core = rec.core;
   const int nx0 = SF_WIN_X0(win), ny0 = SF_WIN_Y0(win);
@@ -495,9 +518,9 @@
   int sr = -1, tag = SF_TAG_PROJECTILE;
   bool hit = false;
   if (lane < rec.ns) {
-    sr = sf_team(sg).stroke[rec.s0 + lane].region;
+    sr = sf_pool().stroke_region[rec.s0 + lane];
     if (sr >= 0) {
-      const int4 R = sf_team(sg).region[sr];
+      const int4 R = sf_pool().region[sr];
       hit = R.x < nx1 && R.x + (R.z & 0xFFFF) > nx0 && R.y < ny1 && R.y + ((R.z >> 16) & 0xFFFF) > ny0;
       tag = (R.w >> 15) & 1;
     }
@@ -507,7 +530,7 @@
   const bool first_is_ship = __shfl_sync(0xffffffffu, tag, 0) == SF_TAG_SHIP;
   SF_PROF(23);
   if (core & SF_CORE_SHIP_ALIVE) {
-    if ((rmask & 1u) && first_is_ship) { const int s0r = __shfl_sync(0xffffffffu, sr, 0); sf_blend_region(s0r, win, sg); rmask &= ~1u; }
+    if ((rmask & 1u) && first_is_ship) { const int s0r = __shfl_sync(0xffffffffu, sr, 0); sf_blend_region(s0r, win); rmask &= ~1u; }
   } else {
     const int ebox = rec.ebox;
     const int bx0 = (ebox & 255) - 64, by0 = ((ebox >> 8) & 255) - 64;
@@ -582,7 +605,7 @@
     const int q = __ffs(rmask) - 1;
     rmask &= rmask - 1;
     const int sq = __shfl_sync(0xffffffffu, sr, q);
-    sf_blend_region(sq, win, sg);
+    sf_blend_region(sq, win);
   }
   SF_PROF(26);
   {
@@ -664,7 +687,7 @@
   return pure && cache;
 }
 
-__device__ __forceinline__ int sf_wire_geometry(SfWarpSmem& W, int lane, const SfTables* T, int kind, double px, double py, int angle, int sg) {
+__device__ __forceinline__ int sf_wire_geometry(SfWarpSmem& W, int lane, const SfTables* T, int kind, double px, double py, int angle) {
   SF_PROF(31);
   const int slot = lane >> 2, line = lane & 3;
   SfQuadGeom G;
@@ -693,17 +716,17 @@
     xmin = min(xmin, __shfl_xor_sync(0xffffffffu, xmin, o)); xmax = max(xmax, __shfl_xor_sync(0xffffffffu, xmax, o));
   }
   SF_PROF(16);
-  int rid = sf_open_regions(lane, line == 0 && kind >= 0, ymin_g, ymax_g, xmin, xmax, sf_block_smem().colour_white, kind == 0 ? SF_TAG_SHIP : SF_TAG_PROJECTILE, sg);
+  int rid = sf_open_regions(lane, line == 0 && kind >= 0, ymin_g, ymax_g, xmin, xmax, sf_block_smem().colour_white, kind == 0 ? SF_TAG_SHIP : SF_TAG_PROJECTILE);
   SF_PROF(17);
   rid = __shfl_sync(0xffffffffu, rid, lane & ~3);
-  sf_publish_quads(W, lane, G, has, rid, line == 0 && kind >= 0, slot, kind >= 0 ? sf_block_smem().wf_nlines[kind] : 0, ymin_g, ymax_g, sg);
+  sf_publish_quads(W, lane, G, has, rid, line == 0 && kind >= 0, slot, kind >= 0 ? sf_block_smem().wf_nlines[kind] : 0, ymin_g, ymax_g);
   SF_PROF(18);
   return rid;
 }
 
 __device__ __forceinline__ void sf_phase_exp_items(const SfDev& D, int be, int lane, int wi, int nw, int sg) {
-  SfTeamSmem& Tm = sf_team(sg);
-  const SfEnvRec& rec = Tm.env[be];
+  SfStagePool& Tm = sf_pool();
+  const SfEnvRec& rec = sf_prep(sg).env[be];
   const SfPt c = sf_xform_base(rec.px, rec.py);
   const SfExpPhase& P = D.tab->exp_phase[c.y & 255];
   const int Y = c.y >> 8, bx0 = (c.x >> 8) - 13, by0 = Y - 13;
@@ -739,9 +762,9 @@
 }
 
 __device__ __forceinline__ void sf_phase_sprite(const SfDev& D, SfBlockSmem& B, int be, int lane, int wi, int nw, int sg) {
-  SfTeamSmem& Tm = sf_team(sg);
+  SfStagePool& Tm = sf_pool();
   const SfTables* T = D.tab;
-  SfEnvRec& rec = Tm.env[be];
+  const SfEnvRec& rec = sf_prep(sg).env[be];
   const SfPt c = sf_xform_base(rec.px, rec.py);
   const SfExpPhase& P = T->exp_phase[c.y & 255];
   const int Y = c.y >> 8, bx0 = (c.x >> 8) - 13, by0 = Y - 13;
@@ -812,7 +835,7 @@
   S.r1 = 0; S.nst = 0; S.build_env = -1; S.build_env2 = -1; S.nbuilders = 0;
   S.closed = false; S.later_any = 0u;
 }
-__device__ __forceinline__ void sf_scan_half(SfTeamSmem& Tm, int lane, int h, int r_begin, SfScanState& S) {
+__device__ __forceinline__ void sf_scan_half(SfStagePrep& Tm, int lane, int h, int r_begin, SfScanState& S) {
   if (!S.closed) S.r1 = 32 * (h + 1);
   const int slot = 32 * h + lane;
   SfEnvRec& rec = Tm.env[slot];
@@ -851,13 +874,12 @@
   if (inr) S.carry_task += __shfl_sync(0xffffffffu, inclt_all, 31 - __clz((int)inr));
   S.carry_cnt = __shfl_sync(0xffffffffu, incl, 31); S.carry_need = __shfl_sync(0xffffffffu, incl_need, 31);
 }
-__device__ __forceinline__ void sf_scan_finish(SfTeamSmem& Tm, int lane, int r_begin, const SfScanState& S) {
+__device__ __forceinline__ void sf_scan_finish(SfStagePrep& Tm, int lane, int r_begin, const SfScanState& S) {
   if (lane == 0) {
     Tm.more = S.later_any != 0u;
     Tm.r0 = r_begin; Tm.r1 = S.r1; Tm.nstrokes = S.nst;
     Tm.build_env = (S.build_env >= 0 && S.build_env < S.r1) ? S.build_env : -1;
     Tm.build_env2 = (Tm.build_env >= 0 && S.build_env2 >= 0 && S.build_env2 < S.r1) ? S.build_env2 : -1;
-    Tm.base_ready = 0;
 #ifndef SF_CHUNK_WARPS
 #define SF_CHUNK_WARPS 12
 #endif
@@ -866,7 +888,7 @@
   }
   __syncwarp();
 }
-__device__ __forceinline__ void sf_round_scan(SfTeamSmem& Tm, int lane, int r_begin, int nslots) {
+__device__ __forceinline__ void sf_round_scan(SfStagePrep& Tm, int lane, int r_begin, int nslots) {
   SfScanState S;
   sf_scan_begin(S);
 #pragma unroll
@@ -876,7 +898,7 @@
 }
 
 __device__ __forceinline__ void sf_env_base_issue(const SfBlockSmem& B, int e, const SfFrameOut& out, int sg) {
-  const int env = sf_team(sg).env[e].env;
+  const int env = sf_prep(sg).env[e].env;
   if (env < 0) return;
   const unsigned src = (unsigned)__cvta_generic_to_shared(B.bg_obs);
   unsigned char* gb = sf_frame_ptr(out, e, env);
@@ -885,7 +907,7 @@
 }
 __device__ __forceinline__ void sf_env_base_patch(const SfDev& D, const SfBlockSmem& B, int lane, int e, const SfFrameOut& out, int sg) {
   const SfTables* T = D.tab;
-  const SfEnvRec& rec = sf_team(sg).env[e];
+  const SfEnvRec& rec = sf_prep(sg).env[e];
   const int env = rec.env;
   if (env < 0) return;
   const unsigned core = rec.core;
@@ -953,30 +975,30 @@
   }
 }
 
-__device__ __forceinline__ void sf_gather_strokes(const SfDev& D, SfTeamSmem& Tm, int lane, int h) {
+__device__ __forceinline__ void sf_gather_strokes(const SfDev& D, SfStagePrep& Tm, int lane, int h) {
   const int slot = 32 * h + lane;
   const SfEnvRec& rec = Tm.env[slot];
   if (slot >= Tm.r0 && slot < Tm.r1 && rec.env >= 0) {
     const int env = rec.env, np = D.n_pad;
     const unsigned core = rec.core;
     SfStrokeRec* S = &Tm.stroke[rec.s0];
-    if (core & SF_CORE_SHIP_ALIVE) { S->x = rec.px; S->y = rec.py; S->desc = 0 | ((int)(core & SF_CORE_ANGLE_MASK) << 2) | (slot << 12); S->region = -1; S++; }
+    if (core & SF_CORE_SHIP_ALIVE) { S->x = rec.px; S->y = rec.py; S->desc = 0 | ((int)(core & SF_CORE_ANGLE_MASK) << 2) | (slot << 12); S++; }
     for (unsigned m = rec.pmask & SF_PMASK_MISSILES; m;) {
       const int k0 = __ffs(m) - 1; m &= m - 1;
       const int k1 = m ? __ffs(m) - 1 : k0; m &= m - 1;
       const int k2 = m ? __ffs(m) - 1 : k0; m &= m - 1;
       const double2 p0 = D.mpos[(size_t)k0 * np + env], p1 = D.mpos[(size_t)k1 * np + env], p2 = D.mpos[(size_t)k2 * np + env];
       const int a0 = D.mang[(size_t)k0 * np + env], a1 = D.mang[(size_t)k1 * np + env], a2 = D.mang[(size_t)k2 * np + env];
-      S->x = p0.x; S->y = p0.y; S->desc = 1 | (a0 << 2) | (slot << 12); S->region = -1; S++;
-      if (k1 != k0) { S->x = p1.x; S->y = p1.y; S->desc = 1 | (a1 << 2) | (slot << 12); S->region = -1; S++; }
-      if (k2 != k0) { S->x = p2.x; S->y = p2.y; S->desc = 1 | (a2 << 2) | (slot << 12); S->region = -1; S++; }
+      S->x = p0.x; S->y = p0.y; S->desc = 1 | (a0 << 2) | (slot << 12); S++;
+      if (k1 != k0) { S->x = p1.x; S->y = p1.y; S->desc = 1 | (a1 << 2) | (slot << 12); S++; }
+      if (k2 != k0) { S->x = p2.x; S->y = p2.y; S->desc = 1 | (a2 << 2) | (slot << 12); S++; }
     }
     for (unsigned m = (unsigned)rec.shell_vis; m; m &= m - 1) {
       const int k = __ffs(m) - 1;
       const double2 p = D.spos[(size_t)k * np + env];
       int angle = __double2int_rz(D.sang[(size_t)k * np + env]);
       if (angle >= 360) angle -= 360;
-      S->x = p.x; S->y = p.y; S->desc = 2 | (angle << 2) | (slot << 12); S->region = -1; S++;
+      S->x = p.x; S->y = p.y; S->desc = 2 | (angle << 2) | (slot << 12); S++;
     }
   }
   __syncwarp();
@@ -984,7 +1006,7 @@
 
 __device__ __forceinline__ void sf_phase_strokes(const SfDev& D, SfBlockSmem& B, SfWarpSmem& W, int lane, int wi, int nw, int nst, int sg) {
   const SfTables* T = D.tab;
-  SfTeamSmem& Tm = sf_team(sg);
+  const SfStagePrep& Tm = sf_prep(sg);
   const int chunk = Tm.chunk;
   const int be = Tm.build_env;
   if (be >= 0) sf_phase_exp_items(D, be, lane, nw - 1 - wi, nw, sg);
@@ -1001,8 +1023,8 @@
       const SfStrokeRec& S = Tm.stroke[idx];
       x = S.x; y = S.y; kind = S.desc & 3; angle = (S.desc >> 2) & 1023;
     }
-    const int rid = sf_wire_geometry(W, lane, T, kind, x, y, angle, sg);
-    if (valid && (lane & 3) == 0) Tm.stroke[idx].region = rid;
+    const int rid = sf_wire_geometry(W, lane, T, kind, x, y, angle);
+    if (valid && (lane & 3) == 0) sf_pool().stroke_region[idx] = (short)rid;
   } else {
     if (lane == 0) W.ngroups = 0;
   }
@@ -1027,7 +1049,7 @@
   for (int g = wi; g < total; g += nw) {
     const int owner = __popc(__ballot_sync(0xffffffffu, incl <= g));
     const int first = __shfl_sync(0xffffffffu, incl - mine, owner);
-    sf_accumulate_pass(owner + 1, (g - first) << 2, sg);
+    sf_accumulate_pass(owner + 1, (g - first) << 2);
   }
   SF_PROF(20);
 }
@@ -1037,9 +1059,9 @@
   int e, j0, i0, j1, i1;
   int quarter = -1, corigin = 0;
   if (t < netask) {
-    const int et = sf_team(sg).etask[t], kind = et >> 6;
+    const int et = sf_prep(sg).etask[t], kind = et >> 6;
     e = et & 63;
-    const SfEnvRec& rec = sf_team(sg).env[e];
+    const SfEnvRec& rec = sf_prep(sg).env[e];
     int x0, y0, x1, y1;
     if (kind < 4) {
       const int bx0 = (rec.ebox & 255) - 64, by0 = ((rec.ebox >> 8) & 255) - 64;
@@ -1054,21 +1076,20 @@
       corigin = (j0 & ~3) | (i0 << 8);
       i0 += kind * hb; i1 = min(i1, i0 + hb - 1);
       if (i0 > i1) return;
-      quarter = kind;
+      quarter = (rec.building & 2) ? kind : -1;
     }
   } else {
-    const SfStrokeRec& S = sf_team(sg).stroke[t - netask];
-    const int sr = S.region;
+    const int sr = sf_pool().stroke_region[t - netask];
     if (sr < 0) return;
-    e = S.desc >> 12;
-    const int4 R = sf_team(sg).region[sr];
+    e = sf_prep(sg).stroke[t - netask].desc >> 12;
+    const int4 R = sf_pool().region[sr];
     j0 = B.col_out0[R.x]; j1 = B.col_out1[R.x + (R.z & 0xFFFF) - 1]; i0 = B.row_out0[R.y]; i1 = B.row_out1[R.y + ((R.z >> 16) & 0xFFFF) - 1];
   }
-  const int env = sf_team(sg).env[e].env;
+  const int env = sf_prep(sg).env[e].env;
   const bool cached = sf_window_orect(T, D.expc + (size_t)env * (SF_EXP_W * SF_EXP_W), e, j0, i0, j1, i1, sf_frame_ptr(out, e, env),
                                       quarter >= 0 ? D.expo + (size_t)env * SF_EXPO_BYTES : nullptr, corigin, sg);
   if (cached && lane == 0) {
-    const SfEnvRec& rec = sf_team(sg).env[e];
+    const SfEnvRec& rec = sf_prep(sg).env[e];
     const unsigned long long want = (unsigned long long)rec.life | ((unsigned long long)sf_expo_key(rec) << 32);
     unsigned long long* m = reinterpret_cast<unsigned long long*>(&D.expo_meta[env]);
     unsigned long long old = *reinterpret_cast<volatile unsigned long long*>(m);
@@ -1082,7 +1103,7 @@
 }
 
 __device__ __forceinline__ void sf_phase_native_tile(const SfDev& D, SfBlockSmem& B, SfWarpSmem& W, int lane, int e, int tile, const SfFrameOut& out, int sg) {
-  const int env = sf_team(sg).env[e].env;
+  const int env = sf_prep(sg).env[e].env;
   if (env < 0) return;
   const int tx = (tile % 3) * 30, ty = (tile / 3) * 30;
   const int pw = min(30, SF_NAT_W - tx), ph = min(30, SF_NAT_H - ty);
@@ -1101,21 +1122,30 @@
 #define SF_WTICK(k) ((void)0)
 #endif
 
-__device__ __forceinline__ void sf_publish_recs(const SfDev& D, SfTeamSmem& Tm, int lane, int h, bool native) {
-  SfEnvRec& r = Tm.env[32 * h + lane];
+__device__ __forceinline__ void sf_publish_recs(const SfDev& D, SfStagePrep* ring, int cur, int lane, int h, bool native) {
+  SfEnvRec& r = ring[cur].env[32 * h + lane];
   if (r.env >= 0 && !(r.core & SF_CORE_SHIP_ALIVE)) {
     const unsigned stamp = __ldcg(&D.expstamp[r.env]);
     const unsigned long long mw = __ldcg(reinterpret_cast<const unsigned long long*>(&D.expo_meta[r.env]));
     const unsigned mx = (unsigned)mw, my = (unsigned)(mw >> 32);
+    const unsigned key = sf_expo_key(r);
     int building = stamp != r.life ? 1 : 0;
-    if (h > 0 && building && !(Tm.env[lane].core & SF_CORE_SHIP_ALIVE) && Tm.env[lane].env == r.env && Tm.env[lane].life == r.life) building = 0;
+    bool refresh = true;
+#pragma unroll 1
+    for (int k = 0; k < SF_PREP_SLOTS * SF_STAGE_TICKS; k++) {
+      const int j = k / SF_STAGE_TICKS, hh = k - j * SF_STAGE_TICKS;
+      if (j == cur && hh >= h) continue;
+      const SfEnvRec& o = ring[j].env[32 * hh + lane];
+      if (o.env != r.env || (o.core & SF_CORE_SHIP_ALIVE)) continue;
+      if (o.life == r.life) building = 0;
+      if (o.life != r.life || sf_expo_key(o) != key) refresh = false;
+    }
     if (!native) {
-      const unsigned key = sf_expo_key(r);
       const bool same = mx == r.life && (my & 0x0FFFFFFFu) == key;
       if (same) { if (!building) building |= (int)(my >> 28) << 4; }
       else atomicExch(reinterpret_cast<unsigned long long*>(&D.expo_meta[r.env]), (unsigned long long)r.life | ((unsigned long long)key << 32));
     }
-    r.building = building;
+    r.building = building | (refresh ? 2 : 0);
   }
   __syncwarp();
 }
@@ -1125,13 +1155,9 @@
   int prev_used;
 };
 
-__device__ __forceinline__ void sf_restart_pools(SfTeamSmem& Tm, int lane) {
-  if (lane == 0) { Tm.next_task = 0; Tm.next_patch = 0; Tm.nregions = 0; Tm.cells_used = 0; }
-  __syncwarp();
-}
-
 template <class Prep>
-__device__ __forceinline__ void sf_prepare_first_round(const SfDev& D, const SfBlockSmem& B, SfTeamSmem& Tm, int lane, int t, int nt, SfFrameOut out, Prep prep) {
+__device__ __forceinline__ void sf_prepare_first_round(const SfDev& D, SfBlockSmem& B, int sg, int lane, int t, int nt, SfFrameOut out, Prep prep) {
+  SfStagePrep& Tm = B.prep[sg];
   const bool native = out.native != 0;
 #ifdef SF_BARRIER_TIMING
   long long tb_ = clock64();
@@ -1141,7 +1167,7 @@
 #endif
   prep(t, Tm, 0);
   SF_BT(3);
-  sf_publish_recs(D, Tm, lane, 0, native);
+  sf_publish_recs(D, B.prep, sg, lane, 0, native);
   SF_BT(4);
   SfScanState S;
   sf_scan_begin(S);
@@ -1155,7 +1181,7 @@
   if (nt > 1 && !Tm.more) {
     prep(t + 1, Tm, 1);
     SF_BT(3);
-    sf_publish_recs(D, Tm, lane, 1, native);
+    sf_publish_recs(D, B.prep, sg, lane, 1, native);
     SF_BT(4);
     sf_scan_half(Tm, lane, 1, 0, S);
     sf_scan_finish(Tm, lane, 0, S);
@@ -1166,14 +1192,15 @@
   }
 #endif
   if (lane == 0) Tm.nticks = nticks;
-  sf_restart_pools(Tm, lane);
+  __syncwarp();
   SF_BT(7);
 }
 
-__device__ __forceinline__ void sf_draw_stage(const SfDev& D, SfBlockSmem& B, SfWarpSmem& W, int lane, const SfFrameOut& out, int sg) {
+__device__ __forceinline__ int sf_draw_stage(const SfDev& D, SfBlockSmem& B, SfWarpSmem& W, int lane, const SfFrameOut& out, int sg) {
   const int warp = threadIdx.x >> 5;
   const int wi = warp - 1, nw = SF_RENDER_WARPS - 1;
-  SfTeamSmem& Tm = sf_team(sg);
+  const SfStagePrep& Tm = B.prep[sg];
+  SfStagePool& P = B.pool;
 #ifdef SF_PHASE_TIMING
   long long t_last_ = clock64(), w_last_ = t_last_;
   const int gwarp = warp;
@@ -1191,16 +1218,16 @@
     if (base_issuer) {
       asm volatile("cp.async.bulk.wait_group 0;" ::: "memory");
       __syncwarp();
-      if (lane == 0) { __threadfence_block(); *(volatile int*)&Tm.base_ready = 1; }
+      if (lane == 0) { __threadfence_block(); *(volatile int*)&P.base_ready = 1; }
     } else {
-      while (*(volatile int*)&Tm.base_ready == 0) {}
+      while (*(volatile int*)&P.base_ready == 0) {}
     }
     __syncwarp();
     SF_PROF(65);
 #pragma unroll 1
     for (;;) {
       int e = 0;
-      if (lane == 0) e = atomicAdd(&Tm.next_patch, 1);
+      if (lane == 0) e = atomicAdd(&P.next_patch, 1);
       e = r0 + __shfl_sync(0xffffffffu, e, 0);
       if (e >= r1) break;
       sf_env_base_patch(D, B, lane, e, out, sg);
@@ -1208,18 +1235,20 @@
     SF_PROF(66);
   }
 #ifdef SF_PHASE_TIMING
-  if (lane == 0 && blockIdx.x == 0) { atomicAdd(&sf_dbg_cycles[32 + (gwarp & 15)], (unsigned long long)(clock64() - w_last_)); atomicMax(&Tm.dbg_max_b, (int)(clock64() - w_last_)); }
+  if (lane == 0 && blockIdx.x == 0) { atomicAdd(&sf_dbg_cycles[32 + (gwarp & 15)], (unsigned long long)(clock64() - w_last_)); atomicMax(&P.dbg_max_b, (int)(clock64() - w_last_)); }
 #endif
   SF_WTICK(10);
+  const int used = P.cells_used;
   sf_render_sync();
   SF_TICK(2); SF_WTICK(8);
+  if (threadIdx.x == 32) { P.nregions = 0; P.cells_used = 0; P.next_patch = 0; P.base_ready = 0; }
   SF_PROF_RESET();
   if (!out.native) {
     const int netask = Tm.netask;
 #pragma unroll 1
     for (;;) {
       int t = 0;
-      if (lane == 0) t = atomicAdd(&Tm.next_task, 1);
+      if (lane == 0) t = atomicAdd(&P.next_task, 1);
       t = __shfl_sync(0xffffffffu, t, 0);
       if (t >= netask + nst) break;
       SF_PROF(29);
@@ -1230,34 +1259,50 @@
     for (int t = wi; t < (r1 - r0) * 12; t += nw) sf_phase_native_tile(D, B, W, lane, r0 + t / 12, t % 12, out, sg);
   }
 #ifdef SF_PHASE_TIMING
-  if (lane == 0 && blockIdx.x == 0) { atomicAdd(&sf_dbg_cycles[48 + (gwarp & 15)], (unsigned long long)(clock64() - w_last_)); atomicMax(&Tm.dbg_max_c, (int)(clock64() - w_last_)); }
+  if (lane == 0 && blockIdx.x == 0) { atomicAdd(&sf_dbg_cycles[48 + (gwarp & 15)], (unsigned long long)(clock64() - w_last_)); atomicMax(&P.dbg_max_c, (int)(clock64() - w_last_)); }
   SF_WTICK(11);
   if (threadIdx.x == 32 && blockIdx.x == 0) {
-    atomicAdd(&sf_dbg_cycles[71], (unsigned long long)Tm.dbg_max_b); atomicAdd(&sf_dbg_cycles[72], (unsigned long long)Tm.dbg_max_c);
+    atomicAdd(&sf_dbg_cycles[71], (unsigned long long)P.dbg_max_b); atomicAdd(&sf_dbg_cycles[72], (unsigned long long)P.dbg_max_c);
     atomicAdd(&sf_dbg_cycles[73], 1ull); atomicAdd(&sf_dbg_cycles[74], (unsigned long long)(Tm.netask + nst)); atomicAdd(&sf_dbg_cycles[75], (unsigned long long)Tm.netask);
     atomicAdd(&sf_dbg_cycles[76], (unsigned long long)(Tm.build_env >= 0));
-    Tm.dbg_max_b = 0; Tm.dbg_max_c = 0;
-  }
-#endif
+    P.dbg_max_b = 0; P.dbg_max_c = 0;
+  }
+#endif
+  return used;
+}
+
+
+__device__ __forceinline__ int sf_stepper_claim(int stage) {
+  const int sg = stage % SF_PREP_SLOTS;
+  SF_TL(4);
+  if (stage >= SF_PREP_SLOTS) sf_stage_empty_wait(sg);
+  SF_TL(5);
+  return sg;
+}
+__device__ __forceinline__ void sf_stepper_drain(int stage) {
+#pragma unroll 1
+  for (int s = max(stage - SF_PREP_SLOTS, 0); s < stage; s++)
+    asm volatile("bar.sync %0, %1;" :: "r"(3 + SF_PREP_SLOTS + s % SF_PREP_SLOTS), "r"(32 * SF_RENDER_WARPS) : "memory");
 }
 
 template <class Prep>
 __device__ __forceinline__ void sf_stepper_ticks(const SfDev& D, SfBlockSmem& B, int lane, bool native, int T, int& stage, Prep prep) {
   SfFrameOut out;
   out.obs = nullptr; out.obs_bytes = 0; out.tick_bytes = 0; out.native = native ? 1 : 0;
-  sf_prepare_first_round(D, B, B.team[stage], lane, 0, T, out, prep);
+  int sg = sf_stepper_claim(stage);
+  sf_prepare_first_round(D, B, sg, lane, 0, T, out, prep);
   SF_TL(3);
   int t = 0;
 #pragma unroll 1
   for (;;) {
-    SF_TL(4);
-    sf_team_sync();
-    SF_TL(5);
-    SfTeamSmem& Tm = B.team[stage];
-    SfTeamSmem& Nx = B.team[stage ^ 1];
+    sf_stage_full_arrive(sg);
+    stage++;
+    const SfStagePrep& Tm = B.prep[sg];
     const bool more = Tm.more != 0;
     const int nticks = Tm.nticks;
-    const bool last = !more && t + nticks >= T;
+    if (!more && t + nticks >= T) break;
+    const int nx = sf_stepper_claim(stage);
+    SfStagePrep& Nx = B.prep[nx];
     if (more) {
 #pragma unroll
       for (int h = 0; h < SF_STAGE_TICKS; h++) Nx.env[32 * h + lane] = Tm.env[32 * h + lane];
@@ -1265,13 +1310,11 @@
       __syncwarp();
       sf_round_scan(Nx, lane, Tm.r1, SF_GROUP_ENVS * nticks);
       sf_gather_strokes(D, Nx, lane, nticks - 1);
-      sf_restart_pools(Nx, lane);
-    } else if (!last) {
-      sf_prepare_first_round(D, B, Nx, lane, t + nticks, T - (t + nticks), out, prep);
-    }
-    stage ^= 1;
-    if (!more) t += nticks;
-    if (last) break;
+    } else {
+      sf_prepare_first_round(D, B, nx, lane, t + nticks, T - (t + nticks), out, prep);
+      t += nticks;
+    }
+    sg = nx;
   }
   SF_TL(7);
 }
@@ -1281,22 +1324,23 @@
   int t = 0;
 #pragma unroll 1
   for (;;) {
+    const int sg = st.stage;
     SF_TL(4);
-    sf_team_sync();
+    sf_stage_full_wait(sg);
     SF_TL(5);
-    SfTeamSmem& Tm = B.team[st.stage];
-    SfTeamSmem& Nx = B.team[st.stage ^ 1];
+    const SfStagePrep& Tm = B.prep[sg];
     const bool more = Tm.more != 0;
     const int nticks = Tm.nticks;
     const bool last = !more && t + nticks >= T;
     {
       const int nz = (st.prev_used + 1) >> 1;
-      for (int k = threadIdx.x - 32; k < nz; k += 32 * (SF_RENDER_WARPS - 1)) reinterpret_cast<unsigned*>(Nx.cells)[k] = 0u;
+      for (int k = threadIdx.x - 32; k < nz; k += 32 * (SF_RENDER_WARPS - 1)) reinterpret_cast<unsigned*>(B.pool.cells)[k] = 0u;
+      if (threadIdx.x == 32) B.pool.next_task = 0;
     }
     out.obs = obs0 + (size_t)t * out.tick_bytes;
-    sf_draw_stage(D, B, W, lane, out, st.stage);
-    st.prev_used = Tm.cells_used;
-    st.stage ^= 1;
+    st.prev_used = sf_draw_stage(D, B, W, lane, out, sg);
+    sf_stage_empty_arrive(sg);
+    st.stage = sg + 1 == SF_PREP_SLOTS ? 0 : sg + 1;
     if (!more) t += nticks;
     if (last) break;
   }
```

Result: faster. 160.5 million (median of 6 runs) (+3.4%).
